# jacarvalho/mpd-public

Measured on AMD Instinct MI355X. Metric: denoising-steps/s, higher is better.
Workload: dtype f32; 1 GPU; cfg2: EnvDense2D-RobotPointMass shape, 100 trajectories (1 context(s)) x H=64 x D=4, T=100 (+5) reverse steps, unguided, U-Net dim_mults (1, 2, 4, 8), one plan = one bench step; parallelism=single, denoising_steps_per_plan=105

## Files before the change

include/mpdx.h:

```cpp
#ifndef MPDX_H
#define MPDX_H

#include <stddef.h>
#include <stdint.h>

#ifdef __cplusplus
extern "C" {
#endif

#define MPDX_E_INVALID   (-1)
#define MPDX_E_NOTFOUND  (-2)
#define MPDX_E_STATE     (-3)
#define MPDX_E_DEVICE    (-4)

#define MPDX_MAX_LEVELS 8

typedef struct mpdx_unet mpdx_unet;

typedef struct mpdx_unet_cfg {
    int32_t state_dim;
    int32_t n_support_points;
    int32_t unet_input_dim;
    int32_t n_levels;
    int32_t dim_mults[MPDX_MAX_LEVELS];
    int32_t time_emb_dim;
    int32_t self_attention;
} mpdx_unet_cfg;

const char* mpdx_last_error(void);
int mpdx_version(void);

int    mpdx_unet_create(const mpdx_unet_cfg* cfg, mpdx_unet** out);
void   mpdx_unet_destroy(mpdx_unet* u);
int    mpdx_unet_set_plan_join(mpdx_unet* u, int on);
int    mpdx_unet_plan_joined(const mpdx_unet* u);
int    mpdx_unet_set_inner_run(mpdx_unet* u, int on);
int    mpdx_unet_set_inner_run_parts(mpdx_unet* u, int parts);
int    mpdx_unet_set_inner_run_width(mpdx_unet* u, int width);
int    mpdx_inner_run_block(int B, int width, int cus, int block, int32_t* cluster, int32_t* tile, int32_t* counter_lines);
int    mpdx_unet_inner_runs(const mpdx_unet* u);
int    mpdx_unet_inner_run_layers(const mpdx_unet* u);
int    mpdx_unet_status(const mpdx_unet* u);
int    mpdx_unet_set_status(mpdx_unet* u, unsigned word);
int    mpdx_unet_num_params(const mpdx_unet* u);
int    mpdx_unet_param_info(const mpdx_unet* u, int idx, const char** name, int32_t shape[3], int32_t* ndim);
size_t mpdx_unet_packed_floats(const mpdx_unet* u);
size_t mpdx_unet_timetab_floats(const mpdx_unet* u, int T);
size_t mpdx_unet_workspace_floats(const mpdx_unet* u, int B);
int    mpdx_unet_pack_param(mpdx_unet* u, const char* name, const float* src_dev, size_t n_floats,
                            float* packed_dev, void* stream);
int    mpdx_unet_build_timetab(mpdx_unet* u, const float* packed_dev, const float* freqs16_dev, int T,
                               float* timetab_dev, void* stream);

int mpdx_unet_forward(mpdx_unet* u, const float* packed_dev, const float* timetab_dev, int T,
                      const float* x, int t, float* eps, int B, float* ws, void* stream);

typedef struct mpdx_step_coefs {
    float sqrt_recip_alphas_cumprod;
    float sqrt_recipm1_alphas_cumprod;
    float posterior_mean_coef1;
    float posterior_mean_coef2;
    float noise_scale;
    float noise_std_extra;
    int32_t predict_epsilon;
    int32_t clip_denoised;
    float ddim_k1;
    float ddim_k2;
    float guide_scale;
} mpdx_step_coefs;

int mpdx_ddpm_step(mpdx_unet* u, const float* packed_dev, const float* timetab_dev, int T,
                   float* x_io, const float* noise, const float* hard_start, const float* hard_goal,
                   const mpdx_step_coefs* coefs, int t, int mean_only, float* chain_out,
                   uint32_t* absmax_out, int n_per_ctx, int B, float* ws, void* stream);

int mpdx_add_noise(float* x_io, const float* noise, const float* hard_start, const float* hard_goal,
                   float noise_scale, float noise_std_extra, float* chain_out, int B, int H, int D, void* stream);

int mpdx_hard_conds(float* x_io, float* chain_out, int n, const int32_t* horizon_idx, const float* const* values, int B, int H, int D, void* stream);

int mpdx_q_sample(const float* x_start, const float* noise, const long long* t_dev, const float* sqrt_alphas_cumprod_dev,
                  const float* sqrt_one_minus_alphas_cumprod_dev, const float* hard_start, const float* hard_goal, float* out, int B, int H,
                  int D, int T, void* stream);
int mpdx_weighted_loss(const float* pred, const float* targ, const float* weights_hd, const float* hard_start, const float* hard_goal,
                       int l1, float* out1, int B, int H, int D, void* stream);

size_t mpdx_train_flat_floats(mpdx_unet* u);
size_t mpdx_train_dgrad_pack_floats(mpdx_unet* u);
size_t mpdx_train_workspace_floats(mpdx_unet* u, int B);
int    mpdx_train_param_offset(mpdx_unet* u, int idx, size_t* off, size_t* n);
int    mpdx_train_pack(mpdx_unet* u, const float* flat, float* packed, float* packedT, void* stream);
int    mpdx_train_loss_backward(mpdx_unet* u, const float* flat, const float* packed, const float* packedT, float* grads_flat,
                                const float* x_start, const float* noise, const long long* t_dev, const float* sqrt_alphas_cumprod_dev,
                                const float* sqrt_one_minus_alphas_cumprod_dev, const float* freqs16, const float* hard_start,
                                const float* hard_goal, const float* weights_hd, int T, int B, int predict_epsilon, int l1, float loss_scale,
                                float* loss_out, float* ws, void* stream);
int    mpdx_adam_step(float* params, const float* grads, float* exp_avg, float* exp_avg_sq, size_t n, float lr, float beta1, float beta2,
                      float eps, int step, float max_norm, float* scratch, void* stream);
int    mpdx_train_draw(mpdx_unet* u, unsigned long long seed, const int* step_counter_dev);
int    mpdx_ema_update(float* ema, const float* params, size_t n, float beta, void* stream);

int mpdx_randn(float* out, size_t n, uint64_t seed, uint64_t offset, void* stream);

#define MPDX_MAX_FIELDS 4
#define MPDX_FIELD_OBJECTS   0
#define MPDX_FIELD_WORKSPACE 1
#define MPDX_FIELD_SELF      2
#define MPDX_FIELD_GRID      3
#define MPDX_ROBOT_POINTMASS 0
#define MPDX_ROBOT_PANDA     1
#define MPDX_ROBOT_CHAIN     2

typedef struct mpdx_field {
    int32_t kind;
    float   weight;
    int32_t sphere_off, n_spheres;
    int32_t box_off, n_boxes;
    float   ws_min[3], ws_max[3];
    int32_t grid_sdf_off;
    int32_t grid_grad_off;
    int32_t n[3];
    float   origin[3];
    float   cell;
    int32_t mode;
} mpdx_field;
#define MPDX_GRID_LINEAR  0
#define MPDX_GRID_NEAREST 1

typedef struct mpdx_guide_params {
    int32_t robot;
    int32_t q_dim;
    int32_t ws_dim;
    int32_t interpolate;
    int32_t n_interp;
    int32_t clip_grad;
    float   max_grad_norm;
    float   mins[16], maxs[16];
    float   cutoff_margin;
    float   link_margin;
    int32_t n_fields;
    mpdx_field fields[MPDX_MAX_FIELDS];
    int32_t use_gp;
    float   gp_weight;
    float   dt;
    float   sigma_gp;
    const float* prims;
    int32_t n_prim_floats;
    int32_t clip_rule;
    float   max_grad_value;
    int32_t gp_half_factor;
    int32_t identity_normalizer;
    const float* grids;
    int32_t n_grid_floats;
    int32_t n_scenes;
    int32_t scene_stride;
    const int32_t* scene_of_ctx;
    int32_t scene_n_per_ctx;
    const float* chain;
    int32_t n_chain_floats;
    int32_t tool_frame;
    float   tool_axis[3];
    float   tool_world[3];
    float   tool_cos_min;
    float   tool_weight;
} mpdx_guide_params;
#define MPDX_ROBOT_CHAIN_MAX_JOINTS    8
#define MPDX_ROBOT_CHAIN_MAX_SPHERES   16
#define MPDX_ROBOT_CHAIN_MAX_PAIRS     24
#define MPDX_ROBOT_CHAIN_HEADER_FLOATS 4
#define MPDX_ROBOT_CHAIN_JOINT_FLOATS  16
#define MPDX_ROBOT_CHAIN_SPHERE_FLOATS 8
#define MPDX_ROBOT_CHAIN_REVOLUTE      0
#define MPDX_ROBOT_CHAIN_PRISMATIC     1
#define MPDX_SCENE_HEADER_WORDS 8
#define MPDX_SCENE_MAX_STAGED_FLOATS 12288

int mpdx_guide_step(const mpdx_guide_params* gp, float* x, float* grad_out, const float* hard_start, const float* hard_goal,
                    const uint32_t* absmax_in, uint32_t* absmax_out, int n_per_ctx, int B, int H, int D, void* stream);
int mpdx_guide_step_scaled(const mpdx_guide_params* gp, float* x, float* grad_out, const float* hard_start, const float* hard_goal,
                           const uint32_t* absmax_in, uint32_t* absmax_out, int n_per_ctx, int B, int H, int D, float guide_scale,
                           void* stream);
int mpdx_guide_time(const mpdx_guide_params* gp, float* x, float* grad_out, const uint32_t* absmax_in, int n_per_ctx, int B, int H, int D,
                    int reps, void* stream, float* ms_avg);
int mpdx_guide_trace(const mpdx_guide_params* gp, float* x, const uint32_t* absmax_in, int B, int H, int D, void* stream,
                     long long* stamps128);
int mpdx_guide_variant(const mpdx_guide_params* gp, int B, int H, int D);
int mpdx_absmax(const float* x, uint32_t* absmax_out, int n_per_ctx, int B, int H, int D, void* stream);

int mpdx_traj_metrics(const mpdx_guide_params* gp, const float* x_unnormalised, float* out4, int n_check, int B, int H, int D,
                      void* stream);
int mpdx_traj_metrics_mask(const mpdx_guide_params* gp, const float* x_unnormalised, float* out4, uint8_t* mask, int n_check, int B,
                           int H, int D, void* stream);

int mpdx_traj_tool_metrics(const mpdx_guide_params* gp, const float* x_unnormalised, float* out2, uint8_t* mask, int n_check, int B, int H, int D,
                           void* stream);

int mpdx_sdf_grid_bake(const mpdx_guide_params* gp, int field, float* sdf_out, float* grad_out, const int n[3], const float origin[3], float cell,
                       void* stream);

size_t mpdx_sdf_grid_edt_ws_bytes(const int n[3]);
int mpdx_sdf_grid_from_occupancy(const uint8_t* occ, float* sdf_out, float* grad_out, int32_t* d2_out, const int n[3], float cell, float inflate, void* ws,
                                 size_t ws_bytes, void* stream);
int mpdx_occupancy_from_points(const float* points, int n_points, uint8_t* occ, const int n[3], const float origin[3], float cell, void* stream);

#define MPDX_MESH_SIGN_WINDING 0
#define MPDX_MESH_SIGN_NONE    1
int mpdx_sdf_grid_from_mesh(const float* vertices, int n_vertices, const int32_t* faces, int n_faces, float* sdf_out, float* grad_out ,
                            float* wind_out , const int n[3], const float origin[3], float cell, float inflate,
                            int sign_mode, void* stream);

typedef struct mpdx_gpmp_opts {
    float   sigma_obs;
    float   lambda_up, lambda_down, lambda_min, lambda_max;
    float   step;
    int32_t adaptive;
} mpdx_gpmp_opts;
int mpdx_gpmp_step(const mpdx_guide_params* gp, const mpdx_gpmp_opts* opts, float* x, float* delta, float* state, int B, int H, int D,
                   int solve, void* stream);

typedef struct mpdx_rrt_opts {
    float    q_lo[8], q_hi[8];
    float    step;
    int32_t  max_nodes, max_iters, max_connect_steps, n_edge_checks;
    uint64_t seed;
} mpdx_rrt_opts;
int mpdx_rrt_connect(const mpdx_guide_params* gp, const mpdx_rrt_opts* opts, const float* start, const float* goal, float* nodes,
                     int32_t* parent, int32_t* count, int32_t* link, int32_t* iters, int n, void* stream);

int mpdx_rrt_paths(const mpdx_guide_params* gp, const float* start, const float* goal, const float* nodes, const int32_t* parent, const int32_t* link,
                   float* trajs_out, int32_t* path_len, int n, int max_nodes, int H, float dt, int n_edge_checks, int rounds, void* stream);

typedef struct mpdx_ik_opts {
    int32_t  frame;
    float    offset[3];
    float    q_lo[8], q_hi[8];
    float    rot_weight;
    float    pos_tol, rot_tol;
    float    lambda_init, lambda_up, lambda_down, lambda_min, lambda_max;
    int32_t  adaptive;
    int32_t  max_iters;
    uint64_t seed;
} mpdx_ik_opts;
int mpdx_ik_solve(const mpdx_guide_params* gp, const mpdx_ik_opts* opts, const float* target, const float* q_init, float* q_out, float* err_out,
                  int32_t* status, int n, int restarts, void* stream);

int mpdx_plan(mpdx_unet* u, const float* packed_dev, const float* timetab_dev, int T, const mpdx_step_coefs* coefs,
              int n_without_noise, float* x, const float* noise, const float* hard_start, const float* hard_goal,
              float* chain, int B, float* ws, const mpdx_guide_params* guide, int n_guide_steps, int t_start_guide,
              uint32_t* guide_flags, int n_per_ctx, uint64_t rng_seed, uint64_t rng_offset, void* stream);

int mpdx_unet_profile(mpdx_unet* u, const float* packed_dev, const float* timetab_dev, int T, const float* x, int t,
                      int B, float* ws, void* stream, int cap, float* ms_out, double* flops_out,
                      const char** names_out, int* n_out);
int mpdx_layer_trace(mpdx_unet* u, const float* packed_dev, const float* timetab_dev, const float* x, int layer, int B, float* ws,
                     void* stream, long long* stamps32);
int mpdx_fused_trace(mpdx_unet* u, const float* packed_dev, const float* timetab_dev, const float* x, int seg, int B,
                     float* ws, void* stream, long long* stamps_out, int cap, int* n_out, int* nops_out);
int mpdx_unet_time_units(mpdx_unet* u, const float* packed_dev, const float* timetab_dev, int T, const float* x, int t, int B,
                         float* ws, void* stream, int unit_first, int unit_last, int reps, float* ms_avg);
int mpdx_unet_time_without(mpdx_unet* u, const float* packed_dev, const float* timetab_dev, int T, const float* x, int t, int B,
                           float* ws, void* stream, unsigned long long skip_mask, int reps, float* ms_avg);
int mpdx_unet_unit_layer(const mpdx_unet* u, int B, int i);
int mpdx_unet_fused_program(const mpdx_unet* u, int seg);
double mpdx_unet_unit_bytes(const mpdx_unet* u, int B, int i);
int mpdx_unet_unit_is_pair(const mpdx_unet* u, int B, int i);
int mpdx_bench_layer(mpdx_unet* u, const float* packed_dev, const float* timetab_dev, const float* x, int layer, int B,
                     float* ws, void* stream, int reps, int dbg, float* ms_per_launch);
int mpdx_unet_layer_tile(const mpdx_unet* u, int i, int B, char* buf, size_t buflen);
int mpdx_attention_block(float* x, const float* to_qkv_w, const float* to_out_w, const float* to_out_b, const float* norm_g, const float* norm_b,
                         int B, int L, int Lv, int C, void* stream);

#ifdef __cplusplus
}
#endif
#endif
```

mpd_public_amd/_lib.py:

```python
from __future__ import annotations

import ctypes as C
from pathlib import Path

import os as _os

_LIB_PATH = Path(_os.environ["MPDX_LIB"]) if _os.environ.get("MPDX_LIB") else Path(__file__).resolve().parent / "libmpdx.so"
_lib = None

MAX_LEVELS = 8


class UnetCfg(C.Structure):
    _fields_ = [("state_dim", C.c_int32), ("n_support_points", C.c_int32), ("unet_input_dim", C.c_int32),
                ("n_levels", C.c_int32), ("dim_mults", C.c_int32 * MAX_LEVELS), ("time_emb_dim", C.c_int32),
                ("self_attention", C.c_int32)]


class StepCoefs(C.Structure):
    _fields_ = [("sqrt_recip_alphas_cumprod", C.c_float), ("sqrt_recipm1_alphas_cumprod", C.c_float),
                ("posterior_mean_coef1", C.c_float), ("posterior_mean_coef2", C.c_float),
                ("noise_scale", C.c_float), ("noise_std_extra", C.c_float),
                ("predict_epsilon", C.c_int32), ("clip_denoised", C.c_int32), ("ddim_k1", C.c_float), ("ddim_k2", C.c_float),
                ("guide_scale", C.c_float)]


MAX_FIELDS = 4
SCENE_HEADER_WORDS = 2 * MAX_FIELDS
SCENE_MAX_STAGED_FLOATS = 12 * 1024
FIELD_OBJECTS, FIELD_WORKSPACE, FIELD_SELF, FIELD_GRID = 0, 1, 2, 3
GRID_LINEAR, GRID_NEAREST = 0, 1
MESH_SIGN_WINDING, MESH_SIGN_NONE = 0, 1
ROBOT_POINTMASS, ROBOT_PANDA, ROBOT_CHAIN = 0, 1, 2
ROBOT_CHAIN_MAX_JOINTS, ROBOT_CHAIN_MAX_SPHERES, ROBOT_CHAIN_MAX_PAIRS = 8, 16, 24
ROBOT_CHAIN_HEADER_FLOATS, ROBOT_CHAIN_JOINT_FLOATS, ROBOT_CHAIN_SPHERE_FLOATS = 4, 16, 8
ROBOT_CHAIN_REVOLUTE, ROBOT_CHAIN_PRISMATIC = 0, 1


class Field(C.Structure):
    _fields_ = [("kind", C.c_int32), ("weight", C.c_float), ("sphere_off", C.c_int32), ("n_spheres", C.c_int32),
                ("box_off", C.c_int32), ("n_boxes", C.c_int32), ("ws_min", C.c_float * 3), ("ws_max", C.c_float * 3),
                ("grid_sdf_off", C.c_int32), ("grid_grad_off", C.c_int32), ("n", C.c_int32 * 3), ("origin", C.c_float * 3),
                ("cell", C.c_float), ("mode", C.c_int32)]


class GuideParams(C.Structure):
    _fields_ = [("robot", C.c_int32), ("q_dim", C.c_int32), ("ws_dim", C.c_int32), ("interpolate", C.c_int32),
                ("n_interp", C.c_int32), ("clip_grad", C.c_int32), ("max_grad_norm", C.c_float),
                ("mins", C.c_float * 16), ("maxs", C.c_float * 16), ("cutoff_margin", C.c_float), ("link_margin", C.c_float),
                ("n_fields", C.c_int32), ("fields", Field * MAX_FIELDS), ("use_gp", C.c_int32), ("gp_weight", C.c_float),
                ("dt", C.c_float), ("sigma_gp", C.c_float), ("prims", C.c_void_p), ("n_prim_floats", C.c_int32),
                ("clip_rule", C.c_int32), ("max_grad_value", C.c_float), ("gp_half_factor", C.c_int32),
                ("identity_normalizer", C.c_int32), ("grids", C.c_void_p), ("n_grid_floats", C.c_int32),
                ("n_scenes", C.c_int32), ("scene_stride", C.c_int32), ("scene_of_ctx", C.c_void_p), ("scene_n_per_ctx", C.c_int32),
                ("chain", C.c_void_p), ("n_chain_floats", C.c_int32),
                ("tool_frame", C.c_int32), ("tool_axis", C.c_float * 3), ("tool_world", C.c_float * 3), ("tool_cos_min", C.c_float),
                ("tool_weight", C.c_float)]


class GpmpOpts(C.Structure):
    _fields_ = [("sigma_obs", C.c_float), ("lambda_up", C.c_float), ("lambda_down", C.c_float), ("lambda_min", C.c_float),
                ("lambda_max", C.c_float), ("step", C.c_float), ("adaptive", C.c_int32)]


class RrtOpts(C.Structure):
    _fields_ = [("q_lo", C.c_float * 8), ("q_hi", C.c_float * 8), ("step", C.c_float), ("max_nodes", C.c_int32), ("max_iters", C.c_int32),
                ("max_connect_steps", C.c_int32), ("n_edge_checks", C.c_int32), ("seed", C.c_uint64)]


class IkOpts(C.Structure):
    _fields_ = [("frame", C.c_int32), ("offset", C.c_float * 3), ("q_lo", C.c_float * 8), ("q_hi", C.c_float * 8), ("rot_weight", C.c_float),
                ("pos_tol", C.c_float), ("rot_tol", C.c_float), ("lambda_init", C.c_float), ("lambda_up", C.c_float), ("lambda_down", C.c_float),
                ("lambda_min", C.c_float), ("lambda_max", C.c_float), ("adaptive", C.c_int32), ("max_iters", C.c_int32), ("seed", C.c_uint64)]


_vp, _sz, _i, _f = C.c_void_p, C.c_size_t, C.c_int, C.c_float
SIGNATURES = {
    "mpdx_last_error": (C.c_char_p, []),
    "mpdx_version": (_i, []),
    "mpdx_unet_create": (_i, [C.POINTER(UnetCfg), C.POINTER(_vp)]),
    "mpdx_unet_destroy": (None, [_vp]),
    "mpdx_unet_set_plan_join": (_i, [_vp, _i]),
    "mpdx_unet_plan_joined": (_i, [_vp]),
    "mpdx_unet_set_inner_run": (_i, [_vp, _i]),
    "mpdx_unet_set_inner_run_parts": (_i, [_vp, _i]),
    "mpdx_unet_set_inner_run_width": (_i, [_vp, _i]),
    "mpdx_inner_run_block": (_i, [_i, _i, _i, _i, _vp, _vp, _vp]),
    "mpdx_unet_inner_runs": (_i, [_vp]),
    "mpdx_unet_inner_run_layers": (_i, [_vp]),
    "mpdx_unet_status": (_i, [_vp]),
    "mpdx_unet_set_status": (_i, [_vp, C.c_uint]),
    "mpdx_unet_num_params": (_i, [_vp]),
    "mpdx_unet_param_info": (_i, [_vp, _i, C.POINTER(C.c_char_p), C.POINTER(C.c_int32 * 3), C.POINTER(C.c_int32)]),
    "mpdx_unet_packed_floats": (_sz, [_vp]),
    "mpdx_unet_timetab_floats": (_sz, [_vp, _i]),
    "mpdx_unet_workspace_floats": (_sz, [_vp, _i]),
    "mpdx_unet_pack_param": (_i, [_vp, C.c_char_p, _vp, _sz, _vp, _vp]),
    "mpdx_unet_build_timetab": (_i, [_vp, _vp, _vp, _i, _vp, _vp]),
    "mpdx_unet_forward": (_i, [_vp, _vp, _vp, _i, _vp, _i, _vp, _i, _vp, _vp]),
    "mpdx_ddpm_step": (_i, [_vp, _vp, _vp, _i, _vp, _vp, _vp, _vp, C.POINTER(StepCoefs), _i, _i, _vp, _vp, _i, _i, _vp, _vp]),
    "mpdx_add_noise": (_i, [_vp, _vp, _vp, _vp, _f, _f, _vp, _i, _i, _i, _vp]),
    "mpdx_hard_conds": (_i, [_vp, _vp, _i, C.POINTER(C.c_int32), C.POINTER(_vp), _i, _i, _i, _vp]),
    "mpdx_q_sample": (_i, [_vp, _vp, _vp, _vp, _vp, _vp, _vp, _vp, _i, _i, _i, _i, _vp]),
    "mpdx_weighted_loss": (_i, [_vp, _vp, _vp, _vp, _vp, _i, _vp, _i, _i, _i, _vp]),
    "mpdx_plan": (_i, [_vp, _vp, _vp, _i, C.POINTER(StepCoefs), _i, _vp, _vp, _vp, _vp, _vp, _i, _vp,
                        C.POINTER(GuideParams), _i, _i, _vp, _i, C.c_uint64, C.c_uint64, _vp]),
    "mpdx_guide_step": (_i, [C.POINTER(GuideParams), _vp, _vp, _vp, _vp, _vp, _vp, _i, _i, _i, _i, _vp]),
    "mpdx_guide_step_scaled": (_i, [C.POINTER(GuideParams), _vp, _vp, _vp, _vp, _vp, _vp, _i, _i, _i, _i, _f, _vp]),
    "mpdx_guide_time": (_i, [C.POINTER(GuideParams), _vp, _vp, _vp, _i, _i, _i, _i, _i, _vp, C.POINTER(C.c_float)]),
    "mpdx_traj_metrics": (_i, [C.POINTER(GuideParams), _vp, _vp, _i, _i, _i, _i, _vp]),
    "mpdx_traj_metrics_mask": (_i, [C.POINTER(GuideParams), _vp, _vp, _vp, _i, _i, _i, _i, _vp]),
    "mpdx_traj_tool_metrics": (_i, [C.POINTER(GuideParams), _vp, _vp, _vp, _i, _i, _i, _i, _vp]),
    "mpdx_guide_trace": (_i, [C.POINTER(GuideParams), _vp, _vp, _i, _i, _i, _vp, C.POINTER(C.c_longlong)]),
    "mpdx_guide_variant": (_i, [C.POINTER(GuideParams), _i, _i, _i]),
    "mpdx_absmax": (_i, [_vp, _vp, _i, _i, _i, _i, _vp]),
    "mpdx_sdf_grid_bake": (_i, [C.POINTER(GuideParams), _i, _vp, _vp, C.POINTER(C.c_int * 3), C.POINTER(C.c_float * 3), _f, _vp]),
    "mpdx_sdf_grid_edt_ws_bytes": (_sz, [C.POINTER(C.c_int * 3)]),
    "mpdx_sdf_grid_from_occupancy": (_i, [_vp, _vp, _vp, _vp, C.POINTER(C.c_int * 3), _f, _f, _vp, _sz, _vp]),
    "mpdx_occupancy_from_points": (_i, [_vp, _i, _vp, C.POINTER(C.c_int * 3), C.POINTER(C.c_float * 3), _f, _vp]),
    "mpdx_sdf_grid_from_mesh": (_i, [_vp, _i, _vp, _i, _vp, _vp, _vp, C.POINTER(C.c_int * 3), C.POINTER(C.c_float * 3), _f, _f, _i, _vp]),
    "mpdx_unet_profile": (_i, [_vp, _vp, _vp, _i, _vp, _i, _i, _vp, _vp, _i, C.POINTER(C.c_float), C.POINTER(C.c_double),
                                C.POINTER(C.c_char_p), C.POINTER(C.c_int)]),
    "mpdx_layer_trace": (_i, [_vp, _vp, _vp, _vp, _i, _i, _vp, _vp, C.POINTER(C.c_longlong)]),
    "mpdx_fused_trace": (_i, [_vp, _vp, _vp, _vp, _i, _i, _vp, _vp, C.POINTER(C.c_longlong), _i, C.POINTER(C.c_int), C.POINTER(C.c_int)]),
    "mpdx_unet_time_units": (_i, [_vp, _vp, _vp, _i, _vp, _i, _i, _vp, _vp, _i, _i, _i, C.POINTER(C.c_float)]),
    "mpdx_unet_time_without": (_i, [_vp, _vp, _vp, _i, _vp, _i, _i, _vp, _vp, C.c_uint64, _i, C.POINTER(C.c_float)]),
    "mpdx_unet_unit_layer": (_i, [_vp, _i, _i]),
    "mpdx_unet_unit_is_pair": (_i, [_vp, _i, _i]),
    "mpdx_unet_unit_bytes": (C.c_double, [_vp, _i, _i]),
    "mpdx_unet_fused_program": (_i, [_vp, _i]),
    "mpdx_bench_layer": (_i, [_vp, _vp, _vp, _vp, _i, _i, _vp, _vp, _i, _i, C.POINTER(C.c_float)]),
    "mpdx_unet_layer_tile": (_i, [_vp, _i, _i, C.c_char_p, _sz]),
    "mpdx_attention_block": (_i, [_vp, _vp, _vp, _vp, _vp, _vp, _i, _i, _i, _i, _vp]),
    "mpdx_randn": (_i, [_vp, _sz, C.c_uint64, C.c_uint64, _vp]),
    "mpdx_train_flat_floats": (_sz, [_vp]),
    "mpdx_train_dgrad_pack_floats": (_sz, [_vp]),
    "mpdx_train_workspace_floats": (_sz, [_vp, _i]),
    "mpdx_train_param_offset": (_i, [_vp, _i, C.POINTER(_sz), C.POINTER(_sz)]),
    "mpdx_train_pack": (_i, [_vp, _vp, _vp, _vp, _vp]),
    "mpdx_train_loss_backward": (_i, [_vp, _vp, _vp, _vp, _vp, _vp, _vp, _vp, _vp, _vp, _vp, _vp, _vp, _vp, _i, _i, _i, _i, _f, _vp, _vp, _vp]),
    "mpdx_adam_step": (_i, [_vp, _vp, _vp, _vp, _sz, _f, _f, _f, _f, _i, _f, _vp, _vp]),
    "mpdx_train_draw": (_i, [_vp, C.c_uint64, _vp]),
    "mpdx_ema_update": (_i, [_vp, _vp, _sz, _f, _vp]),
    "mpdx_gpmp_step": (_i, [C.POINTER(GuideParams), C.POINTER(GpmpOpts), _vp, _vp, _vp, _i, _i, _i, _i, _vp]),
    "mpdx_rrt_paths": (_i, [C.POINTER(GuideParams), _vp, _vp, _vp, _vp, _vp, _vp, _vp, _i, _i, _i, _f, _i, _i, _vp]),
    "mpdx_rrt_connect": (_i, [C.POINTER(GuideParams), C.POINTER(RrtOpts), _vp, _vp, _vp, _vp, _vp, _vp, _vp, _i, _vp]),
    "mpdx_ik_solve": (_i, [C.POINTER(GuideParams), C.POINTER(IkOpts), _vp, _vp, _vp, _vp, _vp, _i, _i, _vp]),
}


def lib_path() -> Path:
    return _LIB_PATH


class LibraryUnavailable(RuntimeError):
    """libmpdx.so is missing or cannot be loaded on this host (every compute entry point raises it; nothing falls back)"""


def load():
    global _lib
    if _lib is not None:
        return _lib
    if not _LIB_PATH.exists():
        raise LibraryUnavailable(f"{_LIB_PATH} is missing - build it with `python -m mpd_public_amd.build` (hipcc, gfx950). "
                           "mpd_public_amd has no CPU fallback.")
    try:
        lib = C.CDLL(str(_LIB_PATH))
    except OSError as e:
        raise LibraryUnavailable(f"cannot load {_LIB_PATH}: {e}") from e
    for name, (res, args) in SIGNATURES.items():
        try:
            fn = getattr(lib, name)
        except AttributeError as e:
            raise LibraryUnavailable(f"{_LIB_PATH} does not export {name}; rebuild it") from e
        fn.restype, fn.argtypes = res, args
    _lib = lib
    return lib


def check(rc: int, what: str = "") -> None:
    if rc != 0:
        msg = load().mpdx_last_error()
        raise RuntimeError(f"libmpdx {what} failed (code {rc}): {msg.decode() if msg else '?'}")


def ptr(t) -> int:
    if t is None:
        return None
    return t.data_ptr()


def current_stream() -> int:
    import torch
    return torch.cuda.current_stream().cuda_stream
```

mpd_public_amd/csrc/fused_level.hpp:

```cpp
#pragma once
#include "conv_block.hpp"
#include "fused_geom.hpp"

namespace mpdx {

#define MPDX_FUSED_SHAPES(X)                                                                                   \
    X(0, CONV_S1, 5, 1, 0, 32, 64, 1) X(1, CONV_S1, 5, 2, 1, 32, 64, 1) X(2, CONV_S1, 5, 2, 0, 32, 64, 1) X(3, CONV_DOWN, 3, 2, 0, 32, 32, 0)     \
    X(4, CONV_S1, 5, 2, 0, 64, 32, 1) X(5, CONV_S1, 5, 4, 2, 64, 32, 1) X(6, CONV_S1, 5, 4, 0, 64, 32, 1) X(7, CONV_DOWN, 3, 4, 0, 64, 16, 0)     \
    X(8, CONV_S1, 5, 16, 0, 64, 16, 1) X(9, CONV_S1, 5, 4, 16, 64, 16, 1) X(10, CONV_S1, 5, 4, 0, 64, 16, 1) X(11, CONV_UPT, 4, 4, 0, 64, 32, 0)  \
    X(12, CONV_S1, 5, 8, 0, 32, 32, 1) X(13, CONV_S1, 5, 2, 8, 32, 32, 1) X(14, CONV_S1, 5, 2, 0, 32, 32, 1) X(15, CONV_UPT, 4, 2, 0, 32, 64, 0) \
    X(16, CONV_S1, 5, 4, 0, 128, 16, 1) X(17, CONV_S1, 5, 8, 4, 128, 16, 1) X(18, CONV_S1, 5, 8, 0, 128, 16, 1) X(19, CONV_DOWN, 3, 8, 0, 128, 8, 0)
constexpr int kFusedShapeFinal = 63;

inline int fused_shape_id(int mode, int ks, int nc16, int rnc16, int cout, int L_out, int gn) {
#define X(id, M, K, N, R, CO, LO, G) if (mode == M && ks == K && nc16 == N && rnc16 == R && cout == CO && L_out == LO && gn == G) return id;
    MPDX_FUSED_SHAPES(X)
#undef X
    return -1;
}

constexpr int kFusedWaves = 4;
constexpr int kFusedThreads = 64 * kFusedWaves;

template <int MODE_, int KS_, int NC16_, int NCR_, int COUT_, int LOUT_, int GN_>
struct FusedShape {
    static constexpr int MODE = MODE_, KS = KS_, NC16 = NC16_, NCR = NCR_, COUT = COUT_, LOUT = LOUT_, GN = GN_;
    static constexpr int NTAP = (MODE == CONV_UPT) ? 2 : KS;
    static constexpr int NBLK = NC16 * NTAP;
    static constexpr int TOT = NBLK + NCR;
    static constexpr int MSn = COUT / 16;
    static constexpr int MSW = MSn < kFusedWaves ? MSn : kFusedWaves;
    static constexpr int MP = MSn / MSW;
    static constexpr int NSn = LOUT >= 16 ? LOUT / 16 : 1;
    static constexpr int T = MSn * NSn;
    static constexpr int NTW = T / kFusedWaves;
    static constexpr int NSEQ = (MODE == CONV_UPT) ? NTW : MP;
    static constexpr int NJ = (MODE == CONV_UPT) ? 1 : NTW / MP;
    static constexpr int SLEN = NSEQ * TOT;
    static constexpr int GS = COUT / 8;
    static constexpr int RB = GS / 4;
    static constexpr int NPARTS = NSn * RB;
    static_assert(T == 4 || T == 8, "4 or 8 tiles");
    static_assert(MSn == 2 || MSn == 4 || MSn == 8, "2, 4 or 8 tile rows");
    static_assert(MP == 1 || (MODE != CONV_UPT && NSn == 1), "M-passes: one position tile");
    static_assert(MODE != CONV_UPT || NTW == 2, "ConvTranspose: a wave owns both parities of its tile");
    static_assert(MODE != CONV_UPT || NCR == 0, "no folded residual on resampling ops");
    static_assert(!GN || NPARTS == 2 || NPARTS == 4, "GroupNorm region of 128 or 256 elements");
    static_assert(LOUT >= 16 || !GN, "half-used tiles: resampling ops only");
};

struct FusedOp {
    int shape;
    int src_off4, src_rs4;
    int rsrc_off4, rsrc_rs4;
    int res_off4, res_rs4;
    int dst_off4, dst_rs4;
    int gdst;
    int sbase;
    int p_off;
    int tb_off;
    int save_out, save_pre;
};

constexpr int kMaxFusedOps = 16;
#ifndef MPDX_FUSED_RING
#define MPDX_FUSED_RING 16
#endif
#ifndef MPDX_FUSED_DB
#define MPDX_FUSED_DB 2
#endif
constexpr int kFusedRing = MPDX_FUSED_RING;

struct FusedArgs {
    const float* packed;
    const float* tt_row;
    const float* gsrc1;
    const float* gsrc2;
    float* gout[3];
    int gc1, gc2, L0;
    int in_off4, in_rs4, in_rows, in_clear;
    const float* gsrc3;
    float* save;
    int tt_stride;
    int fpar_off;
    int c3, L3, s3_off4, s3_rs4, s3_col4;
    int B, nops;
    int stat_off;
    int par_off;
    int gpar_off, par_floats;
    int tt_off;
    int tt_lo, tt_n;
    int lg_c4n;
    FusedOp ops[kMaxFusedOps];
    int msmask[kMaxFusedOps];
    int slen[kMaxFusedOps];
    const float* x_in; const float* noise; const float* hs; const float* hg;
    float* out; float* chain; uint32_t* absmax;
    int D, Cf, fmode, n_per_ctx, fw_off, fb_off, H;
    mpdx_step_coefs k;
    NoiseRng rng;
    long long* trace;
};

struct FusedJoinDown {
    const float* packed;
    const float* tt_row;
    float* gout[3];
    int gpar_off, tt_lo;
    int sbase[kMaxFusedOps];
};
struct FusedJoinArgs { FusedArgs up; FusedJoinDown dn; };
__device__ __forceinline__ FusedOp fused_runtime_desc(const FusedJoinDown& a, int i) {
    FusedOp op = {};
    op.sbase = a.sbase[i]; op.save_out = op.save_pre = -1;
    return op;
}

struct FusedLay {
    int in_off4, in_rs4, in_rows, L0, gc1, gc2, c3, L3, s3_off4, s3_rs4, s3_col4, stat_off, par_off, par_floats, tt_off, tt_n, fpar_off, H, Cf, lg_c4n;
};
template <class GEOM>
__device__ __forceinline__ FusedLay fused_lay(const FusedArgs& a) {
    if constexpr (GEOM::has) {
        constexpr FusedGeom g = GEOM::g;
        constexpr int c4n = (g.gc1 + g.gc2 + 3) >> 2;
        constexpr int lg = g.gc1 < 0 ? -2 : (c4n == 1 ? 0 : c4n == 2 ? 1 : c4n == 4 ? 2 : c4n == 8 ? 3 : c4n == 16 ? 4 : c4n == 32 ? 5 : c4n == 64 ? 6 : -1);
        return FusedLay{g.in_off4, g.in_rs4, g.in_rows, g.L0, g.gc1 < 0 ? a.gc1 : g.gc1, g.gc1 < 0 ? a.gc2 : g.gc2, g.c3, g.L3, g.s3_off4, g.s3_rs4, g.s3_col4,
                        g.stat_off, g.par_off, g.par_floats < 0 ? a.par_floats : g.par_floats, g.tt_off, g.tt_n, g.fpar_off, g.H, g.Cf,
                        lg == -2 ? a.lg_c4n : lg};
    } else {
        return FusedLay{a.in_off4, a.in_rs4, a.in_rows, a.L0, a.gc1, a.gc2, a.c3, a.L3, a.s3_off4, a.s3_rs4, a.s3_col4, a.stat_off, a.par_off, a.par_floats,
                        a.tt_off, a.tt_n, a.fpar_off, a.H, a.Cf, a.lg_c4n};
    }
}

inline bool fused_geom_matches(const FusedArgs& a, const FusedGeom& g, int state_dim) {
    if (a.nops != g.nops || a.in_off4 != g.in_off4 || a.in_rs4 != g.in_rs4 || a.in_rows != g.in_rows || a.L0 != g.L0) return false;
    if (g.gc1 < 0) { if (a.gc1 != state_dim || a.gc2 != 0 || state_dim > 16) return false; }
    else if (a.gc1 != g.gc1 || a.gc2 != g.gc2) return false;
    if (a.c3 != g.c3 || (g.c3 && (a.L3 != g.L3 || a.s3_off4 != g.s3_off4 || a.s3_rs4 != g.s3_rs4 || a.s3_col4 != g.s3_col4))) return false;
    if (a.stat_off != g.stat_off || a.par_off != g.par_off || a.tt_off != g.tt_off || a.tt_n != g.tt_n) return false;
    if (g.par_floats >= 0 && a.par_floats != g.par_floats) return false;
    if (g.H && (a.H != g.H || a.Cf != g.Cf || a.fpar_off != g.fpar_off || state_dim > 16)) return false;
    for (int k = 0; k < g.nops; ++k) {
        const FusedOp& o = a.ops[k];
        const FusedGeomOp& t = g.ops[k];
        if (o.shape != t.shape || o.src_off4 != t.src_off4 || o.src_rs4 != t.src_rs4) return false;
        if (o.shape == kFusedShapeFinal) continue;
        if (o.rsrc_off4 != t.rsrc_off4 || o.rsrc_rs4 != t.rsrc_rs4 || o.res_off4 != t.res_off4 || o.res_rs4 != t.res_rs4 || o.dst_off4 != t.dst_off4 ||
            o.dst_rs4 != t.dst_rs4 || o.gdst != t.gdst || o.p_off != t.p_off || o.tb_off != t.tb_off)
            return false;
    }
    return true;
}

__device__ __forceinline__ void lds_barrier() { asm volatile("s_waitcnt lgkmcnt(0)\n\ts_barrier" ::: "memory"); }

typedef int i32x4_t __attribute__((ext_vector_type(4)));
__device__ __forceinline__ __amdgpu_buffer_rsrc_t fused_weights_rsrc(const float* packed) {
    return __builtin_amdgcn_make_buffer_rsrc((void*)packed, 0, 0x7fffffff, 0x00020000);
}
__device__ __forceinline__ f32x4 fused_ld_block(__amdgpu_buffer_rsrc_t rs, int stream_bytes, int blk, unsigned lane_bytes) {
    return __builtin_bit_cast(f32x4, __builtin_amdgcn_raw_buffer_load_b128(rs, (int)lane_bytes, stream_bytes + blk * 1024, 0));
}

__device__ __forceinline__ void fused_ring_request(f32x4 (&ring)[kFusedRing], __amdgpu_buffer_rsrc_t rs, int wbase, int slen, unsigned lane_bytes) {
#pragma unroll
    for (int p = 0; p < kFusedRing; ++p)
        if (p < slen) ring[p] = fused_ld_block(rs, wbase, p, lane_bytes);
    __builtin_amdgcn_sched_barrier(0);
}


__device__ __forceinline__ float row_sum16(float v) {
    v += __builtin_bit_cast(float, __builtin_amdgcn_update_dpp(0, __builtin_bit_cast(int, v), 0xB1, 0xF, 0xF, true));
    v += __builtin_bit_cast(float, __builtin_amdgcn_update_dpp(0, __builtin_bit_cast(int, v), 0x4E, 0xF, 0xF, true));
    v += __builtin_bit_cast(float, __builtin_amdgcn_update_dpp(0, __builtin_bit_cast(int, v), 0x141, 0xF, 0xF, true));
    v += __builtin_bit_cast(float, __builtin_amdgcn_update_dpp(0, __builtin_bit_cast(int, v), 0x140, 0xF, 0xF, true));
    return v;
}

template <class S, bool SAVE = false, class A = FusedArgs>
__device__ __forceinline__ void fused_conv_op(const A& a, const FusedLay& lay, const FusedOp& op, f32x4 (&ring)[kFusedRing], float* smem, int wave, int lane, int b,
                                              int nbase, int nmax, long long* tr_base, int& tr) {
    constexpr int P = kFusedRing, DB = MPDX_FUSED_DB, NTW = S::NTW, NJ = S::NJ;
    f32x4* const sm4 = (f32x4*)smem;
    const int j = lane & 15, q = lane >> 4;
    const int ms = wave & (S::MSW - 1);
    const int nsg = wave / S::MSW;
#define FOP_STAMP() do { if (tr_base) tr_base[tr] = (long long)__builtin_readcyclecounter(); ++tr; } while (0)
    int ns[NTW], npos[NTW];
#pragma unroll
    for (int t = 0; t < NTW; ++t) {
        ns[t] = (S::MP > 1) ? 0 : nsg * NTW + t;
        npos[t] = (S::MODE == CONV_UPT) ? 2 * (nsg * 16 + j) + t : ns[t] * 16 + j;
    }
    const bool col_ok = S::LOUT >= 16 || j < S::LOUT;
    const f32x4* brow[NJ];
    const f32x4* rrow[NJ];
#pragma unroll
    for (int t = 0; t < NJ; ++t) {
        int boff;
        if (S::MODE == CONV_UPT) boff = op.src_off4 + (nsg * 16 + j + 2) * op.src_rs4 + q;
        else {
            constexpr int pad = (S::MODE == CONV_S1) ? S::KS / 2 : 1;
            int l = ns[t] * 16 + j;
            if (S::LOUT < 16) l = l < S::LOUT ? l : S::LOUT - 1;
            boff = op.src_off4 + ((S::MODE == CONV_DOWN ? 2 * l : l) + 2 - pad) * op.src_rs4 + q;
        }
        brow[t] = sm4 + boff;
        rrow[t] = sm4 + (S::NCR > 0 ? op.rsrc_off4 + (ns[t] * 16 + j + 2) * op.rsrc_rs4 + q : 0);
    }
    const int rs4 = op.src_rs4;
    const __amdgpu_buffer_rsrc_t wrs = fused_weights_rsrc(a.packed);
    const int sbase = (op.sbase + ms * (S::SLEN * 256)) * 4;
    const unsigned lane_bytes = (unsigned)lane * 16u;
    auto read_b = [&](int r, int t) -> f32x4 {
        const int rr = r % S::TOT, par = r / S::TOT;
        if (rr < S::NBLK) {
            const int c16 = rr / S::NTAP, ts = rr % S::NTAP;
            const int roff = (S::MODE == CONV_UPT) ? ((ts == 0) ? 0 : (par == 0 ? -1 : 1)) : ts;
            return brow[t][roff * rs4 + c16 * 4];
        }
        return rrow[t][(rr - S::NBLK) * 4];
    };
    f32x4 acc[NTW][2], racc[NTW][2];
#pragma unroll
    for (int t = 0; t < NTW; ++t) acc[t][0] = acc[t][1] = racc[t][0] = racc[t][1] = (f32x4){0.f, 0.f, 0.f, 0.f};
    FOP_STAMP();
    f32x4 bq[DB + 1][NJ];
#pragma unroll
    for (int r = 0; r < DB && r < S::SLEN; ++r)
#pragma unroll
        for (int t = 0; t < NJ; ++t) bq[r][t] = read_b(r, t);
    __builtin_amdgcn_sched_barrier(0);
#pragma unroll
    for (int r = 0; r < S::SLEN; ++r) {
        if (r + DB < S::SLEN) {
#pragma unroll
            for (int t = 0; t < NJ; ++t) bq[(r + DB) % (DB + 1)][t] = read_b(r + DB, t);
        }
        const f32x4 af = ring[r % P];
        const bool is_res = (r % S::TOT) >= S::NBLK;
#pragma unroll
        for (int e = 0; e < 4; ++e)
#pragma unroll
            for (int t = 0; t < NJ; ++t) {
                const int tt = (S::NSEQ > 1) ? r / S::TOT : t;
                f32x4& d = is_res ? racc[tt][e & 1] : acc[tt][e & 1];
                d = __builtin_amdgcn_mfma_f32_16x16x4f32(af[e], bq[r % (DB + 1)][t][e], d, 0, 0, 0);
            }
        if (r + P < S::SLEN) ring[r % P] = fused_ld_block(wrs, sbase, r + P, lane_bytes);
        else { const int k = r % P; ring[k] = fused_ld_block(wrs, nbase, k < nmax ? k : nmax, lane_bytes); }
        if (S::SLEN < P) {
#pragma unroll
            for (int k = S::SLEN; k < P; ++k)
                if ((k - S::SLEN) % S::SLEN == r) ring[k] = fused_ld_block(wrs, nbase, k < nmax ? k : nmax, lane_bytes);
        }
        __builtin_amdgcn_sched_barrier(0);
    }
    FOP_STAMP();

    __builtin_amdgcn_s_setprio(2);
    const float* par_op = smem + lay.par_off + op.p_off;
    int c0t[NTW], mst[NTW];
#pragma unroll
    for (int t = 0; t < NTW; ++t) { mst[t] = (S::MP > 1) ? ms + t * S::MSW : ms; c0t[t] = mst[t] * 16 + q * 4; }
    f32x4 y[NTW];
    if (S::GN) {
        constexpr bool LOCAL = (S::MSW == kFusedWaves);
        constexpr int NG = (S::MP > 1) ? NTW : 1;
        constexpr int TPG = NTW / NG;
        f32x4 v[NTW], addv[NTW], gat[NTW], bet[NTW];
        bool have_add = false;
#pragma unroll
        for (int t = 0; t < NTW; ++t) {
            const int c0 = c0t[t];
            const f32x4 bi = *(const f32x4*)(par_op + c0);
            if (S::MP > 1 || t == 0) { gat[t] = *(const f32x4*)(par_op + S::COUT + c0); bet[t] = *(const f32x4*)(par_op + 2 * S::COUT + c0); }
            else { gat[t] = gat[0]; bet[t] = bet[0]; }
            if (op.tb_off >= 0) { addv[t] = *(const f32x4*)(smem + lay.tt_off + op.tb_off + c0); have_add = true; }
            if (S::NCR > 0) {
                const f32x4 r = (racc[t][0] + racc[t][1]) + *(const f32x4*)(par_op + 3 * S::COUT + c0);
                addv[t] = (op.tb_off >= 0) ? addv[t] + r : r;
                have_add = true;
            } else if (op.res_off4 >= 0) {
                const f32x4 r = sm4[op.res_off4 + (npos[t] + 2) * op.res_rs4 + (c0 >> 2)];
                addv[t] = (op.tb_off >= 0) ? addv[t] + r : r;
                have_add = true;
            }
            v[t] = (acc[t][0] + acc[t][1]) + bi;
            if constexpr (SAVE) if (op.save_pre >= 0) *(f32x4*)(a.save + op.save_pre + ((size_t)b * S::LOUT + npos[t]) * S::COUT + c0) = v[t];
        }
        auto rows_sum = [&](float x) -> float {
            if constexpr (LOCAL && S::RB >= 2)
                x += __builtin_bit_cast(float, __builtin_amdgcn_ds_swizzle(__builtin_bit_cast(int, x), 0x401F));
            if constexpr (LOCAL && S::RB == 4)
                x += __builtin_bit_cast(float, __builtin_amdgcn_ds_bpermute((lane ^ 32) << 2, __builtin_bit_cast(int, x)));
            return x;
        };
        constexpr int NLOC = 64 * TPG * (LOCAL ? S::RB : 1);
        float mean_g[NG], rstd_g[NG];
        f32x4 d[NTW];
        float m2_g[NG];
#pragma unroll
        for (int g = 0; g < NG; ++g) {
            float sl = 0.f;
#pragma unroll
            for (int k = 0; k < TPG; ++k) {
                const f32x4& x = v[g * TPG + k];
                const float p = (x[0] + x[1]) + (x[2] + x[3]);
                sl = (k == 0) ? p : sl + p;
            }
            mean_g[g] = rows_sum(row_sum16(sl)) * (1.0f / (float)NLOC);
            float ql = 0.f;
#pragma unroll
            for (int k = 0; k < TPG; ++k) {
                const int t = g * TPG + k;
                d[t] = v[t] - mean_g[g];
                const float p = (d[t][0] * d[t][0] + d[t][1] * d[t][1]) + (d[t][2] * d[t][2] + d[t][3] * d[t][3]);
                ql = (k == 0) ? p : ql + p;
            }
            m2_g[g] = rows_sum(row_sum16(ql));
        }
        if constexpr (LOCAL) {
            FOP_STAMP();
#pragma unroll
            for (int g = 0; g < NG; ++g) rstd_g[g] = gn_rstd(m2_g[g] * (1.0f / (float)NLOC));
        } else {
            float* stat = smem + lay.stat_off;
            if (j == 0) *(f32x2*)(stat + ((nsg * S::MSW + ms) * 4 + q) * 2) = (f32x2){mean_g[0], m2_g[0]};
            lds_barrier();
            FOP_STAMP();
            const f32x2 o = *(const f32x2*)(stat + (((nsg ^ 1) * S::MSW + ms) * 4 + q) * 2);
            const float dm = o[0] - mean_g[0];
            const float mean = 0.5f * (mean_g[0] + o[0]);
            const float M2 = (m2_g[0] + o[1]) + (0.5f * (float)NLOC) * (dm * dm);
            rstd_g[0] = gn_rstd(M2 * (1.0f / (float)(2 * NLOC)));
            const float shift = mean_g[0] - mean;
#pragma unroll
            for (int t = 0; t < NTW; ++t) d[t] = d[t] + shift;
        }
#pragma unroll
        for (int t = 0; t < NTW; ++t) {
            const int g = (S::MP > 1) ? t : 0;
            const f32x4 sc = gat[t] * rstd_g[g];
#pragma unroll
            for (int e = 0; e < 4; ++e) y[t][e] = mish_nosel(d[t][e] * sc[e] + bet[t][e]);
            if (have_add) y[t] += addv[t];
        }
    } else {
#pragma unroll
        for (int t = 0; t < NTW; ++t) y[t] = (acc[t][0] + acc[t][1]) + *(const f32x4*)(par_op + c0t[t]);
        FOP_STAMP();
    }
#pragma unroll
    for (int t = 0; t < NTW; ++t) {
        if (!col_ok) continue;
        if (op.dst_off4 >= 0) sm4[op.dst_off4 + (npos[t] + 2) * op.dst_rs4 + (c0t[t] >> 2)] = y[t];
        if (op.gdst >= 0) *(f32x4*)(a.gout[op.gdst] + ((size_t)b * S::LOUT + npos[t]) * S::COUT + c0t[t]) = y[t];
        if constexpr (SAVE) if (op.save_out >= 0) *(f32x4*)(a.save + op.save_out + ((size_t)b * S::LOUT + npos[t]) * S::COUT + c0t[t]) = y[t];
    }
    if (op.dst_off4 >= 0) {
        const f32x4 z = {0.f, 0.f, 0.f, 0.f};
        const int tid = wave * 64 + lane;
        if (tid < 2 * op.dst_rs4) {
            sm4[op.dst_off4 + tid] = z;
            sm4[op.dst_off4 + (S::LOUT + 2) * op.dst_rs4 + tid] = z;
        }
    }
    FOP_STAMP();
    __builtin_amdgcn_s_setprio(0);
    lds_barrier();
    FOP_STAMP();
#undef FOP_STAMP
}

template <class GEOM>
__device__ __forceinline__ void fused_prologue(const FusedArgs& a, const FusedLay& lay, float* smem, f32x4 (&ring)[kFusedRing], int tid, int lane, int wave, int b,
                                               long long* tr_base, int& tr) {
    f32x4* const sm4 = (f32x4*)smem;
#define FUSED_STAMP() do { if (tr_base) tr_base[tr] = (long long)__builtin_readcyclecounter(); ++tr; } while (0)
    fused_ring_request(ring, fused_weights_rsrc(a.packed), (a.ops[0].sbase + (wave & a.msmask[0]) * a.slen[0] * 256) * 4, a.slen[0], (unsigned)lane * 16u);

    constexpr int NT_ = kFusedThreads;
    constexpr int kIn4 = !GEOM::has ? 2048 : (GEOM::g.gc1 < 0 ? GEOM::g.L0 * 4 : GEOM::g.L0 * ((GEOM::g.gc1 + GEOM::g.gc2 + 3) / 4));
    constexpr int kS34 = !GEOM::has ? 1024 : GEOM::g.L3 * (GEOM::g.c3 / 4);
    constexpr int kPar4 = !GEOM::has ? 2048
                                     : ((GEOM::g.par_floats >= 0 ? GEOM::g.par_floats : GEOM::g.fpar_off + (16 * (GEOM::g.Cf + 4) + 16 + 3) / 4 * 4) + GEOM::g.tt_n) / 4;
    const int cin = lay.gc1 + lay.gc2;
    const int c4n = (cin + 3) >> 2;
    const int n_in = lay.L0 * c4n;
    constexpr int IK = (kIn4 + NT_ - 1) / NT_;
    f32x4 iv[IK];
    int idst[IK], ck[IK];
    const bool vec_ok = ((lay.gc1 & 3) == 0) && ((lay.gc2 & 3) == 0);
    {
        int lk[IK];
        bool vk[IK];
#pragma unroll
        for (int k = 0; k < IK; ++k) {
            const int idx = tid + k * NT_;
            vk[k] = idx < n_in;
            const int idc = vk[k] ? idx : 0;
            lk[k] = lay.lg_c4n >= 0 ? (idc >> lay.lg_c4n) : (idc / c4n);
            ck[k] = (idc - lk[k] * c4n) << 2;
            idst[k] = vk[k] ? lay.in_off4 + (lk[k] + 2) * lay.in_rs4 + (ck[k] >> 2) : -1;
        }
        if (vec_ok) {
#pragma unroll
            for (int k = 0; k < IK; ++k) {
                if (k * NT_ >= n_in) continue;
                const size_t pos = (size_t)b * lay.L0 + lk[k];
                const float* src = (ck[k] < lay.gc1) ? a.gsrc1 + pos * lay.gc1 + ck[k] : a.gsrc2 + pos * lay.gc2 + (ck[k] - lay.gc1);
                iv[k] = *(const f32x4*)src;
            }
        } else {
#pragma unroll
            for (int k = 0; k < IK; ++k) {
                if (k * NT_ >= n_in) continue;
                const size_t pos = (size_t)b * lay.L0 + lk[k];
#pragma unroll
                for (int e = 0; e < 4; ++e) {
                    const int ce = ck[k] + e;
                    const float* src = (ce < lay.gc1) ? a.gsrc1 + pos * lay.gc1 + ce : (ce < cin) ? a.gsrc2 + pos * lay.gc2 + (ce - lay.gc1) : a.gsrc1 + pos * lay.gc1;
                    iv[k][e] = *src;
                }
            }
        }
    }
    constexpr int SK = (kS34 + NT_ - 1) / NT_;
    f32x4 sv[SK > 0 ? SK : 1];
    const int s3c4 = lay.c3 >> 2, n_s3 = lay.L3 * s3c4;
#pragma unroll
    for (int k = 0; k < SK; ++k) {
        const int idx = tid + k * NT_;
        if (k * NT_ >= n_s3) continue;
        sv[k] = *(const f32x4*)(a.gsrc3 + ((size_t)b * n_s3 + (idx < n_s3 ? idx : 0)) * 4);
    }
    constexpr int PK = (kPar4 + NT_ - 1) / NT_;
    f32x4 pv[PK];
    const int npar4 = lay.par_floats >> 2, ntt4 = lay.tt_n >> 2;
#pragma unroll
    for (int k = 0; k < PK; ++k) {
        const int idx = tid + k * NT_;
        if (k * NT_ >= npar4 + ntt4) continue;
        const float* src = idx < npar4 ? a.packed + a.gpar_off + (size_t)idx * 4 : a.tt_row + (size_t)b * a.tt_stride + a.tt_lo + (size_t)(idx - npar4 < ntt4 ? idx - npar4 : 0) * 4;
        pv[k] = *(const f32x4*)src;
    }
    FUSED_STAMP();
    {
        const f32x4 z = {0.f, 0.f, 0.f, 0.f};
        for (int i = tid; i < 2 * lay.in_rs4; i += NT_) {
            sm4[lay.in_off4 + i] = z;
            sm4[lay.in_off4 + (lay.in_rows - 2) * lay.in_rs4 + i] = z;
        }
        if (a.in_clear) {
            const int padw = lay.in_rs4 - c4n;
            for (int i = tid; i < lay.L0 * padw; i += NT_) {
                const int l = i / padw, cc = i - l * padw;
                sm4[lay.in_off4 + (l + 2) * lay.in_rs4 + c4n + cc] = z;
            }
        }
    }
    FUSED_STAMP();
#pragma unroll
    for (int k = 0; k < IK; ++k) {
        if (!vec_ok) {
#pragma unroll
            for (int e = 0; e < 4; ++e) iv[k][e] = (ck[k] + e < cin) ? iv[k][e] : 0.f;
        }
        if (idst[k] >= 0) sm4[idst[k]] = iv[k];
    }
#pragma unroll
    for (int k = 0; k < SK; ++k) {
        const int idx = tid + k * NT_;
        if (idx < n_s3) {
            const int l = idx / s3c4, c = idx - l * s3c4;
            sm4[lay.s3_off4 + (l + 2) * lay.s3_rs4 + lay.s3_col4 + c] = sv[k];
        }
    }
#pragma unroll
    for (int k = 0; k < PK; ++k) {
        const int idx = tid + k * NT_;
        if (idx < npar4) sm4[(lay.par_off >> 2) + idx] = pv[k];
        else if (idx - npar4 < ntt4) sm4[(lay.tt_off >> 2) + idx - npar4] = pv[k];
    }
    lds_barrier();
    FUSED_STAMP();

#undef FUSED_STAMP
}

constexpr int kFinalPre = 4;
struct FinalPre { float xv[kFinalPre], nz[kFinalPre], hc[kFinalPre]; };

__device__ __forceinline__ void fused_final_prefetch(const FusedArgs& a, const FusedLay& lay, FinalPre& fp, int tid, int b) {
    if (a.fmode == 0) return;
    const int H = lay.H, n = H * a.D;
#pragma unroll
    for (int k = 0; k < kFinalPre; ++k) {
        const int idx = tid + k * kFusedThreads;
        if (k * kFusedThreads >= n) continue;
        const int ic = idx < n ? idx : 0;
        const int p = ic / a.D, d = ic - p * a.D;
        const size_t o = (size_t)b * n + ic;
        fp.xv[k] = a.x_in[o];
        if (a.fmode == 1 && !a.rng.on && a.noise) fp.nz[k] = a.noise[o];
        if (a.hs && p == 0) fp.hc[k] = a.hs[(size_t)b * a.D + d];
        if (a.hg && p == H - 1) fp.hc[k] = a.hg[(size_t)b * a.D + d];
    }
}

template <int CF = 0, int JOIN_OFF4 = -1, int JOIN_RS4 = 0>
__device__ __forceinline__ void fused_final_op(const FusedArgs& a, const FusedLay& lay, const FusedOp& op, const FinalPre& fp, float* smem, int tid, int lane, int b) {
    f32x4* const sm4 = (f32x4*)smem;
    constexpr int NT_ = kFusedThreads;
    float vmax = 0.f;
    const int H = lay.H, n = H * a.D;
    const int Cf = CF ? CF : lay.Cf;
    const int wrs = Cf + 4;
    const float* const fw = smem + lay.par_off + lay.fpar_off;
    float nzr[kFinalPre];
    const bool coop = a.fmode == 1 && a.rng.on && (((a.rng.elem0 + (unsigned long long)b * (unsigned)n) & 3ull) == 0ull) && (n & 3) == 0;
    if (coop) {
        const int qidx = (tid & ~63) + (lane >> 4) * NT_ + (lane & 15) * 4;
        float z[4] = {0.f, 0.f, 0.f, 0.f};
        if (qidx < n) philox_normal4(a.rng.seed, a.rng.offset + ((a.rng.elem0 + (unsigned long long)b * (unsigned)n + (unsigned)qidx) >> 2), z);
#pragma unroll
        for (int k = 0; k < kFinalPre; ++k) {
            const int src = k * 16 + (lane >> 2);
            const float v0 = __shfl(z[0], src, 64), v1 = __shfl(z[1], src, 64), v2 = __shfl(z[2], src, 64), v3 = __shfl(z[3], src, 64);
            const int c = lane & 3;
            nzr[k] = c == 0 ? v0 : c == 1 ? v1 : c == 2 ? v2 : v3;
        }
    }
#pragma unroll
    for (int k = 0; k < kFinalPre; ++k) {
        const int idx = tid + k * NT_;
        if (idx >= n) continue;
        const int p = idx / a.D, d = idx - p * a.D;
        float s = fw[a.D * wrs + d];
        const float* wrow = fw + d * wrs;
#pragma unroll
        for (int c = 0; c < Cf; c += 4) {
            const f32x4 hv = sm4[op.src_off4 + (p + 2) * op.src_rs4 + (c >> 2)];
            const f32x4 wv = *(const f32x4*)(wrow + c);
            s = fmaf(hv[0], wv[0], s); s = fmaf(hv[1], wv[1], s);
            s = fmaf(hv[2], wv[2], s); s = fmaf(hv[3], wv[3], s);
        }
        const size_t o = (size_t)b * n + idx;
        float r;
        if (a.fmode == 0) {
            r = s;
        } else {
            const float xv = fp.xv[k];
            float x0 = a.k.predict_epsilon
                           ? __fsub_rn(__fmul_rn(a.k.sqrt_recip_alphas_cumprod, xv), __fmul_rn(a.k.sqrt_recipm1_alphas_cumprod, s))
                           : s;
            if (a.fmode == 3) {
                const float pn = a.k.predict_epsilon
                                     ? s
                                     : __fdiv_rn(__fsub_rn(__fmul_rn(a.k.sqrt_recip_alphas_cumprod, xv), s), a.k.sqrt_recipm1_alphas_cumprod);
                r = __fadd_rn(__fmul_rn(x0, a.k.ddim_k1), __fmul_rn(a.k.ddim_k2, pn));
                if (a.hs && p == 0) r = fp.hc[k];
                if (a.hg && p == H - 1) r = fp.hc[k];
            } else {
                if (a.k.clip_denoised) x0 = fminf(fmaxf(x0, -1.0f), 1.0f);
                r = __fadd_rn(__fmul_rn(a.k.posterior_mean_coef1, x0), __fmul_rn(a.k.posterior_mean_coef2, xv));
                if (a.fmode == 1) {
                    if (a.rng.on) r = __fadd_rn(r, __fmul_rn(__fmul_rn(a.k.noise_scale, coop ? nzr[k] : philox_normal_at(a.rng.seed, a.rng.offset, a.rng.elem0 + o)), a.k.noise_std_extra));
                    else if (a.noise) r = __fadd_rn(r, __fmul_rn(__fmul_rn(a.k.noise_scale, fp.nz[k]), a.k.noise_std_extra));
                    if (a.hs && p == 0) r = fp.hc[k];
                    if (a.hg && p == H - 1) r = fp.hc[k];
                }
            }
        }
        a.out[o] = r;
        if (a.chain) a.chain[o] = r;
        if constexpr (JOIN_OFF4 >= 0) smem[(JOIN_OFF4 + (p + 2) * JOIN_RS4) * 4 + d] = r;
        vmax = fmaxf(vmax, fabsf(r));
    }
    if (a.absmax) {
#pragma unroll
        for (int s = 32; s >= 1; s >>= 1) vmax = fmaxf(vmax, __shfl_xor(vmax, s, 64));
        if (lane == 0) atomicMax(a.absmax + b / a.n_per_ctx, __float_as_uint(vmax));
    }
}

template <bool SAVE>
__global__ __launch_bounds__(kFusedThreads) void fused_level_kernel(const FusedArgs a) {
#ifndef MPDX_NO_WARM_KERNARG
    warm_kernarg<(int)sizeof(FusedArgs)>();
#endif
    extern __shared__ __attribute__((aligned(16))) float smem[];
    const int tid = threadIdx.x, lane = tid & 63;
    const int wave = __builtin_amdgcn_readfirstlane(tid >> 6);
    const int b = blockIdx.x;
    int tr = 0;
    long long* const tr_base = (MPDX_TRACE_PTR(a.trace) && b == 0 && lane == 0) ? a.trace + wave * 128 : nullptr;
    if (tr_base) tr_base[tr] = (long long)__builtin_readcyclecounter();
    ++tr;
    f32x4 ring[kFusedRing];
    FinalPre fp;
    const FusedLay lay = fused_lay<GeomNone>(a);
    fused_prologue<GeomNone>(a, lay, smem, ring, tid, lane, wave, b, tr_base, tr);
    for (int oi = 0; oi < a.nops; ++oi) {
        const FusedOp op = a.ops[oi];
        if (oi + 1 < a.nops && a.ops[oi + 1].shape == kFusedShapeFinal) fused_final_prefetch(a, lay, fp, tid, b);
        if (op.shape == kFusedShapeFinal) {
            fused_final_op(a, lay, op, fp, smem, tid, lane, b);
            if (tr_base) tr_base[tr] = (long long)__builtin_readcyclecounter();
            ++tr;
            continue;
        }
        int nbase = op.sbase * 4;
        int nmax = 0;
        if (oi + 1 < a.nops && a.ops[oi + 1].shape != kFusedShapeFinal) {
            nbase = (a.ops[oi + 1].sbase + (wave & a.msmask[oi + 1]) * a.slen[oi + 1] * 256) * 4;
            nmax = a.slen[oi + 1] - 1;
        }
        switch (op.shape) {
#define X(id, M, K, N, R, CO, LO, G) \
    case id: fused_conv_op<FusedShape<M, K, N, R, CO, LO, G>, SAVE>(a, lay, op, ring, smem, wave, lane, b, nbase, nmax, tr_base, tr); break;
            MPDX_FUSED_SHAPES(X)
#undef X
            default: break;
        }
    }
}

template <int ID> struct FusedShapeOf;
#define X(id, M, K, N, R, CO, LO, G) template <> struct FusedShapeOf<id> { using type = FusedShape<M, K, N, R, CO, LO, G>; };
MPDX_FUSED_SHAPES(X)
#undef X

__device__ __forceinline__ FusedOp fused_runtime_desc(const FusedArgs& a, int i) { return a.ops[i]; }
template <class GEOM, int I, bool SAVE, class A = FusedArgs>
__device__ __forceinline__ FusedOp fused_static_desc(const A& a) {
    FusedOp op = fused_runtime_desc(a, I);
    if constexpr (GEOM::has) {
        constexpr FusedGeomOp g = GEOM::g.ops[I];
        op.shape = g.shape;
        op.src_off4 = g.src_off4; op.src_rs4 = g.src_rs4; op.rsrc_off4 = g.rsrc_off4; op.rsrc_rs4 = g.rsrc_rs4;
        op.res_off4 = g.res_off4; op.res_rs4 = g.res_rs4; op.dst_off4 = g.dst_off4; op.dst_rs4 = g.dst_rs4;
        op.p_off = g.p_off; op.tb_off = g.tb_off;
        if constexpr (!SAVE) op.gdst = g.gdst;
    }
    return op;
}

template <class GEOM, int SH, int I, int NEXT_SH, int PREV_COUT, bool SAVE>
__device__ __forceinline__ void fused_static_op(const FusedArgs& a, const FusedLay& lay, f32x4 (&ring)[kFusedRing], FinalPre& fp, float* smem, int tid, int wave,
                                                int lane, int b, long long* tr_base, int& tr) {
    if constexpr (NEXT_SH == kFusedShapeFinal) fused_final_prefetch(a, lay, fp, tid, b);
    const FusedOp op = fused_static_desc<GEOM, I, SAVE>(a);
    if constexpr (SH == kFusedShapeFinal) {
        fused_final_op<PREV_COUT>(a, lay, op, fp, smem, tid, lane, b);
        if (tr_base) tr_base[tr] = (long long)__builtin_readcyclecounter();
        ++tr;
    } else {
        int nbase = a.ops[I].sbase * 4;
        int nmax = 0;
        if constexpr (NEXT_SH >= 0 && NEXT_SH != kFusedShapeFinal) {
            using N = typename FusedShapeOf<NEXT_SH>::type;
            nbase = (a.ops[I + 1].sbase + (wave & (N::MSn < kFusedWaves ? N::MSn - 1 : kFusedWaves - 1)) * (N::SLEN * 256)) * 4;
            nmax = N::SLEN - 1;
        }
        fused_conv_op<typename FusedShapeOf<SH>::type, SAVE>(a, lay, op, ring, smem, wave, lane, b, nbase, nmax, tr_base, tr);
    }
}

template <class GEOM_, int... SH>
struct FusedSeq {
    using GEOM = GEOM_;
    static constexpr int N = sizeof...(SH);
    static constexpr int ids[sizeof...(SH)] = {SH...};
    template <int I>
    static constexpr int prev_cout() {
        if constexpr (I > 0 && ids[I > 0 ? I - 1 : 0] != kFusedShapeFinal) return FusedShapeOf<ids[I > 0 ? I - 1 : 0]>::type::COUT;
        else return 0;
    }
    template <int I, bool SAVE>
    __device__ static __forceinline__ void run_from(const FusedArgs& a, const FusedLay& lay, f32x4 (&ring)[kFusedRing], FinalPre& fp, float* smem, int tid, int wave,
                                                    int lane, int b, long long* tr_base, int& tr) {
        if constexpr (I < N) {
            fused_static_op<GEOM, ids[I], I, (I + 1 < N ? ids[I + 1 < N ? I + 1 : I] : -1), prev_cout<I>(), SAVE>(a, lay, ring, fp, smem, tid, wave, lane, b, tr_base, tr);
            run_from<I + 1, SAVE>(a, lay, ring, fp, smem, tid, wave, lane, b, tr_base, tr);
        }
    }
};

template <class SEQ, bool SAVE = false>
__global__ __launch_bounds__(kFusedThreads) void fused_program_kernel(const FusedArgs a) {
#ifndef MPDX_NO_WARM_KERNARG
    warm_kernarg<(int)sizeof(FusedArgs)>();
#endif
    extern __shared__ __attribute__((aligned(16))) float smem[];
    const int tid = threadIdx.x, lane = tid & 63;
    const int wave = __builtin_amdgcn_readfirstlane(tid >> 6);
    const int b = blockIdx.x;
    int tr = 0;
    long long* const tr_base = (MPDX_TRACE_PTR(a.trace) && b == 0 && lane == 0) ? a.trace + wave * 128 : nullptr;
    if (tr_base) tr_base[tr] = (long long)__builtin_readcyclecounter();
    ++tr;
    f32x4 ring[kFusedRing];
    FinalPre fp;
    const FusedLay lay = fused_lay<typename SEQ::GEOM>(a);
    fused_prologue<typename SEQ::GEOM>(a, lay, smem, ring, tid, lane, wave, b, tr_base, tr);
    SEQ::template run_from<0, SAVE>(a, lay, ring, fp, smem, tid, wave, lane, b, tr_base, tr);
}

using FusedSeqDown = FusedSeq<GeomDown, 0, 1, 2, 2, 3, 4, 5, 6, 6, 7>;
using FusedSeqUpA = FusedSeq<GeomNone, 8, 9, 10, 10, 11>;
using FusedSeqUpB = FusedSeq<GeomNone, 12, 13, 14, 14, 15, 2, kFusedShapeFinal>;
using FusedSeqUpAB = FusedSeq<GeomUpAB, 8, 9, 10, 10, 11, 12, 13, 14, 14, 15, 2, kFusedShapeFinal>;
using FusedSeqDown3 = FusedSeq<GeomDown3, 0, 1, 2, 2, 3, 4, 5, 6, 6, 7, 16, 17, 18, 18, 19>;
using FusedSeqMid2 = FusedSeq<GeomNone, 16, 17, 18, 18, 19>;
using FusedSeqMid3 = FusedSeq<GeomMid3, 16, 17, 18, 18, 18, 18, 18, 18>;


constexpr int kJoinTail = 16512;

template <class SU, class SD>
struct FusedJoinLay {
    static constexpr FusedGeom gu = SU::GEOM::g, gd = SD::GEOM::g;
    static constexpr int shift = kJoinTail - gd.stat_off;
    static constexpr int stat_off = gd.stat_off + shift, tt_off = gd.tt_off + shift, par_off = gd.par_off + shift;
    static constexpr int lds_floats = par_off + gd.par_floats;
    static constexpr int npar4 = gd.par_floats / 4, ntt4 = gd.tt_n / 4;
    static constexpr int JK = (npar4 + ntt4 + kFusedThreads - 1) / kFusedThreads;
    static constexpr int fsrc_off4 = gu.ops[SU::N - 1].src_off4, fsrc_rs4 = gu.ops[SU::N - 1].src_rs4;
    static_assert(SU::GEOM::has && SD::GEOM::has, "joined programs need geometry tables");
    static_assert(SU::ids[SU::N - 1] == kFusedShapeFinal && SU::ids[SU::N - 2] != kFusedShapeFinal, "the up program ends in conv op + final op");
    static_assert(gd.gc1 < 0 && gd.c3 == 0 && gd.L0 == gu.H, "the down program starts from the network input");
    static_assert(gd.par_floats >= 0 && gd.par_floats % 4 == 0 && gd.tt_n % 4 == 0, "down parameters: whole float4");
    static_assert(gu.par_off + gu.fpar_off + 16 * (gu.Cf + 4) + 16 <= kJoinTail && gd.stat_off <= kJoinTail, "down tail behind both programs' other areas");
    static_assert(gd.in_off4 + gd.in_rows * gd.in_rs4 <= fsrc_off4 || fsrc_off4 + (gu.H + 4) * fsrc_rs4 <= gd.in_off4, "staged input overlaps the final op's source");
    static_assert((gd.in_off4 + gd.in_rows * gd.in_rs4) * 4 <= gu.stat_off, "staged input overlaps the up program's tail");
    static_assert(2 * gd.in_rs4 <= kFusedThreads, "the junction zeroes the halo rows in one pass of the workgroup");
};

template <class SU, class SD, int I>
__device__ __forceinline__ void fused_join_up_from(const FusedArgs& a, const FusedJoinDown& dn, const FusedLay& lay, f32x4 (&ring)[kFusedRing], FinalPre& fp, float* smem,
                                                   int tid, int wave, int lane, int b, long long* tr_base, int& tr) {
    using GU = typename SU::GEOM;
    if constexpr (I < SU::N) {
        constexpr int SH = SU::ids[I], NEXT = I + 1 < SU::N ? SU::ids[I + 1 < SU::N ? I + 1 : I] : -1;
        if constexpr (SH == kFusedShapeFinal) {
            const FusedOp op = fused_static_desc<GU, I, false>(a);
            fused_final_op<SU::template prev_cout<I>(), SD::GEOM::g.in_off4, SD::GEOM::g.in_rs4>(a, lay, op, fp, smem, tid, lane, b);
            if (tr_base) tr_base[tr] = (long long)__builtin_readcyclecounter();
            ++tr;
        } else if constexpr (NEXT == kFusedShapeFinal) {
            fused_final_prefetch(a, lay, fp, tid, b);
            const FusedOp op = fused_static_desc<GU, I, false>(a);
            using N0 = typename FusedShapeOf<SD::ids[0]>::type;
            const int nbase = (dn.sbase[0] + (wave & (N0::MSn < kFusedWaves ? N0::MSn - 1 : kFusedWaves - 1)) * (N0::SLEN * 256)) * 4;
            fused_conv_op<typename FusedShapeOf<SH>::type, false>(a, lay, op, ring, smem, wave, lane, b, nbase, N0::SLEN - 1, tr_base, tr);
        } else {
            fused_static_op<GU, SH, I, NEXT, SU::template prev_cout<I>(), false>(a, lay, ring, fp, smem, tid, wave, lane, b, tr_base, tr);
        }
        fused_join_up_from<SU, SD, I + 1>(a, dn, lay, ring, fp, smem, tid, wave, lane, b, tr_base, tr);
    }
}

template <class SD, int I>
__device__ __forceinline__ void fused_join_down_from(const FusedJoinDown& dn, const FusedLay& lay, f32x4 (&ring)[kFusedRing], float* smem, int wave, int lane, int b,
                                                     long long* tr_base, int& tr) {
    if constexpr (I < SD::N) {
        const FusedOp op = fused_static_desc<typename SD::GEOM, I, false>(dn);
        int nbase = dn.sbase[I] * 4;
        int nmax = 0;
        if constexpr (I + 1 < SD::N) {
            using N = typename FusedShapeOf<SD::ids[I + 1 < SD::N ? I + 1 : I]>::type;
            nbase = (dn.sbase[I + 1] + (wave & (N::MSn < kFusedWaves ? N::MSn - 1 : kFusedWaves - 1)) * (N::SLEN * 256)) * 4;
            nmax = N::SLEN - 1;
        }
        fused_conv_op<typename FusedShapeOf<SD::ids[I]>::type, false>(dn, lay, op, ring, smem, wave, lane, b, nbase, nmax, tr + 5 <= 128 ? tr_base : nullptr, tr);
        fused_join_down_from<SD, I + 1>(dn, lay, ring, smem, wave, lane, b, tr_base, tr);
    }
}

template <class SU, class SD>
__global__ __launch_bounds__(kFusedThreads) void fused_join_kernel(const FusedJoinArgs ja) {
#ifndef MPDX_NO_WARM_KERNARG
    warm_kernarg<(int)sizeof(FusedJoinArgs)>();
#endif
    using JL = FusedJoinLay<SU, SD>;
    extern __shared__ __attribute__((aligned(16))) float smem[];
    f32x4* const sm4 = (f32x4*)smem;
    const FusedArgs& a = ja.up;
    const FusedJoinDown& dn = ja.dn;
    const int tid = threadIdx.x, lane = tid & 63;
    const int wave = __builtin_amdgcn_readfirstlane(tid >> 6);
    const int b = blockIdx.x;
    int tr = 0;
    long long* const tr_base = (MPDX_TRACE_PTR(a.trace) && b == 0 && lane == 0) ? a.trace + wave * 128 : nullptr;
    if (tr_base) tr_base[tr] = (long long)__builtin_readcyclecounter();
    ++tr;
    f32x4 jv[JL::JK];
#pragma unroll
    for (int k = 0; k < JL::JK; ++k) {
        const int idx = tid + k * kFusedThreads;
        const int it = idx - JL::npar4 < JL::ntt4 ? idx - JL::npar4 : 0;
        const float* src = idx < JL::npar4 ? dn.packed + dn.gpar_off + (size_t)idx * 4 : dn.tt_row + dn.tt_lo + (size_t)it * 4;
        jv[k] = *(const f32x4*)src;
    }
    __builtin_amdgcn_sched_barrier(0);
    f32x4 ring[kFusedRing];
    FinalPre fp;
    const FusedLay lay = fused_lay<typename SU::GEOM>(a);
    fused_prologue<typename SU::GEOM>(a, lay, smem, ring, tid, lane, wave, b, tr_base, tr);
#pragma unroll
    for (int k = 0; k < JL::JK; ++k) {
        const int idx = tid + k * kFusedThreads;
        if (idx < JL::npar4) sm4[(JL::par_off >> 2) + idx] = jv[k];
        else if (idx - JL::npar4 < JL::ntt4) sm4[(JL::tt_off >> 2) + idx - JL::npar4] = jv[k];
    }
    fused_join_up_from<SU, SD, 0>(a, dn, lay, ring, fp, smem, tid, wave, lane, b, tr_base, tr);

    {
        constexpr FusedGeom gd = SD::GEOM::g;
        const f32x4 z = {0.f, 0.f, 0.f, 0.f};
        if (tid < 2 * gd.in_rs4) {
            sm4[gd.in_off4 + tid] = z;
            sm4[gd.in_off4 + (gd.in_rows - 2) * gd.in_rs4 + tid] = z;
        }
        const int D = a.D;
#pragma unroll
        for (int k = 0; k < (gd.L0 * gd.in_rs4 + kFusedThreads - 1) / kFusedThreads; ++k) {
            const int i = tid + k * kFusedThreads;
            if (i >= gd.L0 * gd.in_rs4) continue;
            const int l = i / gd.in_rs4, c = (i - l * gd.in_rs4) * 4;
            const int at = gd.in_off4 + (l + 2) * gd.in_rs4 + (c >> 2);
            if (c >= D) sm4[at] = z;
            else if (c + 4 > D) {
#pragma unroll
                for (int e = 1; e < 4; ++e)
                    if (c + e >= D) smem[at * 4 + e] = 0.f;
            }
        }
    }
    lds_barrier();
    if (tr_base) tr_base[tr] = (long long)__builtin_readcyclecounter();
    ++tr;
    FusedLay dlay = {};
    dlay.stat_off = JL::stat_off; dlay.par_off = JL::par_off; dlay.tt_off = JL::tt_off;
    fused_join_down_from<SD, 0>(dn, dlay, ring, smem, wave, lane, b, tr_base, tr);
}

}
```

mpd_public_amd/csrc/host.hpp:

```cpp
#pragma once
#include <hip/hip_runtime.h>

#include <algorithm>
#include <cmath>
#include <cstdarg>
#include <cstdio>
#include <cstdlib>
#include <cstring>
#include <mutex>
#include <set>
#include <string>
#include <unordered_map>
#include <vector>

#include "../../include/mpdx.h"
#include "conv_block.hpp"
#include "conv_ws.hpp"
#include "fused_level.hpp"
#include "switches.hpp"
#include "train_types.hpp"

namespace mpdx {

int fail(int code, const char* fmt, ...);
#define HIP_TRY(expr)                                                                                 \
    do {                                                                                              \
        hipError_t e_ = (expr);                                                                       \
        if (e_ != hipSuccess) return ::mpdx::fail((int)e_, "%s: %s (%s:%d)", #expr, hipGetErrorString(e_), __FILE__, __LINE__); \
    } while (0)
int raise_lds_limit(const void* kern);
int dev_hooks_missing(const char* fn);
inline bool finite_f(float v) { return fabsf(v) < 3.0e38f; }

struct FinalArgs {
    const float* h;
    const float* w;
    const float* bias;
    const float* x_in;
    const float* noise;
    const float* hs;
    const float* hg;
    float* out;
    float* chain;
    uint32_t* absmax;
    int B, H, D, C;
    int Hc;
    int mode;
    int n_per_ctx;
    mpdx_step_coefs k;
    NoiseRng rng;
};

enum ParamKind { PK_VEC = 0, PK_CONV = 1, PK_CONVT = 2 };

struct Param {
    std::string name;
    int32_t shape[3] = {0, 0, 0};
    int32_t ndim = 0;
    size_t n = 0;
    size_t off = 0;
    size_t foff = 0;
    size_t pn = 0;
    int kind = PK_VEC;
    int cout = 0, cin = 0, ksz = 0, cin_pad = 0, nslot = 0;
    bool done = false;
};

enum { SRC_X = -1, SRC_NONE = -2 };

struct Layer {
    int mode = CONV_S1, ks = 5, epi = EPI_GN_MISH;
    int c1 = 0, c2 = 0, cout = 0, L_in = 0, L_out = 0, gs = 0;
    int Lv_out = 0;
    int src1 = SRC_NONE, src2 = SRC_NONE, dst = 0, res = SRC_NONE;
    int w = -1, b = -1, gamma = -1, beta = -1;
    int tb_off = -1;
    int cin_pad = 0, rs = 0;
    bool attn = false;
    int w2 = -1, b2 = -1;
    bool pin_nt = false;
    std::string name;
};

}

struct mpdx_unet {
    mpdx_unet_cfg cfg;
    std::vector<mpdx::Param> params;
    std::unordered_map<std::string, int> pidx;
    std::vector<mpdx::Layer> layers;
    size_t packed_floats = 0;
    size_t slot_floats = 0;
    int n_slots = 0;
    int tt_row = 0;
    std::vector<int> tt_w, tt_b, tt_cout, tt_off;
    int final_slot = 0;
    int n_done = 0;
    int Hc = 0, xpad_slot = -1;
    bool masked() const { return Hc != cfg.n_support_points; }
    int plan_join = 1;
    enum RunPart { kRunSeven = 1, kRunTail = 2 };
    int inner_run = kRunSeven | kRunTail;
    int inner_run_width = 0;
    int plan_joined = 0, inner_runs = 0;
    int inner_run_layers = 0;
    struct InnerRunState {
        int capacity = -1;
        int seven_wgs[2] = {0, 0}, tail_wgs[2] = {0, 0};
        long long budget = 0;
        unsigned* counters = nullptr;
        struct Counters {
            unsigned* p = nullptr;
            unsigned base = 0;
            int live = 1 << 30;
            bool rezero = false;
        } ctr[2];
        unsigned *status = nullptr, *status_dev = nullptr;
        unsigned status_host = 0;
        unsigned status_word() const { return status ? __atomic_load_n(status, __ATOMIC_RELAXED) : status_host; }
    } run;
    struct CopyJob { size_t src, dst; int n0, ss0, ds0, n1, ss1, ds1, n_inner; };
    struct Fused {
        int first = 0, count = 0;
        bool has_final = false;
        int in1 = 0, in2 = 0;
        int in3 = mpdx::SRC_NONE;
        int gout_slot[3] = {-1, -1, -1};
        size_t lds_bytes = 0;
        mpdx::FusedArgs tmpl;
        int program = -1;
        std::vector<CopyJob> jobs;
        std::vector<int> op_layer;
        int in3_consumer = -1;
    };
    std::vector<Fused> fused;
    void* jobs_dev = nullptr;
    int n_jobs = 0;
    const float* streams_for = nullptr;
    int pack_version = 0, streams_version = -1;
    enum UnitKind { kProgram, kLayer, kPair, kInnerRun, kTailRun };
    struct Unit { UnitKind kind; int fused; int layer; int count; int width = 0; };
    std::vector<int> owner;
    struct TrainLayer {
        int src1_l = -2, src2_l = -2, res_l = -2;
        bool need_dgrad = false;
        size_t dgrad_woff = 0;
        mpdx::Layer dg;
    };
    bool train_ready = false;
    size_t flat_floats = 0, packedT_floats = 0;
    std::vector<TrainLayer> tl;
    std::vector<mpdx::PackDesc> pack_descs_host;
    void* pack_descs_dev = nullptr;
    void* pack_chunks_dev = nullptr;
    size_t n_pack_chunks = 0;
};

namespace mpdx {

int pick_row_stride(int cin_pad, int mode, int L_in, int L_out, int LP);
void choose_tile(const Layer& l, int B, int& MT, int& NT);
bool layer_ksplit(const Layer& l);
int check_ready(const mpdx_unet* u);
unsigned fused_mask(int B);
bool fused_save_variant(const mpdx_unet::Fused& f);
int ensure_fused_streams(mpdx_unet* u, const float* packed, hipStream_t st);
int claim_fused_stream_jobs(mpdx_unet* u, const float* packed, const void** jobs, int* n);
int launch_final_step(const FinalArgs& fa, hipStream_t st);
int launch_conv_layer(const Layer& l, ConvArgs& a, int B, hipStream_t st);
bool pair_tile(const Layer& l1, const Layer& l2, int B, int& MT, int& NT);
int launch_conv_pair(int MT, int NT, const ConvArgs& a1, const ConvArgs& a2, const Layer& l1, const Layer& l2, hipStream_t st);
template <int N> struct RunArgs;
bool inner_run_width_ok(int width);
int inner_run_clusters(int B, int width);
int inner_run_grid(int B, int width);
void inner_run_slot(int block, int* cluster, int* tile);
int inner_run_workgroups_per_cu(int width);
int tail_run_workgroups_per_cu(int width);
int launch_inner_run(const RunArgs<7>& ra, int B, int width, hipStream_t st);
int launch_tail_run(const RunArgs<4>& ra, int B, int width, hipStream_t st);
struct AttnArgs;
const char* attn_unsupported(int C, int L);
int launch_attention(const Layer& l, AttnArgs& a, int B, hipStream_t st);
int launch_weight_stationary(int variant, const Layer& l, ConvArgs& a, const ConvArgs& a2, int B, hipStream_t st);
int launch_fused_args(const mpdx_unet::Fused& f, const FusedArgs& a, int B, hipStream_t st, bool save = false);
int launch_fused_train(const mpdx_unet::Fused& f, const FusedArgs& a, int B, hipStream_t st);
int launch_fused_join(const FusedJoinArgs& ja, int B, hipStream_t st);
size_t fused_join_lds_bytes();
struct NoiseRng;
int launch_guide(const mpdx_guide_params* gp, float* x, float* grad_out, const float* hs, const float* hg, const uint32_t* amax_in,
                 uint32_t* amax_out, int n_per_ctx, int B, int H, int D, hipStream_t st, const float* noise = nullptr, float noise_scale = 0.f,
                 float noise_extra = 0.f, float* chain = nullptr, float guide_scale = 1.0f, const NoiseRng* rng = nullptr);
const char* chain_params_problem(const mpdx_guide_params& gp);
const char* tool_params_problem(const mpdx_guide_params& gp);
struct ChainInfo;
int guide_block_problem(const mpdx_guide_params* gp, int D, ChainInfo* chain_info);

}
```

mpd_public_amd/csrc/k_fused.hip:

```cpp
#include "host.hpp"

namespace mpdx {

int launch_fused_args(const mpdx_unet::Fused& f, const FusedArgs& a, int B, hipStream_t st, bool save) {
    if (save) return launch_fused_train(f, a, B, st);
    switch (f.program) {
        case 0:
            if (int rc = raise_lds_limit((const void*)fused_program_kernel<FusedSeqDown>)) return rc;
            hipLaunchKernelGGL(fused_program_kernel<FusedSeqDown>, dim3(B), dim3(kFusedThreads), f.lds_bytes, st, a);
            break;
        case 1:
            if (int rc = raise_lds_limit((const void*)fused_program_kernel<FusedSeqUpA>)) return rc;
            hipLaunchKernelGGL(fused_program_kernel<FusedSeqUpA>, dim3(B), dim3(kFusedThreads), f.lds_bytes, st, a);
            break;
        case 2:
            if (int rc = raise_lds_limit((const void*)fused_program_kernel<FusedSeqUpB>)) return rc;
            hipLaunchKernelGGL(fused_program_kernel<FusedSeqUpB>, dim3(B), dim3(kFusedThreads), f.lds_bytes, st, a);
            break;
        case 3:
            if (int rc = raise_lds_limit((const void*)fused_program_kernel<FusedSeqUpAB>)) return rc;
            hipLaunchKernelGGL(fused_program_kernel<FusedSeqUpAB>, dim3(B), dim3(kFusedThreads), f.lds_bytes, st, a);
            break;
        case 4:
            if (int rc = raise_lds_limit((const void*)fused_program_kernel<FusedSeqMid2>)) return rc;
            hipLaunchKernelGGL(fused_program_kernel<FusedSeqMid2>, dim3(B), dim3(kFusedThreads), f.lds_bytes, st, a);
            break;
        case 5:
            if (int rc = raise_lds_limit((const void*)fused_program_kernel<FusedSeqDown3>)) return rc;
            hipLaunchKernelGGL(fused_program_kernel<FusedSeqDown3>, dim3(B), dim3(kFusedThreads), f.lds_bytes, st, a);
            break;
        case 6:
            if (int rc = raise_lds_limit((const void*)fused_program_kernel<FusedSeqMid3>)) return rc;
            hipLaunchKernelGGL(fused_program_kernel<FusedSeqMid3>, dim3(B), dim3(kFusedThreads), f.lds_bytes, st, a);
            break;
        default:
            if (int rc = raise_lds_limit((const void*)fused_level_kernel<false>)) return rc;
            hipLaunchKernelGGL(fused_level_kernel<false>, dim3(B), dim3(kFusedThreads), f.lds_bytes, st, a);
    }
    return 0;
}

size_t fused_join_lds_bytes() { return (size_t)FusedJoinLay<FusedSeqUpAB, FusedSeqDown3>::lds_floats * sizeof(float); }
int launch_fused_join(const FusedJoinArgs& ja, int B, hipStream_t st) {
    if (int rc = raise_lds_limit((const void*)fused_join_kernel<FusedSeqUpAB, FusedSeqDown3>)) return rc;
    hipLaunchKernelGGL((fused_join_kernel<FusedSeqUpAB, FusedSeqDown3>), dim3(B), dim3(kFusedThreads), fused_join_lds_bytes(), st, ja);
    return 0;
}

}
```

mpd_public_amd/csrc/mpdx.hip:

```cpp
#include "host.hpp"
#include "attn.hpp"
#include "inner_run.hpp"
#include "loss.hpp"
#include "scene_table.hpp"

namespace mpdx {

static thread_local char g_err[512] = "";
int fail(int code, const char* fmt, ...) {
    va_list ap;
    va_start(ap, fmt);
    vsnprintf(g_err, sizeof(g_err), fmt, ap);
    va_end(ap);
    return code;
}

int raise_lds_limit(const void* kern) {
    static std::mutex mu;
    static std::set<std::pair<int, const void*>> done;
    int dev = 0;
    HIP_TRY(hipGetDevice(&dev));
    std::lock_guard<std::mutex> lock(mu);
    if (done.count({dev, kern})) return 0;
    HIP_TRY(hipFuncSetAttribute(kern, hipFuncAttributeMaxDynamicSharedMemorySize, 160 * 1024));
// ... 381 lines not shown
    int L = H, cur = SRC_X, curC = D;
    for (int i = 0; i < nl; ++i) {
        const int co = dims[i + 1];
        const std::string p = "downs." + std::to_string(i);
        const int a = other(cur);
        rtb(p + ".0", cur, curC, SRC_NONE, 0, co, L, a);
        rtb(p + ".1", a, co, SRC_NONE, 0, co, L, S0 + i);
        attention(p + ".2", S0 + i, co, L);
        cur = S0 + i; curC = co;
        if (i < nl - 1) {
            conv_layer(p + ".4.conv.weight", p + ".4.conv.bias", CONV_DOWN, 3, EPI_BIAS, cur, co, SRC_NONE, 0, co, L, L / 2, P0);
            cur = P0; L /= 2;
        }
    }
    rtb("mid_block1", cur, curC, SRC_NONE, 0, curC, L, P0);
    attention("mid_attn", P0, curC, L);
    rtb("mid_block2", P0, curC, SRC_NONE, 0, curC, L, P1);
    cur = P1;
    for (int j = 0; j < nl - 1; ++j) {
        const int lv = nl - 1 - j;
        const int dout = dims[lv + 1], din = dims[lv];
        const std::string p = "ups." + std::to_string(j);
        const int a = other(cur);
        rtb(p + ".0", cur, dout, S0 + lv, dout, din, L, a);
        const int b = other(a);
        rtb(p + ".1", a, din, SRC_NONE, 0, din, L, b);
        attention(p + ".2", b, din, L);
        const int d = other(b);
        conv_layer(p + ".4.conv.weight", p + ".4.conv.bias", CONV_UPT, 4, EPI_BIAS, b, din, SRC_NONE, 0, din, L, 2 * L, d);
        cur = d; L *= 2; curC = din;
    }
    cblock("final_conv.0", cur, curC, SRC_NONE, 0, c.unet_input_dim, L, HB);
    u->final_slot = HB;
    add_param(u, "final_conv.1.weight", {D, c.unet_input_dim, 1});
    add_param(u, "final_conv.1.bias", {D});
    u->slot_floats = std::max(slot, (size_t)c.unet_input_dim * H);
    if (H != Hv) u->xpad_slot = u->n_slots++;
}

}

#include "fused_build.hpp"

namespace mpdx {

void choose_tile(const Layer& l, int B, int& MT, int& NT) {
    const int min_mt = (l.epi == EPI_GN_MISH && l.gs > 16) ? 32 : 16;
    const int min_nt = std::max(l.mode == CONV_UPT ? 32 : 16, l.L_out);
    const long npos = (long)B * l.L_out;
    if (const char* ov = sw::tile()) {
        int mt = 0, nt = 0;
        if (sscanf(ov, "%dx%d", &mt, &nt) == 2 && mt >= min_mt && nt >= min_nt && l.cout % mt == 0 && nt % l.L_out == 0) { MT = mt; NT = nt; return; }
    }
    if (min_nt > 64) {
        NT = min_nt;
        MT = (min_mt <= 16 && l.cout % 16 == 0) ? 16 : 32;
        return;
    }
    const int target = std::max(1, sw::target_wgs());
    auto wgs = [&](int mt, int nt) { return (long)(l.cout / mt) * ((npos + nt - 1) / nt); };
    const int pad = (l.mode == CONV_S1) ? l.ks / 2 : 1;
    auto lds = [&](int mt, int nt) {
        const size_t stage = (size_t)(nt / l.L_out) * (l.L_in + 2 * pad) * l.rs * sizeof(float);
        const size_t red = (size_t)8 * nt * (mt + 4) * sizeof(float);
        return std::max(stage, red);
    };
    const int mts[2] = {32, 16}, nts[3] = {64, 32, 16};
    if (l.pin_nt && !layer_ksplit(l)) {
        NT = min_nt;
        for (int mt : mts)
            if (mt >= min_mt && l.cout % mt == 0 && lds(mt, NT) <= (size_t)sw::lds_cap_kb() * 1024 && wgs(mt, NT) >= target) { MT = mt; return; }
        MT = (min_mt <= 16 && l.cout % 16 == 0) ? 16 : 32;
        return;
    }
    const size_t cap = (size_t)sw::lds_cap_kb() * 1024;
    for (int nt : nts)
        for (int mt : mts) {
            if (mt < min_mt || nt < min_nt || l.cout % mt || lds(mt, nt) > cap) continue;
            if (wgs(mt, nt) >= target) { MT = mt; NT = nt; return; }
        }
    MT = (min_mt <= 16 && l.cout % 16 == 0) ? 16 : 32;
    NT = min_nt;
}

static int layer_ntap(const Layer& l) { return l.mode == CONV_UPT ? 2 : l.ks; }
bool layer_ksplit(const Layer& l) {
    if (!(l.mode == CONV_S1 && l.ks == 5 && l.epi == EPI_GN_MISH)) return true;
    if (const int forced = sw::ksplit(); forced >= 0) return forced != 0;
    return (l.cin_pad / 16) * layer_ntap(l) >= 16;
}
static double layer_flops(const Layer& l, int B) {
    if (l.attn) return (double)B * l.L_out * (1024.0 * l.cout + 16384.0);
    return 2.0 * l.cout * (double)B * l.L_out * (l.c1 + l.c2) * layer_ntap(l);
}


static int make_conv_args(const mpdx_unet* u, const Layer& l, const float* packed, const float* tt_row, const float* x, float* ws, int B,
                          int dbg, ConvArgs& a) {
    const size_t slot = u->slot_floats * (size_t)B;
    auto src = [&](int s) -> const float* { return s == SRC_X ? x : (s == SRC_NONE ? nullptr : ws + slot * s); };
    memset(&a, 0, sizeof(a));
    a.src1 = src(l.src1); a.src2 = src(l.src2);
    a.c1 = l.c1; a.c2 = l.c2;
    a.wp = packed + u->params[l.w].off;
    a.bias = packed + u->params[l.b].off;
    a.gamma = l.gamma >= 0 ? packed + u->params[l.gamma].off : nullptr;
    a.beta = l.beta >= 0 ? packed + u->params[l.beta].off : nullptr;
    a.tbias = (l.tb_off >= 0 && tt_row) ? tt_row + l.tb_off : nullptr;
    a.res = src(l.res);
    a.dst = ws + slot * l.dst;
    a.B = B; a.L_in = l.L_in; a.L_out = l.L_out; a.C_out = l.cout;
    a.cin_pad = l.cin_pad; a.rs = l.rs; a.gs = l.gs; a.dbg = dbg;
    a.Lv_out = l.Lv_out;
    a.trace = g_conv_trace;
    auto lg2 = [](int v) { int k = 0; while ((1 << k) < v) ++k; return k; };
    a.lg_c4n = lg2(l.cin_pad / 4); a.lg_Lin = lg2(l.L_in); a.lg_Lout = lg2(l.L_out); a.lg_gs = l.gs > 0 ? lg2(l.gs) : 0;
    if ((1 << a.lg_c4n) != l.cin_pad / 4 || (1 << a.lg_Lin) != l.L_in || (1 << a.lg_Lout) != l.L_out || (l.gs > 0 && (1 << a.lg_gs) != l.gs))
        return fail(MPDX_E_INVALID, "layer %s: channel/length/group sizes must be powers of two", l.name.c_str());
    return 0;
}

static int weight_stationary_variant(const Layer& l, const Layer* l2, const ConvArgs& a, int B, int dbg) {
    const int ws_env = sw::ws();
    const int wsn_min_b = sw::wsn_min_b(), wsp_min_b = sw::wsp_min_b();
    const bool wsn_on = sw::wsn() && ws_env != 0 && B >= wsn_min_b;
    const bool wsp_on = ws_env != 0 && B >= wsp_min_b && sw::wsp();
    if (l.mode == CONV_UPT && l.ks == 4 && l.epi == EPI_BIAS && !l2 && l.L_in == 8 && l.L_out == 16 && !l.Lv_out && l.c1 == 128 && l.c2 == 0 &&
        l.cin_pad == 128 && l.cout == 128 && !dbg && !a.pre && !a.accum && !a.dst2 && wsn_on && (long)B * 8 >= 16L * kWsGroups * 8)
        return 5;
    if (!(l.mode == CONV_S1 && l.ks == 5 && l.epi == EPI_GN_MISH && l.L_out == 8 && l.L_in == 8) || l.Lv_out) return 0;
    if (dbg || a.pre || (l.c1 & 3) || (l.c2 & 3) || l.cin_pad != l.c1 + l.c2) return 0;
    if ((long)B * l.L_out < 16L * kWsGroups * 8) return 0;
    if (ws_env == 0 || (l2 && ws_env == 2)) return 0;
    if (l2) {
        if (!(l2->mode == CONV_S1 && l2->ks == 1 && l2->epi == EPI_BIAS && l2->cout == l.cout && l2->L_out == 8 && l2->c1 == l.c1 && l2->c2 == l.c2)) return 0;
        if (l.cout == 128 && l.gs == 16 && l.cin_pad == 512) return 3;
        if (l.cout == 256 && l.gs == 32 && l.cin_pad == 128 && l.c2 == 0 && wsp_on && !a.res)
            return 6;
        return 0;
    }
    if (l.cout == 256 && l.gs == 32 && l.cin_pad == 256) return 1;
    if (l.cout == 128 && l.gs == 16 && l.cin_pad == 128 && l.c2 == 0 && wsn_on) return 4;
    return 0;
}


static int run_layer(const mpdx_unet* u, const Layer& l, const float* packed, const float* tt_row, const float* x,
                     float* ws, int B, hipStream_t st, int dbg = 0) {
    if (l.attn) {
        AttnArgs aa;
        memset(&aa, 0, sizeof(aa));
        aa.x = ws + u->slot_floats * (size_t)B * l.dst;
        aa.wqkv = packed + u->params[l.w].off; aa.wout = packed + u->params[l.w2].off; aa.bout = packed + u->params[l.b2].off;
        aa.g = packed + u->params[l.gamma].off; aa.b = packed + u->params[l.beta].off;
        return launch_attention(l, aa, B, st);
    }
    ConvArgs a;
    if (int rc = make_conv_args(u, l, packed, tt_row, x, ws, B, dbg, a)) return rc;
    if (const int v = weight_stationary_variant(l, nullptr, a, B, dbg)) return launch_weight_stationary(v, l, a, a, B, st);
    return launch_conv_layer(l, a, B, st);
}

bool pair_tile(const Layer& l1, const Layer& l2, int B, int& MT, int& NT) {
    if (!sw::pair()) return false;
    if (!(l1.mode == CONV_S1 && l1.ks == 5 && l1.epi == EPI_GN_MISH && l2.mode == CONV_S1 && l2.ks == 1 && l2.epi == EPI_BIAS)) return false;
    if ((l1.gs * l1.L_out != 128 && l1.gs * l1.L_out != 256) || l1.Lv_out) return false;
    if (l1.src1 != l2.src1 || l1.src2 != l2.src2 || l1.cout != l2.cout || l1.L_out != l2.L_out || !layer_ksplit(l1)) return false;
    choose_tile(l1, B, MT, NT);
    if (l1.cout % MT) MT = 16;
    if (l1.cout % MT || NT % l1.L_out) return false;
    const size_t lds = std::max({(size_t)(NT / l1.L_out) * (l1.L_in + 4) * l1.rs * sizeof(float), (size_t)(NT / l2.L_out) * l2.L_in * l2.rs * sizeof(float),
                                 (size_t)8 * NT * (MT + 4) * sizeof(float)});
    return lds <= 160 * 1024;
}

static int run_pair(const mpdx_unet* u, const Layer& l1, const Layer& l2, const float* packed, const float* tt_row, const float* x, float* ws,
                    int B, hipStream_t st) {
    int MT, NT;
    if (!pair_tile(l1, l2, B, MT, NT)) return fail(MPDX_E_STATE, "layers %s / %s do not pair", l1.name.c_str(), l2.name.c_str());
    ConvArgs a1, a2;
    if (int rc = make_conv_args(u, l1, packed, tt_row, x, ws, B, 0, a1)) return rc;
    if (int rc = make_conv_args(u, l2, packed, tt_row, x, ws, B, 0, a2)) return rc;
    if (const int v = weight_stationary_variant(l1, &l2, a1, B, 0)) return launch_weight_stationary(v, l1, a1, a2, B, st);
    a1.n_tiles_n = a2.n_tiles_n = (int)(((long)B * l1.L_out + NT - 1) / NT);
    return launch_conv_pair(MT, NT, a1, a2, l1, l2, st) == 1 ? 0 : fail(MPDX_E_INVALID, "pair launch failed (tile %dx%d)", MT, NT);
}

int check_ready(const mpdx_unet* u) {
    if (u->n_done != (int)u->params.size())
        return fail(MPDX_E_STATE, "%d of %zu parameters packed; call mpdx_unet_pack_param for every state-dict tensor first",
                    u->n_done, u->params.size());
    return 0;
}

unsigned fused_mask(int B) {
    (void)B;
    return sw::fused() ? sw::fused_mask() : 0u;
}
static std::vector<mpdx_unet::Unit> current_units(const mpdx_unet* u, int B, bool* final_in_fused) {
    std::vector<mpdx_unet::Unit> out;
    const unsigned m = fused_mask(B);
    bool fin = false;
    const int nlay = (int)u->layers.size();
    auto fused_on = [&](int i) { const int o = u->owner[i]; return o >= 0 && ((m >> o) & 1u); };
    for (int i = 0; i < nlay; ++i) {
        const int o = u->owner[i];
        if (fused_on(i)) {
            if (i == u->fused[o].first) { out.push_back({mpdx_unet::kProgram, o, i, u->fused[o].count}); fin |= u->fused[o].has_final; }
            continue;
        }
        int MT, NT;
        if (i + 1 < nlay && !fused_on(i + 1) && pair_tile(u->layers[i], u->layers[i + 1], B, MT, NT)) {
            out.push_back({mpdx_unet::kPair, -1, i, 2});
            ++i;
            continue;
        }
        out.push_back({mpdx_unet::kLayer, -1, i, 1});
    }
    if (final_in_fused) *final_in_fused = fin;
    return out;
}

static int run_final(mpdx_unet* u, const float* packed, FinalArgs& fa, int B, float* ws, hipStream_t st) {
    const mpdx_unet_cfg& c = u->cfg;
    fa.h = ws + u->slot_floats * (size_t)B * u->final_slot;
    fa.w = packed + u->params[u->pidx.at("final_conv.1.weight")].off;
    fa.bias = packed + u->params[u->pidx.at("final_conv.1.bias")].off;
    fa.B = B; fa.H = c.n_support_points; fa.D = c.state_dim; fa.C = c.unet_input_dim;
    fa.Hc = u->Hc;
    return launch_final_step(fa, st);
}
int launch_final_step(const FinalArgs& fa, hipStream_t st) {
    const int n = fa.B * fa.H;
    const size_t lds = (size_t)(fa.D * fa.C + fa.D) * sizeof(float);
    hipLaunchKernelGGL(final_step_kernel, dim3((n + 255) / 256), dim3(256), lds, st, fa);
    return 0;
}

static long long* g_fused_trace = nullptr;
static int g_fused_trace_seg = -1;

__global__ __launch_bounds__(256) void restream_all_kernel(float* __restrict__ packed, const CopyJobDev* __restrict__ jobs) {
    restream_job(packed, jobs[blockIdx.y], blockIdx.x * 256u + threadIdx.x, gridDim.x * 256u);
}

static int ensure_stream_jobs(mpdx_unet* u) {
    if (!u->jobs_dev) {
        std::vector<CopyJobDev> all;
        for (const auto& f : u->fused)
            for (const auto& j : f.jobs) all.push_back({(unsigned long long)j.src, (unsigned long long)j.dst, j.n0, j.ss0, j.ds0, j.n1, j.ss1, j.ds1, j.n_inner});
        u->n_jobs = (int)all.size();
        if (u->n_jobs) {
            HIP_TRY(hipMalloc(&u->jobs_dev, all.size() * sizeof(CopyJobDev)));
            HIP_TRY(hipMemcpy(u->jobs_dev, all.data(), all.size() * sizeof(CopyJobDev), hipMemcpyHostToDevice));
        }
    }
    return 0;
}
int ensure_fused_streams(mpdx_unet* u, const float* packed, hipStream_t st) {
    if (u->streams_for == packed && u->streams_version == u->pack_version) return 0;
    if (int rc = ensure_stream_jobs(u)) return rc;
    if (u->n_jobs)
        hipLaunchKernelGGL(restream_all_kernel, dim3(64, (unsigned)u->n_jobs), dim3(256), 0, st, const_cast<float*>(packed), (const CopyJobDev*)u->jobs_dev);
    HIP_TRY(hipGetLastError());
    u->streams_for = packed; u->streams_version = u->pack_version;
    return 0;
}
int claim_fused_stream_jobs(mpdx_unet* u, const float* packed, const void** jobs, int* n) {
    *jobs = nullptr; *n = 0;
    if (u->streams_for == packed && u->streams_version == u->pack_version) return 0;
    if (int rc = ensure_stream_jobs(u)) return rc;
    *jobs = u->jobs_dev; *n = u->n_jobs;
    u->streams_for = packed; u->streams_version = u->pack_version;
    return 0;
}

bool fused_save_variant(const mpdx_unet::Fused& f) { return f.program == 0 || f.program == 3 || f.program == 5 || f.program == 6 || f.program < 0; }
static int fill_fused_args(mpdx_unet* u, const mpdx_unet::Fused& f, const float* packed, const float* tt_row, const float* x, float* ws,
                           int B, const FinalArgs* fa, FusedArgs& a) {
    const size_t slot = u->slot_floats * (size_t)B;
    auto src = [&](int s) -> const float* { return s == SRC_X ? x : (s == SRC_NONE ? nullptr : ws + slot * s); };
    a = f.tmpl;
    a.packed = packed; a.tt_row = tt_row;
    a.gsrc1 = src(f.in1); a.gsrc2 = src(f.in2);
    a.gsrc3 = f.in3 != SRC_NONE ? src(f.in3) : a.gsrc1;
    for (int k = 0; k < 3; ++k) a.gout[k] = f.gout_slot[k] >= 0 ? ws + slot * f.gout_slot[k] : nullptr;
    a.B = B;
    a.trace = (g_fused_trace && (g_fused_trace_seg < 0 || g_fused_trace_seg == (int)(&f - &u->fused[0]))) ? g_fused_trace : nullptr;
    if (f.has_final) {
        if (!fa) return fail(MPDX_E_STATE, "fused final segment needs the step arguments");
        a.x_in = fa->x_in; a.noise = fa->noise; a.hs = fa->hs; a.hg = fa->hg; a.out = fa->out; a.chain = fa->chain;
        a.absmax = fa->absmax; a.fmode = fa->mode; a.n_per_ctx = fa->n_per_ctx > 0 ? fa->n_per_ctx : B; a.k = fa->k;
        a.rng = fa->rng;
    }
    return 0;
}
static int run_fused(mpdx_unet* u, const mpdx_unet::Fused& f, const float* packed, const float* tt_row, const float* x, float* ws,
                     int B, const FinalArgs* fa, hipStream_t st) {
    if (int rc = ensure_fused_streams(u, packed, st)) return rc;
    FusedArgs a;
    if (int rc = fill_fused_args(u, f, packed, tt_row, x, ws, B, fa, a)) return rc;
    return launch_fused_args(f, a, B, st);
}
static int run_fused_join(mpdx_unet* u, const mpdx_unet::Fused& up, const mpdx_unet::Fused& dn, const float* packed, const float* tt_row, const float* tt_next,
                          const float* x, float* ws, int B, const FinalArgs* fa, hipStream_t st, long long* trace = nullptr) {
    if (int rc = ensure_fused_streams(u, packed, st)) return rc;
    FusedJoinArgs ja;
    FusedArgs d;
    if (int rc = fill_fused_args(u, up, packed, tt_row, x, ws, B, fa, ja.up)) return rc;
    if (int rc = fill_fused_args(u, dn, packed, tt_next, x, ws, B, nullptr, d)) return rc;
    ja.up.trace = trace;
    ja.dn.packed = d.packed; ja.dn.tt_row = d.tt_row;
    for (int k = 0; k < 3; ++k) ja.dn.gout[k] = d.gout[k];
    ja.dn.gpar_off = d.gpar_off; ja.dn.tt_lo = d.tt_lo;
    for (int k = 0; k < kMaxFusedOps; ++k) ja.dn.sbase[k] = k < d.nops ? d.ops[k].sbase : 0;
    return launch_fused_join(ja, B, st);
}

static int run_index(int width) { return width == kRunNarrow ? 1 : 0; }
static int inner_run_resident(int cus, int width, int wgs_per_cu) { return cus * std::min(width == kRunNarrow ? 2 : 1, wgs_per_cu); }
static int inner_run_counter_lines(int cus, int width) { return inner_run_resident(cus, width, 2) / 8 + 8; }
static size_t inner_run_counter_bytes(int cus, int width) { return (size_t)inner_run_counter_lines(cus, width) * kInnerRunCounterStride * sizeof(unsigned); }
static int inner_run_create(mpdx_unet::InnerRunState& r, int cus) {
    if (r.capacity >= 0) return 0;
    r.capacity = 0;
    int dev = 0, khz = 0;
    if (cus <= 0 || hipGetDevice(&dev) != hipSuccess || hipDeviceGetAttribute(&khz, hipDeviceAttributeClockRate, dev) != hipSuccess)
        return (void)hipGetLastError(), 0;
    bool any = false;
    for (int width : {kRunWide, kRunNarrow}) {
        r.seven_wgs[run_index(width)] = inner_run_workgroups_per_cu(width);
        r.tail_wgs[run_index(width)] = tail_run_workgroups_per_cu(width);
        any = any || r.seven_wgs[run_index(width)] > 0 || r.tail_wgs[run_index(width)] > 0;
    }
    if (!any) return 0;
    const size_t bytes = inner_run_counter_bytes(cus, kRunWide) + inner_run_counter_bytes(cus, kRunNarrow);
    HIP_TRY(hipMalloc((void**)&r.counters, bytes));
    HIP_TRY(hipMemset(r.counters, 0, bytes));
    r.ctr[0].p = r.counters;
    r.ctr[1].p = r.counters + inner_run_counter_lines(cus, kRunWide) * kInnerRunCounterStride;
    HIP_TRY(hipHostMalloc((void**)&r.status, 64, hipHostMallocMapped));
    *r.status = r.status_host;
    HIP_TRY(hipHostGetDevicePointer((void**)&r.status_dev, r.status, 0));
    r.budget = 4LL * (khz > 0 ? khz : 2400000);
    r.capacity = cus;
    return 0;
}
static int inner_run_begin(mpdx_unet::InnerRunState& r, int width, int nc, int n_layers, hipStream_t st, unsigned** counters_out, unsigned* base_out) {
    mpdx_unet::InnerRunState::Counters& k = r.ctr[run_index(width)];
    if (nc > inner_run_counter_lines(r.capacity, width)) return fail(MPDX_E_STATE, "run of width %d: %d clusters, %d counter lines", width, nc, inner_run_counter_lines(r.capacity, width));
    if (k.rezero || nc > k.live) {
        HIP_TRY(hipMemsetAsync(k.p, 0, inner_run_counter_bytes(r.capacity, width), st));
        k.base = 0; k.rezero = false;
    }
    k.live = nc;
    *counters_out = k.p;
    *base_out = k.base;
    k.base += 8u * (unsigned)n_layers;
    return 0;
}
static void inner_run_free(mpdx_unet::InnerRunState& r) {
    if (r.counters) (void)hipFree(r.counters);
    if (r.status) (void)hipHostFree(r.status);
}
static int handle_status_error(const mpdx_unet* u, const char* fn) {
    const unsigned w = u->run.status_word();
    if (!w) return 0;
    return fail(MPDX_E_DEVICE, "%s: a workgroup of the inner-level run gave up its wait (status 0x%x: layer %u of the run); the outputs of that plan hold NaN. "
                "mpdx_unet_set_status(u, 0) clears the word", fn, w, w >> 8);
}
static long long* g_run_trace = nullptr;
static int g_run_trace_kind = -1;
constexpr int kRunTraceSlots = 32;
template <int N>
static int fill_run_args(mpdx_unet* u, int kind, int first, int width, const float* packed, const float* row, const float* x, float* ws, int B, hipStream_t st, RunArgs<N>& ra) {
    memset(&ra, 0, sizeof(ra));
    if (!inner_run_width_ok(width)) return fail(MPDX_E_STATE, "run unit of width %d", width);
    const int nc = inner_run_clusters(B, width);
    for (int k = 0; k < N; ++k) {
        if (int rc = make_conv_args(u, u->layers[first + k], packed, row, x, ws, B, 0, ra.layer[k])) return rc;
        ra.layer[k].n_tiles_n = nc;
        ra.layer[k].trace = g_run_trace && g_run_trace_kind == kind ? g_run_trace + k * kRunTraceSlots : nullptr;
    }
    ra.n_layers = N; ra.nc = nc;
    if (int rc = inner_run_begin(u->run, width, nc, N, st, &ra.counters, &ra.base)) return rc;
    ra.status = u->run.status_dev; ra.budget = u->run.budget;
    u->inner_run_layers += N;
    return 0;
}
static int run_inner_run(mpdx_unet* u, int first, int width, const float* packed, const float* row, const float* x, float* ws, int B, hipStream_t st) {
    InnerRunArgs ra;
    if (int rc = fill_run_args(u, mpdx_unet::kInnerRun, first, width, packed, row, x, ws, B, st, ra)) return rc;
    u->inner_runs++;
    return launch_inner_run(ra, B, width, st);
}
static int run_tail_run(mpdx_unet* u, int first, int spare, int width, const float* packed, const float* row, const float* x, float* ws, int B, hipStream_t st) {
    TailRunArgs ra;
    if (spare < 0 || spare >= u->n_slots) return fail(MPDX_E_STATE, "tail run without a spare slot");
    if (int rc = fill_run_args(u, mpdx_unet::kTailRun, first, width, packed, row, x, ws, B, st, ra)) return rc;
    float* const sp = ws + u->slot_floats * (size_t)B * spare;
    ra.layer[0].dst = sp; ra.layer[1].src1 = sp; ra.layer[2].res = sp;
    return launch_tail_run(ra, B, width, st);
}

static int run_unit(mpdx_unet* u, const mpdx_unet::Unit& un, const float* packed, const float* row, const float* x, float* ws, int B,
                    const FinalArgs* fa, hipStream_t st) {
    if (un.kind == mpdx_unet::kProgram) return run_fused(u, u->fused[un.fused], packed, row, x, ws, B, fa, st);
    if (un.kind == mpdx_unet::kPair) return run_pair(u, u->layers[un.layer], u->layers[un.layer + 1], packed, row, x, ws, B, st);
    if (un.kind == mpdx_unet::kInnerRun) return run_inner_run(u, un.layer, un.width, packed, row, x, ws, B, st);
    if (un.kind == mpdx_unet::kTailRun) return run_tail_run(u, un.layer, un.fused, un.width, packed, row, x, ws, B, st);
    return run_layer(u, u->layers[un.layer], packed, row, x, ws, B, st);
}
static double unit_flops(const mpdx_unet* u, const mpdx_unet::Unit& un, int B) {
    double fl = 0.0;
    for (int k = un.layer; k < un.layer + un.count; ++k) fl += layer_flops(u->layers[k], B);
    return fl;
}

static double layer_param_bytes(const mpdx_unet* u, const Layer& l) {
    if (l.attn) return 4.0 * ((double)u->params[l.w].n + (double)u->params[l.w2].n + 3.0 * l.cout);
    double n = (double)u->params[l.w].n + l.cout;
    if (l.gamma >= 0) n += 2.0 * l.cout;
    if (l.tb_off >= 0) n += l.cout;
    return 4.0 * n;
}
static double unit_bytes(const mpdx_unet* u, const mpdx_unet::Unit& un, int B) {
    auto act = [&](int L, int C) { return 4.0 * B * (double)L * C; };
    if (un.kind == mpdx_unet::kProgram) {
        const auto& f = u->fused[un.fused];
        const Layer& l0 = u->layers[f.first];
        double b = act(l0.L_in, l0.c1 + l0.c2);
        if (f.in3_consumer >= 0) b += act(u->layers[f.in3_consumer].L_in, u->layers[f.in3_consumer].c2);
        for (int k = f.first; k < f.first + f.count; ++k) b += layer_param_bytes(u, u->layers[k]);
        for (int k = 0; k < f.tmpl.nops; ++k)
            if (f.tmpl.ops[k].shape != kFusedShapeFinal && f.tmpl.ops[k].gdst >= 0) {
                const Layer& l = u->layers[f.op_layer[k]];
                b += act(l.L_out, l.cout);
            }
        if (f.has_final) b += 3.0 * act(u->cfg.n_support_points, u->cfg.state_dim);
        return b;
    }
    double b = 0.0;
    for (int k = un.layer; k < un.layer + un.count; ++k) {
        const Layer& l = u->layers[k];
        b += layer_param_bytes(u, l) + act(l.L_out, l.cout) + (l.res != SRC_NONE ? act(l.L_out, l.cout) : 0.0);
        if (k == un.layer || un.kind != mpdx_unet::kPair) b += act(l.L_in, l.c1 + l.c2);
    }
    return b;
}

enum PassEvent { kSkipUnit, kBeforeLaunch, kAfterLaunch };
static int no_hook(PassEvent, int) { return 0; }
template <class Hook>
static int walk_pass(mpdx_unet* u, const std::vector<mpdx_unet::Unit>& units, const float* packed, const float* row, const float* x, float* ws,
                     int B, FinalArgs& fa, hipStream_t st, Hook&& hook, bool first_done = false, const float* next_row = nullptr,
                     long long* join_trace = nullptr) {
    const int n = (int)units.size();
    bool final_done = false;
    for (int i = first_done ? 1 : 0; i < n; ++i) {
        const mpdx_unet::Unit& un = units[i];
        if (un.kind == mpdx_unet::kProgram) final_done |= u->fused[un.fused].has_final;
        if (hook(kSkipUnit, i)) continue;
        if (int rc = hook(kBeforeLaunch, i)) return rc;
        const int rc = next_row && i == n - 1 ? run_fused_join(u, u->fused[un.fused], u->fused[units[0].fused], packed, row, next_row, x, ws, B, &fa, st, join_trace)
                                              : run_unit(u, un, packed, row, x, ws, B, &fa, st);
        if (rc) return rc;
        if (int rc = hook(kAfterLaunch, i)) return rc;
    }
    if (final_done) return 0;
    if (int rc = hook(kBeforeLaunch, n)) return rc;
    if (int rc = run_final(u, packed, fa, B, ws, st)) return rc;
    return hook(kAfterLaunch, n);
}

static const float* padded_input(const mpdx_unet* u, const float* x, float* ws, int B, hipStream_t st) {
    if (!u->masked()) return x;
    float* xc = ws + u->slot_floats * (size_t)B * u->xpad_slot;
    const size_t nx = (size_t)B * u->Hc * u->cfg.state_dim;
    hipLaunchKernelGGL(pad_input_kernel, dim3((unsigned)std::min<size_t>((nx + 255) / 256, 2048)), dim3(256), 0, st, x, xc, B, u->cfg.n_support_points, u->Hc,
                       u->cfg.state_dim);
    return xc;
}
static int run_unet_and_final(mpdx_unet* u, const float* packed, const float* timetab, int T, const float* x, int t, int B,
                              float* ws, FinalArgs& fa, hipStream_t st) {
    if (int rc = check_ready(u)) return rc;
    if (t < 0 || t >= T) return fail(MPDX_E_INVALID, "timestep %d outside [0,%d)", t, T);
    if (B <= 0) return fail(MPDX_E_INVALID, "B must be positive");
    return walk_pass(u, current_units(u, B, nullptr), packed, timetab + (size_t)t * u->tt_row, padded_input(u, x, ws, B, st), ws, B, fa, st, no_hook);
}

static int inner_run_first(const mpdx_unet* u, const std::vector<mpdx_unet::Unit>& units) {
    auto fits = [&](const mpdx_unet::Unit& un) {
        if (un.kind != mpdx_unet::kLayer) return false;
        const Layer& l = u->layers[un.layer];
        if (l.attn || !(l.mode == CONV_S1 && l.ks == 5 && l.epi == EPI_GN_MISH) || l.Lv_out) return false;
        if (!(l.c1 == 256 && l.c2 == 0 && l.src2 == SRC_NONE && l.cout == 256 && l.L_in == 8 && l.L_out == 8 && l.gs == 32 && l.cin_pad == 256 && l.rs == 264)) return false;
        if ((l.tb_off >= 0) == (l.res != SRC_NONE)) return false;
        return layer_ksplit(l);
    };
    const int n = (int)units.size();
    for (int i = 0; i + kInnerRunLayers <= n; ++i) {
        int k = 0;
        while (k < kInnerRunLayers && fits(units[i + k])) ++k;
        if (k == kInnerRunLayers) return i;
    }
    return -1;
}
static int tail_run_first(const mpdx_unet* u, const std::vector<mpdx_unet::Unit>& units, int* spare) {
    *spare = -1;
    auto layer_of = [&](const mpdx_unet::Unit& un) -> const Layer* {
        if (un.kind != mpdx_unet::kLayer) return nullptr;
        const Layer& l = u->layers[un.layer];
        if (l.attn || l.Lv_out || !(l.c1 == 128 && l.c2 == 0 && l.src2 == SRC_NONE && l.cout == 128 && l.L_in == 8 && l.cin_pad == 128)) return nullptr;
        return &l;
    };
    auto fits_gn = [&](const mpdx_unet::Unit& un) {
        const Layer* l = layer_of(un);
        if (!l || !(l->mode == CONV_S1 && l->ks == 5 && l->epi == EPI_GN_MISH && l->L_out == 8 && l->gs == 16 && l->rs == 136)) return false;
        if ((l->tb_off >= 0) == (l->res != SRC_NONE)) return false;
        return layer_ksplit(*l);
    };
    auto fits_up = [&](const mpdx_unet::Unit& un) {
        const Layer* l = layer_of(un);
        return l && l->mode == CONV_UPT && l->ks == 4 && l->epi == EPI_BIAS && l->L_out == 16 && l->rs == 132 && l->res == SRC_NONE && l->tb_off < 0;
    };
    const int n = (int)units.size();
    for (int i = 0; i + kTailRunLayers <= n; ++i) {
        int k = 0;
        while (k < kTailRunLayers - 1 && fits_gn(units[i + k])) ++k;
        if (!(k == kTailRunLayers - 1 && fits_up(units[i + k]))) continue;
        const int f = units[i].layer;
        const Layer &l0 = u->layers[f], &l1 = u->layers[f + 1], &l2 = u->layers[f + 2], &l3 = u->layers[f + 3];
        if (units[i + 1].layer != f + 1 || units[i + 2].layer != f + 2 || units[i + 3].layer != f + 3) continue;
        if (!(l1.src1 == l0.dst && l2.src1 == l1.dst && l2.res == l0.dst && l3.src1 == l2.dst && l0.res != SRC_NONE && l1.res == SRC_NONE)) continue;
        std::vector<int> kept = {l0.dst, l1.dst, l2.dst};
        auto drop = [&](int s) { kept.erase(std::remove(kept.begin(), kept.end(), s), kept.end()); };
        auto held = [&](int s) { return std::find(kept.begin(), kept.end(), s) != kept.end(); };
        if (l0.dst == l1.dst || l1.dst == l2.dst || l0.dst == l2.dst) continue;
        drop(l3.dst);
        bool read_later = false;
        for (int j = f + kTailRunLayers; j < (int)u->layers.size() && !read_later; ++j) {
            const Layer& l = u->layers[j];
            read_later = held(l.src1) || held(l.src2) || held(l.res);
            drop(l.dst);
        }
        if (read_later || held(u->final_slot)) continue;
        auto named = [&](const Layer& l, int s) { return l.src1 == s || l.src2 == s || l.res == s || l.dst == s; };
        for (int s = 0; s < u->n_slots && *spare < 0; ++s) {
            if (s == u->xpad_slot || named(l0, s) || named(l1, s) || named(l2, s) || named(l3, s)) continue;
            bool dead = s != u->final_slot;
            for (int j = f + kTailRunLayers; j < (int)u->layers.size() && dead; ++j) {
                const Layer& l = u->layers[j];
                if (l.src1 == s || l.src2 == s || l.res == s) dead = false;
                else if (l.dst == s) break;
            }
            if (dead) *spare = s;
        }
        if (*spare < 0 || l3.dst == l1.dst || l3.dst == l2.dst || l3.dst == l0.src1 || l3.dst == l0.res) { *spare = -1; continue; }
        return i;
    }
    return -1;
}
static int device_cus() {
    int dev = 0, cus = 0;
    if (hipGetDevice(&dev) != hipSuccess || hipDeviceGetAttribute(&cus, hipDeviceAttributeMultiprocessorCount, dev) != hipSuccess) (void)hipGetLastError();
    return cus;
}
static int inner_run_auto_width(int B) { return (void)B, kRunNarrow; }
static int tail_run_auto_width(int B) { return B <= 64 ? kRunNarrow : kRunWide; }
struct PlanSchedule {
    std::vector<mpdx_unet::Unit> units;
    bool run = false;
    bool join = false;
    int build(mpdx_unet* u, int B, bool with_run = true) {
        units = current_units(u, B, nullptr);
        const int cus = device_cus();
        if (with_run && u->inner_run && !u->masked() && !u->cfg.self_attention && u->cfg.n_levels == 4 && u->cfg.n_support_points == 64) {
            if (int rc = inner_run_create(u->run, cus)) return rc;
            const bool may = u->run.capacity > 0 && sw::geo() && !sw::debug();
            auto width_of = [&](const int (&wgs)[2], int automatic) {
                auto fits = [&](int w) { return may && inner_run_grid(B, w) <= inner_run_resident(u->run.capacity, w, wgs[run_index(w)]); };
                if (u->inner_run_width) return fits(u->inner_run_width) ? u->inner_run_width : 0;
                return fits(automatic) ? automatic : fits(kRunWide) ? kRunWide : 0;
            };
            const int sw7 = width_of(u->run.seven_wgs, inner_run_auto_width(B)), swt = width_of(u->run.tail_wgs, tail_run_auto_width(B));
            const int rf = sw7 && (u->inner_run & mpdx_unet::kRunSeven) ? inner_run_first(u, units) : -1;
            if (rf >= 0) {
                units[rf] = {mpdx_unet::kInnerRun, -1, units[rf].layer, kInnerRunLayers, sw7};
                units.erase(units.begin() + rf + 1, units.begin() + rf + kInnerRunLayers);
                run = true;
            }
            int spare = -1;
            const int tf = swt && (u->inner_run & mpdx_unet::kRunTail) ? tail_run_first(u, units, &spare) : -1;
            if (tf >= 0) {
                units[tf] = {mpdx_unet::kTailRun, spare, units[tf].layer, kTailRunLayers, swt};
                units.erase(units.begin() + tf + 1, units.begin() + tf + kTailRunLayers);
                run = true;
            }
        }
        if (!u->plan_join || u->masked() || units.size() < 2) return 0;
        const mpdx_unet::Unit &first = units.front(), &last = units.back();
        if (first.kind != mpdx_unet::kProgram || last.kind != mpdx_unet::kProgram || first.fused == last.fused) return 0;
        const mpdx_unet::Fused &dn = u->fused[first.fused], &up = u->fused[last.fused];
        join = dn.program == 5 && dn.in1 == SRC_X && dn.in2 == SRC_NONE && !dn.has_final && up.program == 3 && up.has_final && B <= cus;
        return 0;
    }
};

int dev_hooks_missing(const char* fn) {
#ifdef MPDX_DEV_HOOKS
    return (void)fn, 0;
#endif
    return fail(MPDX_E_STATE, "%s needs a development build of libmpdx.so (MPDX_BUILD_DEFS=-DMPDX_DEV_HOOKS MPDX_BUILD_OUT=build_ab/libmpdx_dev.so python -m mpd_public_amd.build, then MPDX_LIB=build_ab/libmpdx_dev.so): "
                "the production kernels carry no trace / ablation hooks", fn);
}

}

using namespace mpdx;

#include "unet_measure.hpp"

extern "C" {

const char* mpdx_last_error(void) { return g_err; }
int mpdx_version(void) { return 1; }

int mpdx_unet_create(const mpdx_unet_cfg* cfg, mpdx_unet** out) {
    if (!cfg || !out) return fail(MPDX_E_INVALID, "null argument");
    if (cfg->n_levels < 2 || cfg->n_levels > MPDX_MAX_LEVELS) return fail(MPDX_E_INVALID, "n_levels %d unsupported", cfg->n_levels);
    if (cfg->state_dim < 1 || cfg->state_dim > 64) return fail(MPDX_E_INVALID, "state_dim %d unsupported", cfg->state_dim);
    if (cfg->time_emb_dim != 32) return fail(MPDX_E_INVALID, "time_emb_dim must be 32 (TimeEncoder(32, .), temporal_unet.py:66)");
    if (cfg->unet_input_dim % 16) return fail(MPDX_E_INVALID, "unet_input_dim must be a multiple of 16");
    if (cfg->self_attention != 0 && cfg->self_attention != 1) return fail(MPDX_E_INVALID, "self_attention must be 0 or 1");
    if (cfg->dim_mults[0] != 1) return fail(MPDX_E_INVALID, "dim_mults[0] must be 1: final_conv takes unet_input_dim channels (temporal_unet.py:113-116)");
    for (int i = 0; i < cfg->n_levels; ++i)
        if (cfg->dim_mults[i] < 1) return fail(MPDX_E_INVALID, "dim_mults[%d] = %d", i, cfg->dim_mults[i]);
    const int H = cfg->n_support_points;
    if (H < 16 || H > 128 || (H % (1 << (cfg->n_levels - 1))) || (H >> (cfg->n_levels - 1)) < 2)
        return fail(MPDX_E_INVALID, "n_support_points %d must be a multiple of 2^(levels-1) = %d in [16, 128] with >= 2 points at the coarsest level", H,
                    1 << (cfg->n_levels - 1));
    mpdx_unet* u = new mpdx_unet();
    u->cfg = *cfg;
    build_model(u);
    for (const Layer& l : u->layers)
        if (l.epi == EPI_GN_MISH) {
            const int re = l.gs * l.L_out;
            if (re < 64 || re > 2048 || (re & (re - 1)) || l.gs < 4 || 32 % l.gs) {
                std::string nm = l.name;
                delete u;
                return fail(MPDX_E_INVALID, "layer %s: GroupNorm region of %d elements (group of %d) unsupported", nm.c_str(), re, l.gs);
            }
        }
    for (const Layer& l : u->layers)
        if (l.attn)
            if (const char* why = attn_unsupported(l.cout, l.L_out)) {
                const std::string nm = l.name;
                const int ch = l.cout, np = l.L_out;
                delete u;
                return fail(MPDX_E_INVALID, "self-attention block %s (%d channels on %d positions): %s", nm.c_str(), ch, np, why);
            }
    if ((int)u->tt_w.size() > 40) { delete u; return fail(MPDX_E_INVALID, "too many residual blocks"); }
    build_units(u);
    u->packed_floats += 64;
    *out = u;
    return 0;
}

int mpdx_unet_set_plan_join(mpdx_unet* u, int on) {
    if (!u) return fail(MPDX_E_INVALID, "null argument");
    u->plan_join = on ? 1 : 0;
    return 0;
}
int mpdx_unet_plan_joined(const mpdx_unet* u) { return u ? u->plan_joined : 0; }

int mpdx_unet_set_inner_run(mpdx_unet* u, int on) {
    if (!u) return fail(MPDX_E_INVALID, "null argument");
    u->inner_run = on ? (mpdx_unet::kRunSeven | mpdx_unet::kRunTail) : 0;
    return 0;
}
int mpdx_unet_set_inner_run_parts(mpdx_unet* u, int parts) {
    if (!u) return fail(MPDX_E_INVALID, "null argument");
    if (parts & ~(mpdx_unet::kRunSeven | mpdx_unet::kRunTail)) return fail(MPDX_E_INVALID, "inner-run parts 0x%x: bit 0 the seven 256 -> 256 layers, bit 1 the tail of up level 0", parts);
    u->inner_run = parts;
    return 0;
}
int mpdx_unet_set_inner_run_width(mpdx_unet* u, int width) {
    if (!u) return fail(MPDX_E_INVALID, "null argument");
    if (width != 0 && !inner_run_width_ok(width)) return fail(MPDX_E_INVALID, "inner-run width %d: 0 (automatic), 16 or 32 positions per cluster", width);
    u->inner_run_width = width;
    return 0;
}
int mpdx_inner_run_block(int B, int width, int cus, int block, int32_t* cluster, int32_t* tile, int32_t* counter_lines) {
    if (B <= 0 || cus <= 0 || !inner_run_width_ok(width)) return fail(MPDX_E_INVALID, "mpdx_inner_run_block: B=%d width=%d cus=%d", B, width, cus);
    const int grid = inner_run_grid(B, width);
    if (block < 0 || block >= grid) return fail(MPDX_E_INVALID, "mpdx_inner_run_block: block %d of %d", block, grid);
    int c = 0, m = 0;
    inner_run_slot(block, &c, &m);
    if (cluster) *cluster = c < inner_run_clusters(B, width) ? c : -1;
    if (tile) *tile = m;
    if (counter_lines) *counter_lines = inner_run_counter_lines(cus, width);
    return grid;
}
int mpdx_unet_inner_runs(const mpdx_unet* u) { return u ? u->inner_runs : 0; }
int mpdx_unet_inner_run_layers(const mpdx_unet* u) { return u ? u->inner_run_layers : 0; }
int mpdx_unet_status(const mpdx_unet* u) {
    if (!u) return fail(MPDX_E_INVALID, "null argument");
    return handle_status_error(u, "mpdx_unet_status");
}
int mpdx_unet_set_status(mpdx_unet* u, unsigned word) {
    if (!u) return fail(MPDX_E_INVALID, "null argument");
    if (u->run.status) __atomic_store_n(u->run.status, word, __ATOMIC_RELAXED);
    u->run.status_host = word;
    if (!word && u->run.counters) u->run.ctr[0].rezero = u->run.ctr[1].rezero = true;
    return 0;
}

void mpdx_unet_destroy(mpdx_unet* u) {
    if (u && u->pack_descs_dev) (void)hipFree(u->pack_descs_dev);
    if (u && u->pack_chunks_dev) (void)hipFree(u->pack_chunks_dev);
    if (u && u->jobs_dev) (void)hipFree(u->jobs_dev);
    if (u) inner_run_free(u->run);
    delete u;
}

int mpdx_unet_num_params(const mpdx_unet* u) { return u ? (int)u->params.size() : 0; }

int mpdx_unet_param_info(const mpdx_unet* u, int idx, const char** name, int32_t shape[3], int32_t* ndim) {
    if (!u || idx < 0 || idx >= (int)u->params.size()) return fail(MPDX_E_INVALID, "bad parameter index %d", idx);
    const Param& p = u->params[idx];
    if (name) *name = p.name.c_str();
    if (shape) { shape[0] = p.shape[0]; shape[1] = p.shape[1]; shape[2] = p.shape[2]; }
    if (ndim) *ndim = p.ndim;
    return 0;
}

size_t mpdx_unet_packed_floats(const mpdx_unet* u) { return u ? u->packed_floats : 0; }
size_t mpdx_unet_timetab_floats(const mpdx_unet* u, int T) { return u ? (size_t)T * u->tt_row : 0; }
size_t mpdx_unet_workspace_floats(const mpdx_unet* u, int B) { return u ? u->slot_floats * (size_t)B * u->n_slots : 0; }

int mpdx_unet_pack_param(mpdx_unet* u, const char* name, const float* src, size_t n, float* packed, void* stream) {
    if (!u || !name || !src || !packed) return fail(MPDX_E_INVALID, "null argument");
    auto it = u->pidx.find(name);
    if (it == u->pidx.end()) return fail(MPDX_E_NOTFOUND, "unexpected state-dict key '%s'", name);
    Param& p = u->params[it->second];
    if (n != p.n) return fail(MPDX_E_INVALID, "'%s': got %zu floats, expected %zu", name, n, p.n);
    hipStream_t st = (hipStream_t)stream;
    if (p.kind == PK_VEC) {
        hipLaunchKernelGGL(copy_kernel, dim3((unsigned)std::min<size_t>((p.n + 255) / 256, 1024)), dim3(256), 0, st, src, packed + p.off, p.n);
    } else {
        hipLaunchKernelGGL(pack_conv_weights_kernel, dim3((unsigned)std::min<size_t>((p.pn + 255) / 256, 2048)), dim3(256), 0, st, src,
                           packed + p.off, p.cout, p.cin, p.ksz, p.cin_pad, p.nslot, p.kind == PK_CONVT ? 1 : 0);
    }
    HIP_TRY(hipGetLastError());
    if (!p.done) { p.done = true; u->n_done++; }
    u->pack_version++;
    return 0;
}

int mpdx_unet_build_timetab(mpdx_unet* u, const float* packed, const float* freqs16, int T, float* timetab, void* stream) {
    if (!u || !packed || !freqs16 || !timetab || T <= 0) return fail(MPDX_E_INVALID, "bad argument");
    if (int rc = check_ready(u)) return rc;
    TimeTabArgs a;
    memset(&a, 0, sizeof(a));
    a.packed = packed; a.freqs = freqs16; a.tab = timetab;
    a.w1 = (int)u->params[u->pidx.at("time_mlp.encoder.1.weight")].off;
    a.b1 = (int)u->params[u->pidx.at("time_mlp.encoder.1.bias")].off;
    a.w2 = (int)u->params[u->pidx.at("time_mlp.encoder.3.weight")].off;
    a.b2 = (int)u->params[u->pidx.at("time_mlp.encoder.3.bias")].off;
    a.row = u->tt_row;
    a.nblk = (int)u->tt_w.size();
    for (int i = 0; i < a.nblk; ++i) {
        a.woff[i] = (int)u->params[u->tt_w[i]].off;
        a.boff[i] = (int)u->params[u->tt_b[i]].off;
        a.cout[i] = u->tt_cout[i];
        a.toff[i] = u->tt_off[i];
    }
    hipLaunchKernelGGL(timetab_kernel, dim3(T), dim3(128), 0, (hipStream_t)stream, a);
    HIP_TRY(hipGetLastError());
    return 0;
}

int mpdx_unet_forward(mpdx_unet* u, const float* packed, const float* timetab, int T, const float* x, int t, float* eps,
                      int B, float* ws, void* stream) {
    if (!u || !packed || !timetab || !x || !eps || !ws) return fail(MPDX_E_INVALID, "null argument");
    hipStream_t st = (hipStream_t)stream;
    FinalArgs fa;
    memset(&fa, 0, sizeof(fa));
    fa.out = eps; fa.mode = 0; fa.n_per_ctx = 1;
    if (int rc = run_unet_and_final(u, packed, timetab, T, x, t, B, ws, fa, st)) return rc;
    HIP_TRY(hipGetLastError());
    return 0;
}

int mpdx_ddpm_step(mpdx_unet* u, const float* packed, const float* timetab, int T, float* x_io, const float* noise,
                   const float* hard_start, const float* hard_goal, const mpdx_step_coefs* coefs, int t, int mean_only,
                   float* chain_out, uint32_t* absmax_out, int n_per_ctx, int B, float* ws, void* stream) {
    if (!u || !packed || !timetab || !x_io || !coefs || !ws) return fail(MPDX_E_INVALID, "null argument");
    hipStream_t st = (hipStream_t)stream;
    FinalArgs fa;
    memset(&fa, 0, sizeof(fa));
    fa.x_in = x_io; fa.out = x_io; fa.noise = noise; fa.hs = hard_start; fa.hg = hard_goal;
    fa.chain = chain_out; fa.absmax = absmax_out; fa.n_per_ctx = n_per_ctx > 0 ? n_per_ctx : B;
    fa.mode = mean_only == 2 ? 3 : (mean_only ? 2 : 1);
    fa.k = *coefs;
    if (int rc = run_unet_and_final(u, packed, timetab, T, x_io, t, B, ws, fa, st)) return rc;
    HIP_TRY(hipGetLastError());
    return 0;
}

int mpdx_add_noise(float* x_io, const float* noise, const float* hard_start, const float* hard_goal, float noise_scale,
                   float noise_std_extra, float* chain_out, int B, int H, int D, void* stream) {
    if (!x_io || B <= 0) return fail(MPDX_E_INVALID, "bad argument");
    const size_t n = (size_t)B * H * D;
    hipLaunchKernelGGL(add_noise_kernel, dim3((unsigned)std::min<size_t>((n + 255) / 256, 2048)), dim3(256), 0, (hipStream_t)stream,
                       x_io, noise, hard_start, hard_goal, noise_scale, noise_std_extra, chain_out, B, H, D);
    HIP_TRY(hipGetLastError());
    return 0;
}

int mpdx_hard_conds(float* x_io, float* chain_out, int n, const int32_t* horizon_idx, const float* const* values, int B, int H, int D, void* stream) {
    if (!x_io || B <= 0 || H <= 0 || D <= 0 || n < 0 || (n && (!horizon_idx || !values))) return fail(MPDX_E_INVALID, "bad argument");
    if (n > kMaxHardConds) return fail(MPDX_E_INVALID, "at most 16 hard conditions per call");
    if (n == 0) return 0;
    HardCondArgs a;
    memset(&a, 0, sizeof(a));
    a.n = n;
    for (int k = 0; k < n; ++k) {
        int t = horizon_idx[k];
        if (t < 0) t += H;
        if (t < 0 || t >= H) return fail(MPDX_E_INVALID, "hard condition index out of range for this horizon");
        if (!values[k]) return fail(MPDX_E_INVALID, "null hard condition table");
        a.idx[k] = t; a.vals[k] = values[k];
    }
    const size_t per = (size_t)B * D;
    hipLaunchKernelGGL(hard_conds_kernel, dim3((unsigned)std::min<size_t>((per + 255) / 256, 1024)), dim3(256), 0, (hipStream_t)stream, x_io, chain_out, a, B, H, D);
    HIP_TRY(hipGetLastError());
    return 0;
}

int mpdx_q_sample(const float* x_start, const float* noise, const long long* t_dev, const float* sqrt_alphas_cumprod_dev,
                  const float* sqrt_one_minus_alphas_cumprod_dev, const float* hard_start, const float* hard_goal, float* out, int B, int H,
                  int D, int T, void* stream) {
    if (!x_start || !noise || !t_dev || !sqrt_alphas_cumprod_dev || !sqrt_one_minus_alphas_cumprod_dev || !out || B <= 0 || T <= 0)
        return fail(MPDX_E_INVALID, "bad argument");
    const size_t n = (size_t)B * H * D;
    hipLaunchKernelGGL(q_sample_kernel, dim3((unsigned)std::min<size_t>((n + 255) / 256, 2048)), dim3(256), 0, (hipStream_t)stream, x_start, noise,
                       t_dev, sqrt_alphas_cumprod_dev, sqrt_one_minus_alphas_cumprod_dev, hard_start, hard_goal, out, B, H, D, T);
    HIP_TRY(hipGetLastError());
    return 0;
}

int mpdx_weighted_loss(const float* pred, const float* targ, const float* weights_hd, const float* hard_start, const float* hard_goal,
                       int l1, float* out1, int B, int H, int D, void* stream) {
    if (!pred || !targ || !out1 || B <= 0) return fail(MPDX_E_INVALID, "bad argument");
    hipLaunchKernelGGL(weighted_loss_kernel, dim3(1), dim3(1024), 0, (hipStream_t)stream, pred, targ, weights_hd, hard_start, hard_goal, l1, out1,
                       B, H, D);
    HIP_TRY(hipGetLastError());
    return 0;
}

int mpdx_plan(mpdx_unet* u, const float* packed, const float* timetab, int T, const mpdx_step_coefs* coefs, int n_without_noise,
              float* x, const float* noise, const float* hard_start, const float* hard_goal, float* chain, int B, float* ws,
              const mpdx_guide_params* guide, int n_guide_steps, int t_start_guide, uint32_t* guide_flags, int n_per_ctx,
              uint64_t rng_seed, uint64_t rng_offset, void* stream) {
    if (!u || !packed || !timetab || !coefs || !x || !ws || T <= 0 || n_without_noise < 0 || B <= 0)
        return fail(MPDX_E_INVALID, "bad argument");
    if (int rc = handle_status_error(u, "mpdx_plan")) return rc;
    if (guide)
        if (const char* why = scene_params_problem(*guide)) return fail(MPDX_E_INVALID, "%s", why);
    if (guide)
        if (const char* why = chain_params_problem(*guide)) return fail(MPDX_E_INVALID, "%s", why);
    if (guide)
        if (const char* why = tool_params_problem(*guide)) return fail(MPDX_E_INVALID, "%s", why);
    if (int rc = check_ready(u)) return rc;
    PlanSchedule ps;
    if (int rc = ps.build(u, B)) return rc;
    u->inner_runs = u->inner_run_layers = u->plan_joined = 0;
    hipStream_t st = (hipStream_t)stream;
    const int H = u->cfg.n_support_points, D = u->cfg.state_dim;
    const size_t n = (size_t)B * H * D;
    const int npc = n_per_ctx > 0 ? n_per_ctx : B;
    const int n_ctx = (B + npc - 1) / npc;
    const int steps = T + n_without_noise;
    if (n_guide_steps < 0) return fail(MPDX_E_INVALID, "n_guide_steps %d", n_guide_steps);
    if (n_guide_steps == 0) guide = nullptr;
    const int dbg = sw::debug();
    if (guide) {
        if (!guide_flags) return fail(MPDX_E_INVALID, "guide needs guide_flags");
        if (B % npc) return fail(MPDX_E_INVALID, "B=%d is not a multiple of n_per_ctx=%d", B, npc);
        HIP_TRY(hipMemsetAsync(guide_flags, 0, (size_t)steps * (n_guide_steps + 1) * n_ctx * sizeof(uint32_t), st));
    }
    hipLaunchKernelGGL(add_noise_kernel, dim3((unsigned)std::min<size_t>((n + 255) / 256, 2048)), dim3(256), 0, st, x, (const float*)nullptr,
                       hard_start, hard_goal, 0.f, 0.f, chain, B, H, D);
    bool down_done = false;
    int k = 0;
    for (int i = T - 1; i >= -n_without_noise; --i, ++k) {
        const int t = i < 0 ? 0 : i;
        const bool guided = guide && i < t_start_guide;
        const bool join = ps.join && !guided && i > -n_without_noise;
        const float* tt_next = join ? timetab + (size_t)(i - 1 < 0 ? 0 : i - 1) * u->tt_row : nullptr;
        const float* nz = (t == 0 || !noise) ? nullptr : noise + (size_t)k * n;
        NoiseRng rng;
        memset(&rng, 0, sizeof(rng));
        if (!noise && t != 0) { rng.on = 1; rng.seed = rng_seed; rng.offset = rng_offset; rng.elem0 = (unsigned long long)(k + 1) * n; }
        float* ch = chain ? chain + (size_t)(k + 1) * n : nullptr;
        uint32_t* fl = guided ? guide_flags + (size_t)k * (n_guide_steps + 1) * n_ctx : nullptr;
        FinalArgs fa;
        memset(&fa, 0, sizeof(fa));
        fa.x_in = x; fa.out = x;
        fa.k = coefs[t];
        fa.n_per_ctx = npc;
        if (!guided) {
            fa.rng = rng; fa.noise = nz; fa.hs = hard_start; fa.hg = hard_goal;
            fa.chain = ch; fa.mode = 1;
        } else {
            fa.mode = 2; fa.absmax = fl;
        }
        if (int rc = walk_pass(u, ps.units, packed, timetab + (size_t)t * u->tt_row, padded_input(u, x, ws, B, st), ws, B, fa, st, no_hook, down_done, tt_next))
            return rc;
        down_done = join;
        u->plan_joined += join ? 1 : 0;
        if (guided) {
            for (int j = 0; j < n_guide_steps; ++j) {
                const bool last = j == n_guide_steps - 1;
                if (int rc = launch_guide(guide, x, nullptr, hard_start, hard_goal, fl + (size_t)j * n_ctx, fl + (size_t)(j + 1) * n_ctx, npc, B, H,
                                          D, st, last ? nz : nullptr, coefs[t].noise_scale, coefs[t].noise_std_extra, last ? ch : nullptr,
                                          coefs[t].guide_scale, last ? &rng : nullptr))
                    return rc;
            }
        }
        if (dbg) {
            if (dbg >= 2) {
                const hipError_t e = hipStreamSynchronize(st);
                if (e != hipSuccess) return fail((int)e, "mpdx_plan: loop iteration %d (t=%d%s) faulted: %s", k, t, guided ? ", guided" : "", hipGetErrorString(e));
            }
            hipError_t e = hipGetLastError();
            if (e != hipSuccess) return fail((int)e, "mpdx_plan: launch in loop iteration %d (t=%d%s) failed: %s", k, t, guided ? ", guided" : "", hipGetErrorString(e));
        }
    }
    HIP_TRY(hipGetLastError());
    return ps.run ? handle_status_error(u, "mpdx_plan") : 0;
}

int mpdx_randn(float* out, size_t n, uint64_t seed, uint64_t offset, void* stream) {
    if (!out) return fail(MPDX_E_INVALID, "null argument");
    if (n == 0) return 0;
    const size_t nquad = (n + 3) / 4;
    hipLaunchKernelGGL(randn_kernel, dim3((unsigned)std::min<size_t>((nquad + 255) / 256, 4096)), dim3(256), 0, (hipStream_t)stream, out, n,
                       seed, offset);
    HIP_TRY(hipGetLastError());
    return 0;
}

int mpdx_attention_block(float* x, const float* to_qkv_w, const float* to_out_w, const float* to_out_b, const float* norm_g, const float* norm_b,
                         int B, int L, int Lv, int C, void* stream) {
    if (!x || !to_qkv_w || !to_out_w || !to_out_b || !norm_g || !norm_b) return fail(MPDX_E_INVALID, "null argument");
    if (B <= 0) return fail(MPDX_E_INVALID, "batch must be positive");
    if (const char* why = attn_unsupported(C, L)) return fail(MPDX_E_INVALID, "self-attention block (%d channels on %d positions): %s", C, L, why);
    if (Lv < 1 || Lv > L) return fail(MPDX_E_INVALID, "valid positions must be in [1, %d]", L);
    hipStream_t st = (hipStream_t)stream;
    Layer l;
    l.name = "mpdx_attention_block"; l.attn = true; l.mode = CONV_S1; l.ks = 0; l.epi = EPI_BIAS;
    l.c1 = C; l.cout = C; l.L_in = L; l.L_out = L;
    l.Lv_out = Lv != L ? Lv : 0;
    l.cin_pad = pad_cin(C);
    l.rs = pick_row_stride(l.cin_pad, CONV_S1, L, L, L);
    const int hid_pad = pad_cin(kAttnHid);
    const size_t n_qkv = (size_t)(3 * kAttnHid / 16) * (l.cin_pad / 16) * 256, n_out = (size_t)(C / 16) * (hid_pad / 16) * 256;
    float* packed = nullptr;
    HIP_TRY(hipMalloc(&packed, (n_qkv + n_out) * sizeof(float)));
    hipLaunchKernelGGL(pack_conv_weights_kernel, dim3((unsigned)std::min<size_t>((n_qkv + 255) / 256, 2048)), dim3(256), 0, st, to_qkv_w, packed,
                       3 * kAttnHid, C, 1, l.cin_pad, 1, 0);
    hipLaunchKernelGGL(pack_conv_weights_kernel, dim3((unsigned)std::min<size_t>((n_out + 255) / 256, 2048)), dim3(256), 0, st, to_out_w, packed + n_qkv,
                       C, kAttnHid, 1, hid_pad, 1, 0);
    AttnArgs aa;
    memset(&aa, 0, sizeof(aa));
    aa.x = x; aa.wqkv = packed; aa.wout = packed + n_qkv; aa.bout = to_out_b; aa.g = norm_g; aa.b = norm_b;
    int rc = launch_attention(l, aa, B, st);
    hipError_t e = hipGetLastError();
    const hipError_t es = hipStreamSynchronize(st);
    if (e == hipSuccess) e = es;
    (void)hipFree(packed);
    if (rc) return rc;
    if (e != hipSuccess) return fail((int)e, "mpdx_attention_block: %s", hipGetErrorString(e));
    return 0;
}

}
```

mpd_public_amd/csrc/unet_measure.hpp:

```cpp
#pragma once
#include "host.hpp"

namespace mpdx {

struct __attribute__((visibility("hidden"))) Events {
    std::vector<hipEvent_t> ev;
    int create(int n) { ev.assign(n, nullptr); for (hipEvent_t& e : ev) HIP_TRY(hipEventCreate(&e)); return 0; }
    hipEvent_t operator[](int i) const { return ev[i]; }
    ~Events() { for (hipEvent_t e : ev) if (e) (void)hipEventDestroy(e); }
};
struct __attribute__((visibility("hidden"))) DevStamps {
    long long* p = nullptr;
    int alloc(size_t n, hipStream_t st) { HIP_TRY(hipMalloc(&p, n * sizeof(long long))); HIP_TRY(hipMemsetAsync(p, 0, n * sizeof(long long), st)); return 0; }
    ~DevStamps() { if (p) (void)hipFree(p); }
};
struct __attribute__((visibility("hidden"))) CapturedGraph {
    hipStream_t capturing = nullptr; hipGraph_t graph = nullptr; hipGraphExec_t exec = nullptr;
    ~CapturedGraph() {
        if (capturing) (void)hipStreamEndCapture(capturing, &graph);
        if (exec) (void)hipGraphExecDestroy(exec);
        if (graph) (void)hipGraphDestroy(graph);
    }
};
template <class T>
struct ResetOnExit { T& ref; T value; ~ResetOnExit() { ref = value; } };

static int eps_sink(const mpdx_unet* u, int B, FinalArgs& fa) {
    static float* scratch = nullptr;
    static size_t scratch_n = 0;
    const size_t need = (size_t)B * u->cfg.n_support_points * u->cfg.state_dim;
    if (scratch_n < need) {
        if (scratch) { (void)hipFree(scratch); scratch = nullptr; scratch_n = 0; }
        HIP_TRY(hipMalloc(&scratch, need * sizeof(float)));
        scratch_n = need;
    }
    memset(&fa, 0, sizeof(fa));
    fa.out = scratch; fa.mode = 0; fa.n_per_ctx = 1;
    return 0;
}

struct __attribute__((visibility("hidden"))) MeasuredPass {
    std::vector<mpdx_unet::Unit> units; bool final_in_fused = false;
    FinalArgs fa; const float* row = nullptr;
    int prepare(mpdx_unet* u, const float* timetab, int T, int t, int B) {
        if (int rc = check_ready(u)) return rc;
        if (t < 0 || t >= T) return fail(MPDX_E_INVALID, "timestep %d outside [0,%d)", t, T);
        units = current_units(u, B, &final_in_fused);
        row = timetab + (size_t)t * u->tt_row;
        return eps_sink(u, B, fa);
    }
};

static std::string fused_unit_name(const mpdx_unet* u, const mpdx_unet::Fused& f) {
    const std::string& first = u->layers[f.first].name;
    return "fused[" + first.substr(0, first.find(".blocks")) + "..+" + std::to_string(f.count) + (f.has_final ? " layers+final_conv.1+ddpm_step]" : " layers]");
}

static bool unit_at(const mpdx_unet* u, int B, int i, mpdx_unet::Unit& un) {
    if (!u) return false;
    const auto units = current_units(u, B, nullptr);
    if (i < 0 || i >= (int)units.size()) return false;
    un = units[i];
    return true;
}

}

extern "C" {

int mpdx_unet_profile(mpdx_unet* u, const float* packed, const float* timetab, int T, const float* x, int t, int B, float* ws,
                      void* stream, int cap, float* ms_out, double* flops_out, const char** names_out, int* n_out) {
    if (!u || !packed || !timetab || !x || !ws || !ms_out || !n_out) return fail(MPDX_E_INVALID, "null argument");
    hipStream_t st = (hipStream_t)stream;
    MeasuredPass p;
    if (int rc = p.prepare(u, timetab, T, t, B)) return rc;
    const int nu = (int)p.units.size(), nl = nu + (p.final_in_fused ? 0 : 1);
    if (cap < nl) return fail(MPDX_E_INVALID, "need room for %d launches", nl);
    static std::vector<std::string> fused_names;
    fused_names.resize(u->fused.size());
    for (int i = 0; i < nl; ++i) {
        const char* name = "final_conv.1+ddpm_step";
        if (i < nu && p.units[i].kind == mpdx_unet::kProgram) name = (fused_names[p.units[i].fused] = fused_unit_name(u, u->fused[p.units[i].fused])).c_str();
        else if (i < nu) name = u->layers[p.units[i].layer].name.c_str();
        if (names_out) names_out[i] = name;
        if (flops_out) flops_out[i] = i < nu ? unit_flops(u, p.units[i], B) : 0.0;
    }
    Events ev;
    if (int rc = ev.create(2 * nl)) return rc;
    auto bracket = [&](PassEvent e, int i) -> int {
        if (e != kSkipUnit) HIP_TRY(hipEventRecord(ev[2 * i + (e == kAfterLaunch ? 1 : 0)], st));
        return 0;
    };
    if (int rc = walk_pass(u, p.units, packed, p.row, x, ws, B, p.fa, st, bracket)) return rc;
    HIP_TRY(hipStreamSynchronize(st));
    for (int i = 0; i < nl; ++i) HIP_TRY(hipEventElapsedTime(&ms_out[i], ev[2 * i], ev[2 * i + 1]));
    *n_out = nl;
    return 0;
}

int mpdx_layer_trace(mpdx_unet* u, const float* packed, const float* timetab, const float* x, int layer, int B, float* ws, void* stream,
                     long long* stamps32) {
    if (int rc = dev_hooks_missing(__func__)) return rc;
    if (!u || layer < 0 || layer >= (int)u->layers.size() || !stamps32) return fail(MPDX_E_INVALID, "bad argument");
    if (int rc = check_ready(u)) return rc;
    hipStream_t st = (hipStream_t)stream;
    DevStamps dev;
    if (int rc = dev.alloc(32, st)) return rc;
    ResetOnExit<long long*> untrace{g_conv_trace, nullptr};
    g_conv_trace = dev.p;
    if (int rc = run_layer(u, u->layers[layer], packed, timetab, x, ws, B, st)) return rc;
    HIP_TRY(hipStreamSynchronize(st));
    HIP_TRY(hipMemcpy(stamps32, dev.p, 32 * sizeof(long long), hipMemcpyDeviceToHost));
    return 0;
}

int mpdx_fused_trace(mpdx_unet* u, const float* packed, const float* timetab, const float* x, int seg, int B, float* ws, void* stream,
                     long long* stamps_out, int cap, int* n_out, int* nops_out) {
    if (int rc = dev_hooks_missing(__func__)) return rc;
    if (!u || seg < 0 || seg > (int)u->fused.size() + 2) return fail(MPDX_E_INVALID, "bad segment");
    if (B <= 0) return fail(MPDX_E_INVALID, "B must be positive");
    const int nseg = (int)u->fused.size();
    const bool joined = seg == nseg;
    const int run_kind = seg == nseg + 1 ? (int)mpdx_unet::kInnerRun : seg == nseg + 2 ? (int)mpdx_unet::kTailRun : -1;
    PlanSchedule ps;
    if (int rc = ps.build(u, B, run_kind >= 0)) return rc;
    if (joined && !ps.join) return fail(MPDX_E_INVALID, "bad segment (this network / batch has no joined launch)");
    int run_layers = 0;
    for (const auto& un : ps.units)
        if ((int)un.kind == run_kind) run_layers = un.count;
    if (run_kind >= 0 && !run_layers) return fail(MPDX_E_INVALID, "bad segment (this network / batch / handle setting does not select that run)");
    if (int rc = check_ready(u)) return rc;
    hipStream_t st = (hipStream_t)stream;
    DevStamps dev;
    if (int rc = dev.alloc(1024, st)) return rc;
    FinalArgs fa;
    if (int rc = eps_sink(u, B, fa)) return rc;
    ResetOnExit<long long*> untrace{g_fused_trace, nullptr};
    ResetOnExit<int> unselect{g_fused_trace_seg, -1};
    ResetOnExit<long long*> untrace_run{g_run_trace, nullptr};
    ResetOnExit<int> unselect_run{g_run_trace_kind, -1};
    for (int pass = 0; pass < 3; ++pass) {
        if (pass == 2 && run_kind >= 0) { g_run_trace = dev.p; g_run_trace_kind = run_kind; }
        else if (pass == 2 && !joined) { g_fused_trace = dev.p; g_fused_trace_seg = seg; }
        const float* next_row = pass == 2 && joined ? timetab : nullptr;
        if (int rc = walk_pass(u, ps.units, packed, timetab, padded_input(u, x, ws, B, st), ws, B, fa, st, no_hook, false, next_row, dev.p)) return rc;
    }
    HIP_TRY(hipStreamSynchronize(st));
    const int n = std::min(cap, 1024);
    HIP_TRY(hipMemcpy(stamps_out, dev.p, n * sizeof(long long), hipMemcpyDeviceToHost));
    if (n_out) *n_out = n;
    if (nops_out) {
        if (run_kind >= 0) *nops_out = run_layers;
        else if (joined) *nops_out =u->fused[ps.units.back().fused].tmpl.nops + u->fused[ps.units.front().fused].tmpl.nops;
        else *nops_out = u->fused[seg].tmpl.nops;
    }
    return 0;
}

int mpdx_unet_time_units(mpdx_unet* u, const float* packed, const float* timetab, int T, const float* x, int t, int B, float* ws,
                         void* stream, int unit_first, int unit_last, int reps, float* ms_avg) {
    if (!u || !packed || !timetab || !x || !ws || !ms_avg || reps < 1) return fail(MPDX_E_INVALID, "bad argument");
    hipStream_t st = (hipStream_t)stream;
    MeasuredPass p;
    if (int rc = p.prepare(u, timetab, T, t, B)) return rc;
    if (unit_first < 0 || unit_last >= (int)p.units.size() || unit_first > unit_last) return fail(MPDX_E_INVALID, "bad unit range");
    Events ev;
    if (int rc = ev.create(2 * reps)) return rc;
    int r = 0;
    auto bracket = [&](PassEvent e, int i) -> int {
        if (e == kBeforeLaunch && i == unit_first) HIP_TRY(hipEventRecord(ev[2 * r], st));
        if (e == kAfterLaunch && i == unit_last) HIP_TRY(hipEventRecord(ev[2 * r + 1], st));
        return 0;
    };
    for (r = 0; r < reps; ++r)
        if (int rc = walk_pass(u, p.units, packed, p.row, x, ws, B, p.fa, st, bracket)) return rc;
    HIP_TRY(hipStreamSynchronize(st));
    double tot = 0.0;
    for (r = 0; r < reps; ++r) { float ms = 0.f; HIP_TRY(hipEventElapsedTime(&ms, ev[2 * r], ev[2 * r + 1])); tot += ms; }
    *ms_avg = (float)(tot / reps);
    return 0;
}

int mpdx_unet_time_without(mpdx_unet* u, const float* packed, const float* timetab, int T, const float* x, int t, int B, float* ws,
                           void* stream, unsigned long long skip_mask, int reps, float* ms_avg) {
    if (!u || !packed || !timetab || !x || !ws || !ms_avg || reps < 1) return fail(MPDX_E_INVALID, "bad argument");
    hipStream_t st = (hipStream_t)stream;
    MeasuredPass p;
    if (int rc = p.prepare(u, timetab, T, t, B)) return rc;
    if (p.units.size() > 64) return fail(MPDX_E_INVALID, "more than 64 launch units");
    Events ev;
    if (int rc = ev.create(2)) return rc;
    auto without = [&](PassEvent e, int i) -> int { return e == kSkipUnit && ((skip_mask >> i) & 1ull); };
    for (int r = 0; r < 3; ++r)
        if (int rc = walk_pass(u, p.units, packed, p.row, x, ws, B, p.fa, st, without)) return rc;
    HIP_TRY(hipEventRecord(ev[0], st));
    for (int r = 0; r < reps; ++r)
        if (int rc = walk_pass(u, p.units, packed, p.row, x, ws, B, p.fa, st, without)) return rc;
    HIP_TRY(hipEventRecord(ev[1], st));
    HIP_TRY(hipStreamSynchronize(st));
    float ms = 0.f;
    HIP_TRY(hipEventElapsedTime(&ms, ev[0], ev[1]));
    *ms_avg = ms / (float)reps;
    return 0;
}

int mpdx_unet_unit_layer(const mpdx_unet* u, int B, int i) {
    mpdx_unet::Unit un;
    return (unit_at(u, B, i, un) && un.kind != mpdx_unet::kProgram) ? un.layer : -1;
}

int mpdx_unet_fused_program(const mpdx_unet* u, int seg) {
    if (!u || seg < 0 || seg >= (int)u->fused.size()) return -2;
    return u->fused[seg].program;
}

double mpdx_unet_unit_bytes(const mpdx_unet* u, int B, int i) {
    mpdx_unet::Unit un;
    return unit_at(u, B, i, un) ? unit_bytes(u, un, B) : 0.0;
}

int mpdx_unet_unit_is_pair(const mpdx_unet* u, int B, int i) {
    mpdx_unet::Unit un;
    return (unit_at(u, B, i, un) && un.kind == mpdx_unet::kPair) ? 1 : 0;
}

int mpdx_bench_layer(mpdx_unet* u, const float* packed, const float* timetab, const float* x, int layer, int B, float* ws,
                     void* stream, int reps, int dbg, float* ms_per_launch) {
    if (!u || !packed || !timetab || !x || !ws || !ms_per_launch) return fail(MPDX_E_INVALID, "null argument");
    if (int rc = check_ready(u)) return rc;
    if (layer < 0 || layer >= (int)u->layers.size()) return fail(MPDX_E_INVALID, "bad layer index");
#ifndef MPDX_DEV_HOOKS
    if (dbg & 15) return fail(MPDX_E_STATE, "phase-ablation masks need a development build of libmpdx.so (MPDX_BUILD_DEFS=-DMPDX_DEV_HOOKS)");
#endif
    hipStream_t st = (hipStream_t)stream;
    const Layer& l = u->layers[layer];
    Events ev;
    if (int rc = ev.create(2)) return rc;
    for (int i = 0; i < 5; ++i)
        if (int rc = run_layer(u, l, packed, timetab, x, ws, B, st, dbg & 15)) return rc;
    CapturedGraph g;
    if (dbg & 16) {
        HIP_TRY(hipStreamBeginCapture(st, hipStreamCaptureModeThreadLocal));
        g.capturing = st;
        for (int i = 0; i < reps; ++i)
            if (int rc = run_layer(u, l, packed, timetab, x, ws, B, st, dbg & 15)) return rc;
        g.capturing = nullptr;
        HIP_TRY(hipStreamEndCapture(st, &g.graph));
        HIP_TRY(hipGraphInstantiate(&g.exec, g.graph, nullptr, nullptr, 0));
        HIP_TRY(hipGraphLaunch(g.exec, st));
        HIP_TRY(hipStreamSynchronize(st));
        HIP_TRY(hipEventRecord(ev[0], st));
        HIP_TRY(hipGraphLaunch(g.exec, st));
        HIP_TRY(hipEventRecord(ev[1], st));
    } else {
        HIP_TRY(hipEventRecord(ev[0], st));
        for (int i = 0; i < reps; ++i)
            if (int rc = run_layer(u, l, packed, timetab, x, ws, B, st, dbg)) return rc;
        HIP_TRY(hipEventRecord(ev[1], st));
    }
    HIP_TRY(hipStreamSynchronize(st));
    float ms = 0.f;
    HIP_TRY(hipEventElapsedTime(&ms, ev[0], ev[1]));
    *ms_per_launch = ms / reps;
    return 0;
}

int mpdx_unet_layer_tile(const mpdx_unet* u, int i, int B, char* buf, size_t buflen) {
    if (!u || !buf || i < 0 || i >= (int)u->layers.size()) return fail(MPDX_E_INVALID, "bad layer index");
    const Layer& l = u->layers[i];
    if (l.attn) { snprintf(buf, buflen, "attn %dx%d", attn_cols(l.cout, l.L_out) / l.L_out, l.L_out); return 0; }
    int MT, NT;
    ConvArgs dummy;
    memset(&dummy, 0, sizeof(dummy));
    const Layer* l2 = (i + 1 < (int)u->layers.size() && pair_tile(l, u->layers[i + 1], B, MT, NT)) ? &u->layers[i + 1] : nullptr;
    if (const int v = weight_stationary_variant(l, l2, dummy, B, 0)) {
        if (v == 6) snprintf(buf, buflen, "wsp 32x16/2x1+1x1");
        else if (v >= 4) snprintf(buf, buflen, "wsn 16x16/8x1");
        else snprintf(buf, buflen, "ws %dx16/1x8%s", v == 1 ? 32 : 16, v == 3 ? "+1x1" : "");
        return 0;
    }
    choose_tile(l, B, MT, NT);
    if (l.cout % MT) MT = 16;
    const bool ks = layer_ksplit(l);
    snprintf(buf, buflen, "%dx%d/%dx%d", MT, NT, ks ? 1 : NT / 16, ks ? 8 : 8 / (NT / 16));
    return 0;
}

}
```

mpd_public_amd/temporal_unet.py:

```python
from __future__ import annotations

import ctypes as C
import math

import torch
import torch.nn as nn

from . import _lib

UNET_DIM_MULTS = {0: (1, 2, 4), 1: (1, 2, 4, 8)}


def group_norm_n_groups(n_channels, target_n_groups=8):
    if n_channels < target_n_groups:
        return 1
    for n_groups in range(target_n_groups, target_n_groups + 10):
        if n_channels % n_groups == 0:
            return n_groups
    return 1


class _Holder(nn.Module):

    def forward(self, *a, **k):
        raise RuntimeError("parameter holder - TemporalUnet.forward runs libmpdx kernels, not torch modules")


def _seq_with(**at):
    n = max(int(k) for k in at) + 1
    return nn.Sequential(*[at.get(str(i), nn.Identity()) for i in range(n)])


def _conv_block(cin, cout, k=5):
    m = _Holder()
    m.block = _seq_with(**{"0": nn.Conv1d(cin, cout, k, padding=k // 2), "2": nn.GroupNorm(group_norm_n_groups(cout), cout), "4": nn.Identity()})
    return m


def _res_block(cin, cout, cond_dim):
    m = _Holder()
    m.blocks = nn.ModuleList([_conv_block(cin, cout), _conv_block(cout, cout)])
    m.cond_mlp = _seq_with(**{"1": nn.Linear(cond_dim, cout), "2": nn.Identity()})
    m.residual_conv = nn.Conv1d(cin, cout, 1) if cin != cout else nn.Identity()
    return m


SELF_ATTENTION_TRAINING_REFUSAL = ("self-attention network: the training pass has no backward for the self-attention blocks "
                                   "(self_attention=True runs inference and evaluation only)")


class _LayerNormHolder(_Holder):
    def __init__(self, dim):
        super().__init__()
        self.g = nn.Parameter(torch.ones(1, dim, 1))
        self.b = nn.Parameter(torch.zeros(1, dim, 1))


def _self_attention(dim, heads=4, dim_head=32):
    hidden = heads * dim_head
    res, pre, att = _Holder(), _Holder(), _Holder()
    att.to_qkv = nn.Conv1d(dim, hidden * 3, 1, bias=False)
    att.to_out = nn.Conv1d(hidden, dim, 1)
    pre.fn = att
    pre.norm = _LayerNormHolder(dim)
    res.fn = pre
    return res


def _resample(dim, up):
    m = _Holder()
    m.conv = nn.ConvTranspose1d(dim, dim, 4, 2, 1) if up else nn.Conv1d(dim, dim, 3, 2, 1)
    return m


class TemporalUnet(nn.Module):
    def __init__(self, n_support_points=None, state_dim=None, unet_input_dim=32, dim_mults=(1, 2, 4, 8), time_emb_dim=32,
                 self_attention=False, conditioning_embed_dim=4, conditioning_type=None, attention_num_heads=2,
                 attention_dim_head=32, **kwargs):
        super().__init__()
        if conditioning_type not in (None, "None"):
            raise NotImplementedError("mpd_public_amd.TemporalUnet: only conditioning_type=None is supported "
                                      "(the only configuration the reference scripts build)")
        self.self_attention = bool(self_attention)
        attn = (lambda dim: _self_attention(dim)) if self.self_attention else (lambda dim: nn.Identity())
        self.state_dim = state_dim
        self.conditioning_type = None
        self.n_support_points = n_support_points
        self.unet_input_dim = unet_input_dim
        self.dim_mults = tuple(int(m) for m in dim_mults)
        self.time_emb_dim = time_emb_dim

        dims = [state_dim] + [unet_input_dim * m for m in self.dim_mults]
        in_out = list(zip(dims[:-1], dims[1:]))
        n_res = len(in_out)

        self.time_mlp = _Holder()
        self.time_mlp.encoder = _seq_with(**{"1": nn.Linear(32, 32 * 4), "3": nn.Linear(32 * 4, time_emb_dim)})
        self.downs = nn.ModuleList()
        for i, (ci, co) in enumerate(in_out):
            last = i >= n_res - 1
            self.downs.append(nn.ModuleList([_res_block(ci, co, time_emb_dim), _res_block(co, co, time_emb_dim), attn(co),
                                             nn.Identity(), _resample(co, up=False) if not last else nn.Identity()]))
        self.ups = nn.ModuleList()
        for ci, co in reversed(in_out[1:]):
            self.ups.append(nn.ModuleList([_res_block(co * 2, ci, time_emb_dim), _res_block(ci, ci, time_emb_dim), attn(ci),
                                           nn.Identity(), _resample(ci, up=True)]))
        mid = dims[-1]
        self.mid_block1 = _res_block(mid, mid, time_emb_dim)
        self.mid_attn = attn(mid)
        self.mid_attention = nn.Identity()
        self.mid_block2 = _res_block(mid, mid, time_emb_dim)
        self.final_conv = nn.Sequential(_conv_block(unet_input_dim, unet_input_dim), nn.Conv1d(unet_input_dim, state_dim, 1))

        self._h = None
        self._packed = None
        self._timetab = None
        self._timetab_T = 0
        self._ws = None
        self._ws_B = 0
        self._stamp = None
        try:
            self._handle()
        except _lib.LibraryUnavailable:
            pass

    _DEVICE_STATE = {"_h": None, "_packed": None, "_timetab": None, "_timetab_T": 0, "_ws": None, "_ws_B": 0, "_stamp": None}

    def __getstate__(self):
        state = dict(self.__dict__)
        state.update(self._DEVICE_STATE)
        return state

    def __setstate__(self, state):
        self.__dict__.update(state)
        self.__dict__.update(self._DEVICE_STATE)

    def __del__(self):
        try:
            if getattr(self, "_h", None):
                _lib.load().mpdx_unet_destroy(self._h)
        except Exception:
            pass

    def _handle(self):
        if self._h is None:
            lib = _lib.load()
            mults = (C.c_int32 * _lib.MAX_LEVELS)(*self.dim_mults)
            cfg = _lib.UnetCfg(int(self.state_dim), int(self.n_support_points), int(self.unet_input_dim), len(self.dim_mults),
                               mults, int(self.time_emb_dim), int(self.self_attention))
            h = C.c_void_p()
            _lib.check(lib.mpdx_unet_create(C.byref(cfg), C.byref(h)), "mpdx_unet_create")
            self._h = h
        return self._h

    def set_plan_join(self, on: bool):
        _lib.check(_lib.load().mpdx_unet_set_plan_join(self._handle(), int(bool(on))), "mpdx_unet_set_plan_join")

    def plan_joined(self) -> int:
        return int(_lib.load().mpdx_unet_plan_joined(self._handle()))

    def set_inner_run(self, on: bool):
        _lib.check(_lib.load().mpdx_unet_set_inner_run(self._handle(), int(bool(on))), "mpdx_unet_set_inner_run")

    RUN_SEVEN, RUN_TAIL = 1, 2

    def set_inner_run_parts(self, parts: int):
        _lib.check(_lib.load().mpdx_unet_set_inner_run_parts(self._handle(), int(parts)), "mpdx_unet_set_inner_run_parts")

    def set_inner_run_width(self, width: int):
        _lib.check(_lib.load().mpdx_unet_set_inner_run_width(self._handle(), int(width)), "mpdx_unet_set_inner_run_width")

    def inner_runs(self) -> int:
        return int(_lib.load().mpdx_unet_inner_runs(self._handle()))

    def inner_run_layers(self) -> int:
        return int(_lib.load().mpdx_unet_inner_run_layers(self._handle()))

    def status(self) -> int:
        return int(_lib.load().mpdx_unet_status(self._handle()))

    def _param_stamp(self):
        d = self.__dict__
        n = d.get("_stamp_calls", 0) + 1
        d["_stamp_calls"] = n
        pl = d.get("_plist")
        if pl is None or n % 16 == 0:
            pl = d["_plist"] = list(self.parameters())
        return tuple((p.data_ptr(), p._version) for p in pl)

    def _apply(self, fn, *a, **k):
        self.__dict__["_plist"] = None
        return super()._apply(fn, *a, **k)

    def load_state_dict(self, *a, **k):
        r = super().load_state_dict(*a, **k)
        self.__dict__["_plist"] = None
        return r

    def engine(self, T: int, B: int):
        lib, h = _lib.load(), self._handle()
        dev = next(self.parameters()).device
        if dev.type != "cuda":
            raise RuntimeError("mpd_public_amd.TemporalUnet runs on an AMD GPU only (move the model to 'cuda'); there is no CPU fallback")
        st = _lib.current_stream()
        frozen = self.__dict__.get("_weights_frozen", False) and self._packed is not None and self._stamp is not None
        stamp = self._stamp if frozen else self._param_stamp()
        if self._packed is None or self._stamp != stamp or self._packed.device != dev:
            packed = torch.zeros(lib.mpdx_unet_packed_floats(h), dtype=torch.float32, device=dev)
            sd = self.state_dict()
            n = lib.mpdx_unet_num_params(h)
            if n != len(sd):
                raise RuntimeError(f"state dict has {len(sd)} tensors, libmpdx expects {n}")
            for name, t in sd.items():
                t = t.detach().to(device=dev, dtype=torch.float32).contiguous()
                _lib.check(lib.mpdx_unet_pack_param(h, name.encode(), t.data_ptr(), t.numel(), packed.data_ptr(), st), f"pack {name}")
            self._packed, self._stamp, self._timetab, self._timetab_T = packed, stamp, None, 0
        if self._timetab is None or self._timetab_T < T:
            T_tab = max(int(T), 128)
            tab = torch.empty(lib.mpdx_unet_timetab_floats(h, T_tab), dtype=torch.float32, device=dev)
            half = 16
            freqs = torch.exp(torch.arange(half) * -(math.log(10000) / (half - 1))).to(device=dev, dtype=torch.float32)
            _lib.check(lib.mpdx_unet_build_timetab(h, self._packed.data_ptr(), freqs.data_ptr(), T_tab, tab.data_ptr(), st), "timetab")
            torch.cuda.current_stream().synchronize()
            self._timetab, self._timetab_T = tab, T_tab
        if self._ws is None or self._ws_B < B or self._ws.device != dev:
            self._ws = torch.empty(lib.mpdx_unet_workspace_floats(h, B), dtype=torch.float32, device=dev)
            self._ws_B = B
        return h, self._packed, self._timetab, self._ws

    def forward(self, x, time, context=None):
        if context is not None:
            raise NotImplementedError("context conditioning is not supported (context is always None on this path, inference.py:182)")
        b, h, d = x.shape
        if h != self.n_support_points or d != self.state_dim:
            raise ValueError(f"expected [B,{self.n_support_points},{self.state_dim}], got {tuple(x.shape)}")
        x = x.to(torch.float32).contiguous()
        from .diffusion_model import timestep_hint
        hint = timestep_hint(time)
        tl = [hint] * int(time.numel()) if hint is not None and time.numel() in (1, b) else time.reshape(-1).tolist()
        if len(tl) not in (1, b):
            raise ValueError(f"time must have 1 or {b} entries, got {len(tl)}")
        out = torch.empty_like(x)
        lib = _lib.load()

        def run(xg, t0, og):
            hdl, packed, tab, ws = self.engine(t0 + 1, xg.shape[0])
            _lib.check(lib.mpdx_unet_forward(hdl, packed.data_ptr(), tab.data_ptr(), self._timetab_T, xg.data_ptr(), t0,
                                             og.data_ptr(), xg.shape[0], ws.data_ptr(), _lib.current_stream()), "mpdx_unet_forward")

        distinct = sorted(set(int(v) for v in tl))
        if len(distinct) == 1:
            run(x, distinct[0], out)
            return out
        self.engine(distinct[-1] + 1, b)
        tt = torch.as_tensor(tl, device=x.device)
        for t0 in distinct:
            idx = (tt == t0).nonzero(as_tuple=True)[0]
            xg = x.index_select(0, idx).contiguous()
            og = torch.empty_like(xg)
            run(xg, t0, og)
            out.index_copy_(0, idx, og)
        return out
```

Measured before the change: 6480 denoising-steps/s.

## Split the deepest fused U-Net level across two blocks per trajectory

Adds a level-split mode to the joined up/down fused kernel. From op 10 onward, each trajectory's 128-channel ops are computed by two workgroups, each producing half the output rows. The halves are swapped after every op through a global exchange buffer, guarded by per-trajectory atomic counters with a timed poll, and a poisoned fallback writes NaNs and sets a status word if the partner block never arrives. The aim is to cut the serial latency of the deep level by doubling the CUs per trajectory. In exchange it adds inter-block spin synchronisation, global round-trips for each exchange, and a dependency on both blocks of a pair being co-resident.

```diff
diff --git a/include/mpdx.h b/include/mpdx.h
--- a/include/mpdx.h
+++ b/include/mpdx.h
@@ -34,6 +34,9 @@
 void   mpdx_unet_destroy(mpdx_unet* u);
 int    mpdx_unet_set_plan_join(mpdx_unet* u, int on);
 int    mpdx_unet_plan_joined(const mpdx_unet* u);
+int    mpdx_unet_set_level_split(mpdx_unet* u, int on);
+int    mpdx_unet_plan_split(const mpdx_unet* u);
+int    mpdx_level_split_block(int B, int block, int32_t* trajectory, int32_t* role);
 int    mpdx_unet_set_inner_run(mpdx_unet* u, int on);
 int    mpdx_unet_set_inner_run_parts(mpdx_unet* u, int parts);
 int    mpdx_unet_set_inner_run_width(mpdx_unet* u, int width);
diff --git a/mpd_public_amd/_lib.py b/mpd_public_amd/_lib.py
--- a/mpd_public_amd/_lib.py
+++ b/mpd_public_amd/_lib.py
@@ -82,6 +82,9 @@
     "mpdx_unet_destroy": (None, [_vp]),
     "mpdx_unet_set_plan_join": (_i, [_vp, _i]),
     "mpdx_unet_plan_joined": (_i, [_vp]),
+    "mpdx_unet_set_level_split": (_i, [_vp, _i]),
+    "mpdx_unet_plan_split": (_i, [_vp]),
+    "mpdx_level_split_block": (_i, [_i, _i, _vp, _vp]),
     "mpdx_unet_set_inner_run": (_i, [_vp, _i]),
     "mpdx_unet_set_inner_run_parts": (_i, [_vp, _i]),
     "mpdx_unet_set_inner_run_width": (_i, [_vp, _i]),
diff --git a/mpd_public_amd/csrc/fused_level.hpp b/mpd_public_amd/csrc/fused_level.hpp
--- a/mpd_public_amd/csrc/fused_level.hpp
+++ b/mpd_public_amd/csrc/fused_level.hpp
@@ -1,6 +1,7 @@
 #pragma once
 #include "conv_block.hpp"
 #include "fused_geom.hpp"
+#include "inner_run.hpp"
 
 namespace mpdx {
 
@@ -40,6 +41,7 @@
     static constexpr int GS = COUT / 8;
     static constexpr int RB = GS / 4;
     static constexpr int NPARTS = NSn * RB;
+    static constexpr bool kSplit = false;
     static_assert(T == 4 || T == 8, "4 or 8 tiles");
     static_assert(MSn == 2 || MSn == 4 || MSn == 8, "2, 4 or 8 tile rows");
     static_assert(MP == 1 || (MODE != CONV_UPT && NSn == 1), "M-passes: one position tile");
@@ -47,6 +49,16 @@
     static_assert(MODE != CONV_UPT || NCR == 0, "no folded residual on resampling ops");
     static_assert(!GN || NPARTS == 2 || NPARTS == 4, "GroupNorm region of 128 or 256 elements");
     static_assert(LOUT >= 16 || !GN, "half-used tiles: resampling ops only");
+};
+
+template <class S>
+struct FusedHalfShape {
+    static constexpr int MODE = S::MODE, KS = S::KS, NC16 = S::NC16, NCR = S::NCR, COUT = S::COUT, LOUT = S::LOUT, GN = S::GN;
+    static constexpr int NTAP = S::NTAP, NBLK = S::NBLK, TOT = S::TOT, MSn = S::MSn, MSW = S::MSW, NSn = S::NSn;
+    static constexpr int MP = 1, T = kFusedWaves, NTW = 1, NSEQ = 1, NJ = 1, SLEN = TOT;
+    static constexpr int GS = S::GS, RB = S::RB, NPARTS = S::NPARTS;
+    static constexpr bool kSplit = true;
+    static_assert(S::MP == 2 && S::NSn == 1 && S::MSW == kFusedWaves && S::MODE != CONV_UPT && S::GS == 16, "half rows: 8 tile rows on one position tile, one group per row");
 };
 
 struct FusedOp {
@@ -180,9 +192,41 @@
     return v;
 }
 
-template <class S, bool SAVE = false, class A = FusedArgs>
-__device__ __forceinline__ void fused_conv_op(const A& a, const FusedLay& lay, const FusedOp& op, f32x4 (&ring)[kFusedRing], float* smem, int wave, int lane, int b,
-                                              int nbase, int nmax, long long* tr_base, int& tr) {
+struct FusedSplitCtx {
+    int role = 0;
+    unsigned* counter = nullptr;
+    unsigned target = 0;
+    long long budget = 0;
+    const float* xsrc = nullptr;
+};
+constexpr int kSplitHalfFloats = kFusedWaves * 16 * 16;
+
+__device__ __forceinline__ bool fused_split_poll(const FusedSplitCtx& sx, int* flag, int wave, int lane) {
+    if (wave == 0) {
+        const long long t0 = (long long)__builtin_amdgcn_s_memtime();
+        int ok;
+        for (;;) {
+            const unsigned v = __hip_atomic_load(sx.counter, __ATOMIC_RELAXED, __HIP_MEMORY_SCOPE_AGENT);
+            const int d = (int)(v - sx.target);
+            if (d >= 0) { ok = (unsigned)d < kRunPoisonSeen; break; }
+            if ((long long)__builtin_amdgcn_s_memtime() - t0 > sx.budget) { ok = 0; break; }
+            __builtin_amdgcn_s_sleep(1);
+        }
+        if (lane == 0) *flag = ok;
+    }
+    __syncthreads();
+    return *flag != 0;
+}
+__device__ __forceinline__ void fused_split_load(const float* xsrc, f32x4* sm4, int dst_off4, int dst_rs4, int col4, int wave, int lane) {
+    const int j = lane & 15, q = lane >> 4;
+    const __amdgpu_buffer_rsrc_t rs = __builtin_amdgcn_make_buffer_rsrc((void*)xsrc, 0, 0x7fffffff, 0x00020000);
+    const f32x4 v = __builtin_bit_cast(f32x4, __builtin_amdgcn_raw_buffer_load_b128(rs, ((wave * 16 + j) * 16 + q * 4) * 4, 0, 16));
+    sm4[dst_off4 + (j + 2) * dst_rs4 + col4 + wave * 4 + q] = v;
+}
+
+template <class S, bool SAVE = false, class A = FusedArgs, bool XOUT = false>
+__device__ __forceinline__ bool fused_conv_op(const A& a, const FusedLay& lay, const FusedOp& op, f32x4 (&ring)[kFusedRing], float* smem, int wave, int lane, int b,
+                                              int nbase, int nmax, long long* tr_base, int& tr, float* xdst = nullptr, const FusedSplitCtx& sx = FusedSplitCtx()) {
     constexpr int P = kFusedRing, DB = MPDX_FUSED_DB, NTW = S::NTW, NJ = S::NJ;
     f32x4* const sm4 = (f32x4*)smem;
     const int j = lane & 15, q = lane >> 4;
@@ -213,7 +257,8 @@
     }
     const int rs4 = op.src_rs4;
     const __amdgpu_buffer_rsrc_t wrs = fused_weights_rsrc(a.packed);
-    const int sbase = (op.sbase + ms * (S::SLEN * 256)) * 4;
+    int sbase = (op.sbase + ms * (S::SLEN * 256)) * 4;
+    if constexpr (S::kSplit) sbase = (op.sbase + (ms * 2 + sx.role) * (S::TOT * 256)) * 4;
     const unsigned lane_bytes = (unsigned)lane * 16u;
     auto read_b = [&](int r, int t) -> f32x4 {
         const int rr = r % S::TOT, par = r / S::TOT;
@@ -265,7 +310,11 @@
     const float* par_op = smem + lay.par_off + op.p_off;
     int c0t[NTW], mst[NTW];
 #pragma unroll
-    for (int t = 0; t < NTW; ++t) { mst[t] = (S::MP > 1) ? ms + t * S::MSW : ms; c0t[t] = mst[t] * 16 + q * 4; }
+    for (int t = 0; t < NTW; ++t) {
+        mst[t] = (S::MP > 1) ? ms + t * S::MSW : ms;
+        if constexpr (S::kSplit) mst[t] = ms + kFusedWaves * sx.role;
+        c0t[t] = mst[t] * 16 + q * 4;
+    }
     f32x4 y[NTW];
     if (S::GN) {
         constexpr bool LOCAL = (S::MSW == kFusedWaves);
@@ -358,6 +407,13 @@
     for (int t = 0; t < NTW; ++t) {
         if (!col_ok) continue;
         if (op.dst_off4 >= 0) sm4[op.dst_off4 + (npos[t] + 2) * op.dst_rs4 + (c0t[t] >> 2)] = y[t];
+        if constexpr (XOUT) {
+            static_assert(NTW == 1 && S::LOUT == 16 && S::NSn == 1 && S::MSW == kFusedWaves, "XOUT: one tile per wave, 16 positions");
+            if (op.dst_off4 >= 0) {
+                const __amdgpu_buffer_rsrc_t xrs = __builtin_amdgcn_make_buffer_rsrc((void*)xdst, 0, 0x7fffffff, 0x00020000);
+                __builtin_amdgcn_raw_buffer_store_b128(__builtin_bit_cast(u32x4, y[t]), xrs, ((ms * 16 + j) * 16 + q * 4) * 4, 0, 16);
+            }
+        }
         if (op.gdst >= 0) *(f32x4*)(a.gout[op.gdst] + ((size_t)b * S::LOUT + npos[t]) * S::COUT + c0t[t]) = y[t];
         if constexpr (SAVE) if (op.save_out >= 0) *(f32x4*)(a.save + op.save_out + ((size_t)b * S::LOUT + npos[t]) * S::COUT + c0t[t]) = y[t];
     }
@@ -371,9 +427,21 @@
     }
     FOP_STAMP();
     __builtin_amdgcn_s_setprio(0);
+    if constexpr (S::kSplit) {
+        if (op.dst_off4 >= 0) {
+            asm volatile("s_waitcnt vmcnt(0) lgkmcnt(0)\n\ts_barrier" ::: "memory");
+            if (wave == 0 && lane == 0) __hip_atomic_fetch_add(sx.counter, 1u, __ATOMIC_RELAXED, __HIP_MEMORY_SCOPE_AGENT);
+            FOP_STAMP();
+            const bool ok = fused_split_poll(sx, (int*)(smem + lay.stat_off), wave, lane);
+            FOP_STAMP();
+            if (!ok) return false;
+            fused_split_load(sx.xsrc, sm4, op.dst_off4, op.dst_rs4, (sx.role ^ 1) * 16, wave, lane);
+        }
+    }
     lds_barrier();
     FOP_STAMP();
 #undef FOP_STAMP
+    return true;
 }
 
 template <class GEOM>
@@ -782,6 +850,98 @@
     }
 }
 
+template <class SD, int I, int END>
+__device__ __forceinline__ void fused_join_down_to(const FusedJoinDown& dn, const FusedLay& lay, f32x4 (&ring)[kFusedRing], float* smem, int wave, int lane, int b,
+                                                   long long* tr_base, int& tr, float* xdst) {
+    static_assert(END < SD::N, "half-row ops follow");
+    if constexpr (I < END) {
+        const FusedOp op = fused_static_desc<typename SD::GEOM, I, false>(dn);
+        int nbase = dn.sbase[I] * 4;
+        int nmax = 0;
+        if constexpr (I + 1 < SD::N) {
+            using N = typename FusedShapeOf<SD::ids[I + 1 < SD::N ? I + 1 : I]>::type;
+            if constexpr (I + 1 == END) {
+                nbase = (dn.sbase[I + 1] + wave * 2 * (N::TOT * 256)) * 4;
+                nmax = N::TOT - 1;
+            } else {
+                nbase = (dn.sbase[I + 1] + (wave & (N::MSn < kFusedWaves ? N::MSn - 1 : kFusedWaves - 1)) * (N::SLEN * 256)) * 4;
+                nmax = N::SLEN - 1;
+            }
+        }
+        fused_conv_op<typename FusedShapeOf<SD::ids[I]>::type, false, FusedJoinDown, I + 1 == END>(dn, lay, op, ring, smem, wave, lane, b, nbase, nmax,
+                                                                                                    tr + 5 <= 128 ? tr_base : nullptr, tr, xdst);
+        fused_join_down_to<SD, I + 1, END>(dn, lay, ring, smem, wave, lane, b, tr_base, tr, xdst);
+    }
+}
+
+template <class SD>
+__device__ __forceinline__ void fused_join_junction(const FusedArgs& a, float* smem, int tid) {
+    f32x4* const sm4 = (f32x4*)smem;
+    {
+        constexpr FusedGeom gd = SD::GEOM::g;
+        const f32x4 z = {0.f, 0.f, 0.f, 0.f};
+        if (tid < 2 * gd.in_rs4) {
+            sm4[gd.in_off4 + tid] = z;
+            sm4[gd.in_off4 + (gd.in_rows - 2) * gd.in_rs4 + tid] = z;
+        }
+        const int D = a.D;
+#pragma unroll
+        for (int k = 0; k < (gd.L0 * gd.in_rs4 + kFusedThreads - 1) / kFusedThreads; ++k) {
+            const int i = tid + k * kFusedThreads;
+            if (i >= gd.L0 * gd.in_rs4) continue;
+            const int l = i / gd.in_rs4, c = (i - l * gd.in_rs4) * 4;
+            const int at = gd.in_off4 + (l + 2) * gd.in_rs4 + (c >> 2);
+            if (c >= D) sm4[at] = z;
+            else if (c + 4 > D) {
+#pragma unroll
+                for (int e = 1; e < 4; ++e)
+                    if (c + e >= D) smem[at * 4 + e] = 0.f;
+            }
+        }
+    }
+}
+
+template <class SU, class SD, int END>
+__device__ __forceinline__ void fused_join_body(const FusedJoinArgs& ja, float* smem, f32x4 (&ring)[kFusedRing], const int b, float* xdst) {
+    using JL = FusedJoinLay<SU, SD>;
+    f32x4* const sm4 = (f32x4*)smem;
+    const FusedArgs& a = ja.up;
+    const FusedJoinDown& dn = ja.dn;
+    const int tid = threadIdx.x, lane = tid & 63;
+    const int wave = __builtin_amdgcn_readfirstlane(tid >> 6);
+    int tr = 0;
+    long long* const tr_base = (MPDX_TRACE_PTR(a.trace) && b == 0 && lane == 0) ? a.trace + wave * 128 : nullptr;
+    if (tr_base) tr_base[tr] = (long long)__builtin_readcyclecounter();
+    ++tr;
+    f32x4 jv[JL::JK];
+#pragma unroll
+    for (int k = 0; k < JL::JK; ++k) {
+        const int idx = tid + k * kFusedThreads;
+        const int it = idx - JL::npar4 < JL::ntt4 ? idx - JL::npar4 : 0;
+        const float* src = idx < JL::npar4 ? dn.packed + dn.gpar_off + (size_t)idx * 4 : dn.tt_row + dn.tt_lo + (size_t)it * 4;
+        jv[k] = *(const f32x4*)src;
+    }
+    __builtin_amdgcn_sched_barrier(0);
+    FinalPre fp;
+    const FusedLay lay = fused_lay<typename SU::GEOM>(a);
+    fused_prologue<typename SU::GEOM>(a, lay, smem, ring, tid, lane, wave, b, tr_base, tr);
+#pragma unroll
+    for (int k = 0; k < JL::JK; ++k) {
+        const int idx = tid + k * kFusedThreads;
+        if (idx < JL::npar4) sm4[(JL::par_off >> 2) + idx] = jv[k];
+        else if (idx - JL::npar4 < JL::ntt4) sm4[(JL::tt_off >> 2) + idx - JL::npar4] = jv[k];
+    }
+    fused_join_up_from<SU, SD, 0>(a, dn, lay, ring, fp, smem, tid, wave, lane, b, tr_base, tr);
+
+    fused_join_junction<SD>(a, smem, tid);
+    lds_barrier();
+    if (tr_base) tr_base[tr] = (long long)__builtin_readcyclecounter();
+    ++tr;
+    FusedLay dlay = {};
+    dlay.stat_off = JL::stat_off; dlay.par_off = JL::par_off; dlay.tt_off = JL::tt_off;
+    fused_join_down_to<SD, 0, END>(dn, dlay, ring, smem, wave, lane, b, tr_base, tr, xdst);
+}
+
 template <class SU, class SD>
 __global__ __launch_bounds__(kFusedThreads) void fused_join_kernel(const FusedJoinArgs ja) {
 #ifndef MPDX_NO_WARM_KERNARG
@@ -819,7 +979,6 @@
         else if (idx - JL::npar4 < JL::ntt4) sm4[(JL::tt_off >> 2) + idx - JL::npar4] = jv[k];
     }
     fused_join_up_from<SU, SD, 0>(a, dn, lay, ring, fp, smem, tid, wave, lane, b, tr_base, tr);
-
     {
         constexpr FusedGeom gd = SD::GEOM::g;
         const f32x4 z = {0.f, 0.f, 0.f, 0.f};
@@ -850,4 +1009,158 @@
     fused_join_down_from<SD, 0>(dn, dlay, ring, smem, wave, lane, b, tr_base, tr);
 }
 
-}
+struct SplitSlot { int b, role; };
+constexpr int split_nb8(int B) { return 8 * ((B + 7) / 8); }
+constexpr int split_grid(int B) { return 2 * split_nb8(B); }
+constexpr int split_block(int b, int role, int nb8) { return b + role * nb8; }
+__host__ __device__ constexpr SplitSlot split_slot(int block, int nb8) { return block < nb8 ? SplitSlot{block, 0} : SplitSlot{block - nb8, 1}; }
+constexpr bool split_map_ok() {
+    for (int B = 1; B <= 128; ++B) {
+        const int nb8 = split_nb8(B), grid = split_grid(B);
+        int live = 0;
+        for (int x = 0; x < grid; ++x) {
+            const SplitSlot s = split_slot(x, nb8);
+            if (s.b < 0 || s.role < 0 || s.role > 1) return false;
+            if (s.b >= B) continue;
+            if (split_block(s.b, s.role, nb8) != x || (x & 7) != (s.b & 7)) return false;
+            ++live;
+        }
+        if (live != 2 * B || nb8 % 8 || nb8 < B) return false;
+    }
+    return true;
+}
+static_assert(split_map_ok(), "block <-> (trajectory, role): a bijection on the live blocks, one XCD per trajectory");
+
+constexpr int kSplitFrom = 10, kSplitSlots = 5;
+constexpr int kSplitTrajFloats = kSplitSlots * 2 * kSplitHalfFloats;
+constexpr unsigned kSplitAdvance = 1 + 2 * (kSplitSlots - 1);
+constexpr int kSplitMaxB = 128;
+struct FusedSplitArgs {
+    float* xch;
+    unsigned* counters;
+    unsigned* status;
+    long long budget;
+    unsigned base;
+    int nb8;
+};
+
+template <class SD, int I>
+__device__ __forceinline__ int fused_split_from(const FusedJoinDown& dn, const FusedSplitArgs& sa, const FusedLay& lay, f32x4 (&ring)[kFusedRing], float* smem, int wave,
+                                                int lane, int b, int role, long long* tr_base, int& tr) {
+    if constexpr (I < SD::N) {
+        using S = FusedHalfShape<typename FusedShapeOf<SD::ids[I]>::type>;
+        static_assert(S::TOT >= kFusedRing, "every ring slot holds a block of this op when it starts");
+        const FusedOp op = fused_static_desc<typename SD::GEOM, I, false>(dn);
+        int nbase = dn.sbase[I] * 4;
+        int nmax = 0;
+        if constexpr (I + 1 < SD::N) {
+            using N = typename FusedShapeOf<SD::ids[I + 1 < SD::N ? I + 1 : I]>::type;
+            nbase = (dn.sbase[I + 1] + (wave * 2 + role) * (N::TOT * 256)) * 4;
+            nmax = N::TOT - 1;
+        }
+        constexpr int slot = I - kSplitFrom + 1;
+        float* const xt = sa.xch + (size_t)b * kSplitTrajFloats + slot * 2 * kSplitHalfFloats;
+        FusedSplitCtx sx;
+        sx.role = role; sx.counter = sa.counters + (size_t)b * kInnerRunCounterStride; sx.target = sa.base + 1u + 2u * (unsigned)slot; sx.budget = sa.budget;
+        sx.xsrc = xt + (role ^ 1) * kSplitHalfFloats;
+        if (!fused_conv_op<S, false, FusedJoinDown, S::LOUT == 16>(dn, lay, op, ring, smem, wave, lane, b, nbase, nmax, tr_base, tr, xt + role * kSplitHalfFloats, sx)) return I;
+        return fused_split_from<SD, I + 1>(dn, sa, lay, ring, smem, wave, lane, b, role, tr_base, tr);
+    } else {
+        return -1;
+    }
+}
+
+template <class SD>
+__device__ __forceinline__ void fused_split_give_up(const FusedJoinDown& dn, const FusedSplitArgs& sa, int b, int role, int at, unsigned target) {
+    const int tid = threadIdx.x;
+    if (tid == 0) {
+        __hip_atomic_fetch_or(sa.status, 1u | ((unsigned)at << 8), __ATOMIC_RELAXED, __HIP_MEMORY_SCOPE_SYSTEM);
+        __hip_atomic_store(sa.counters + (size_t)b * kInnerRunCounterStride, target + kRunPoison, __ATOMIC_RELAXED, __HIP_MEMORY_SCOPE_AGENT);
+    }
+    constexpr FusedGeom gd = SD::GEOM::g;
+    constexpr int g1 = gd.ops[SD::N - 2].gdst, g2 = gd.ops[SD::N - 1].gdst;
+    for (int e = tid; e < 24 * 64; e += kFusedThreads) {
+        const int p = e >> 6, c = role * 64 + (e & 63);
+        if (p < 16) dn.gout[g1][((size_t)b * 16 + p) * 128 + c] = __builtin_nanf("");
+        else dn.gout[g2][((size_t)b * 8 + (p - 16)) * 128 + c] = __builtin_nanf("");
+    }
+}
+
+template <class SU, class SD>
+__global__ __launch_bounds__(kFusedThreads) void fused_join_split_kernel(const FusedJoinArgs ja, const FusedSplitArgs sa) {
+    const SplitSlot slot = split_slot((int)blockIdx.x, sa.nb8);
+    if (slot.b >= ja.up.B) return;
+#ifndef MPDX_NO_WARM_KERNARG
+    warm_kernarg<(int)(sizeof(FusedJoinArgs) + sizeof(FusedSplitArgs))>();
+#endif
+    using JL = FusedJoinLay<SU, SD>;
+    constexpr FusedGeom gd = SD::GEOM::g;
+    constexpr FusedGeomOp g0 = gd.ops[kSplitFrom];
+    using S0 = typename FusedShapeOf<SD::ids[kSplitFrom]>::type;
+    static_assert(SD::N == kSplitFrom + kSplitSlots && gd.ops[kSplitFrom - 1].dst_off4 == g0.src_off4 && S0::NC16 == 4, "the level: the program's last five ops, 64 channels in");
+    static_assert(gd.ops[SD::N - 1].dst_off4 < 0 && gd.ops[SD::N - 2].gdst >= 0 && gd.ops[SD::N - 1].gdst >= 0, "the level's last op leaves through global memory only");
+    extern __shared__ __attribute__((aligned(16))) float smem[];
+    f32x4* const sm4 = (f32x4*)smem;
+    const FusedJoinDown& dn = ja.dn;
+    const int tid = threadIdx.x, lane = tid & 63;
+    const int wave = __builtin_amdgcn_readfirstlane(tid >> 6);
+    const int b = slot.b, role = slot.role;
+    float* const x0 = sa.xch + (size_t)b * kSplitTrajFloats;
+    unsigned* const counter = sa.counters + (size_t)b * kInnerRunCounterStride;
+    FusedLay dlay = {};
+    dlay.stat_off = JL::stat_off; dlay.par_off = JL::par_off; dlay.tt_off = JL::tt_off;
+    int tr = 0;
+    long long* const tr_base = (MPDX_TRACE_PTR(ja.up.trace) && b == 0 && lane == 0) ? ja.up.trace + 512 + (role * kFusedWaves + wave) * 64 : nullptr;
+    f32x4 ring[kFusedRing];
+    if (role == 0) {
+        fused_join_body<SU, SD, kSplitFrom>(ja, smem, ring, b, x0);
+        if (tr_base) tr_base[tr] = (long long)__builtin_readcyclecounter();
+        ++tr;
+        asm volatile("s_waitcnt vmcnt(0)" ::: "memory");
+        __syncthreads();
+        if (tid == 0) __hip_atomic_fetch_add(counter, 1u, __ATOMIC_RELAXED, __HIP_MEMORY_SCOPE_AGENT);
+        if (tr_base) tr_base[tr] = (long long)__builtin_readcyclecounter();
+        ++tr;
+    } else {
+        if (tr_base) tr_base[tr] = (long long)__builtin_readcyclecounter();
+        ++tr;
+        f32x4 jv[JL::JK];
+#pragma unroll
+        for (int k = 0; k < JL::JK; ++k) {
+            const int idx = tid + k * kFusedThreads;
+            const int it = idx - JL::npar4 < JL::ntt4 ? idx - JL::npar4 : 0;
+            const float* src = idx < JL::npar4 ? dn.packed + dn.gpar_off + (size_t)idx * 4 : dn.tt_row + dn.tt_lo + (size_t)it * 4;
+            jv[k] = *(const f32x4*)src;
+        }
+        fused_ring_request(ring, fused_weights_rsrc(dn.packed), (dn.sbase[kSplitFrom] + (wave * 2 + 1) * (S0::TOT * 256)) * 4, S0::TOT, (unsigned)lane * 16u);
+#pragma unroll
+        for (int k = 0; k < JL::JK; ++k) {
+            const int idx = tid + k * kFusedThreads;
+            if (idx < JL::npar4) sm4[(JL::par_off >> 2) + idx] = jv[k];
+            else if (idx - JL::npar4 < JL::ntt4) sm4[(JL::tt_off >> 2) + idx - JL::npar4] = jv[k];
+        }
+        if (tid < 2 * g0.src_rs4) {
+            const f32x4 z = {0.f, 0.f, 0.f, 0.f};
+            sm4[g0.src_off4 + tid] = z;
+            sm4[g0.src_off4 + (16 + 2) * g0.src_rs4 + tid] = z;
+        }
+        FusedSplitCtx sx;
+        sx.counter = counter; sx.target = sa.base + 1u; sx.budget = sa.budget;
+        if (tr_base) tr_base[tr] = (long long)__builtin_readcyclecounter();
+        ++tr;
+        if (!fused_split_poll(sx, (int*)(smem + dlay.stat_off), wave, lane)) {
+            fused_split_give_up<SD>(dn, sa, b, role, kSplitFrom - 1, sx.target);
+            return;
+        }
+        if (tr_base) tr_base[tr] = (long long)__builtin_readcyclecounter();
+        ++tr;
+        fused_split_load(x0, sm4, g0.src_off4, g0.src_rs4, 0, wave, lane);
+        lds_barrier();
+    }
+    if (tr_base) tr_base[tr] = (long long)__builtin_readcyclecounter();
+    ++tr;
+    const int at = fused_split_from<SD, kSplitFrom>(dn, sa, dlay, ring, smem, wave, lane, b, role, tr_base, tr);
+    if (at >= 0) fused_split_give_up<SD>(dn, sa, b, role, at, sa.base + 1u + 2u * (unsigned)(at - kSplitFrom + 1));
+}
+
+}
diff --git a/mpd_public_amd/csrc/host.hpp b/mpd_public_amd/csrc/host.hpp
--- a/mpd_public_amd/csrc/host.hpp
+++ b/mpd_public_amd/csrc/host.hpp
@@ -119,6 +119,17 @@
         unsigned status_host = 0;
         unsigned status_word() const { return status ? __atomic_load_n(status, __ATOMIC_RELAXED) : status_host; }
     } run;
+    int level_split = -1;
+    int plan_split = 0;
+    struct LevelSplitState {
+        int capacity = -1;
+        int wgs = 0;
+        float* xch = nullptr;
+        unsigned* counters = nullptr;
+        unsigned base = 0;
+        int live = 1 << 30;
+        bool rezero = false;
+    } split;
     struct CopyJob { size_t src, dst; int n0, ss0, ds0, n1, ss1, ds1, n_inner; };
     struct Fused {
         int first = 0, count = 0;
@@ -187,6 +198,8 @@
 int launch_fused_train(const mpdx_unet::Fused& f, const FusedArgs& a, int B, hipStream_t st);
 int launch_fused_join(const FusedJoinArgs& ja, int B, hipStream_t st);
 size_t fused_join_lds_bytes();
+int launch_fused_join_split(const FusedJoinArgs& ja, const FusedSplitArgs& sa, int B, hipStream_t st);
+int fused_join_split_workgroups_per_cu();
 struct NoiseRng;
 int launch_guide(const mpdx_guide_params* gp, float* x, float* grad_out, const float* hs, const float* hg, const uint32_t* amax_in,
                  uint32_t* amax_out, int n_per_ctx, int B, int H, int D, hipStream_t st, const float* noise = nullptr, float noise_scale = 0.f,
diff --git a/mpd_public_amd/csrc/k_fused.hip b/mpd_public_amd/csrc/k_fused.hip
--- a/mpd_public_amd/csrc/k_fused.hip
+++ b/mpd_public_amd/csrc/k_fused.hip
@@ -47,4 +47,17 @@
     return 0;
 }
 
+int fused_join_split_workgroups_per_cu() {
+    const void* kern = (const void*)fused_join_split_kernel<FusedSeqUpAB, FusedSeqDown3>;
+    if (raise_lds_limit(kern)) return 0;
+    int n = 0;
+    if (hipOccupancyMaxActiveBlocksPerMultiprocessor(&n, kern, kFusedThreads, fused_join_lds_bytes()) != hipSuccess) return (void)hipGetLastError(), 0;
+    return n;
 }
+int launch_fused_join_split(const FusedJoinArgs& ja, const FusedSplitArgs& sa, int B, hipStream_t st) {
+    if (int rc = raise_lds_limit((const void*)fused_join_split_kernel<FusedSeqUpAB, FusedSeqDown3>)) return rc;
+    hipLaunchKernelGGL((fused_join_split_kernel<FusedSeqUpAB, FusedSeqDown3>), dim3(split_grid(B)), dim3(kFusedThreads), fused_join_lds_bytes(), st, ja, sa);
+    return 0;
+}
+
+}
diff --git a/mpd_public_amd/csrc/mpdx.hip b/mpd_public_amd/csrc/mpdx.hip
--- a/mpd_public_amd/csrc/mpdx.hip
+++ b/mpd_public_amd/csrc/mpdx.hip
@@ -707,21 +707,6 @@
     if (int rc = fill_fused_args(u, f, packed, tt_row, x, ws, B, fa, a)) return rc;
     return launch_fused_args(f, a, B, st);
 }
-static int run_fused_join(mpdx_unet* u, const mpdx_unet::Fused& up, const mpdx_unet::Fused& dn, const float* packed, const float* tt_row, const float* tt_next,
-                          const float* x, float* ws, int B, const FinalArgs* fa, hipStream_t st, long long* trace = nullptr) {
-    if (int rc = ensure_fused_streams(u, packed, st)) return rc;
-    FusedJoinArgs ja;
-    FusedArgs d;
-    if (int rc = fill_fused_args(u, up, packed, tt_row, x, ws, B, fa, ja.up)) return rc;
-    if (int rc = fill_fused_args(u, dn, packed, tt_next, x, ws, B, nullptr, d)) return rc;
-    ja.up.trace = trace;
-    ja.dn.packed = d.packed; ja.dn.tt_row = d.tt_row;
-    for (int k = 0; k < 3; ++k) ja.dn.gout[k] = d.gout[k];
-    ja.dn.gpar_off = d.gpar_off; ja.dn.tt_lo = d.tt_lo;
-    for (int k = 0; k < kMaxFusedOps; ++k) ja.dn.sbase[k] = k < d.nops ? d.ops[k].sbase : 0;
-    return launch_fused_join(ja, B, st);
-}
-
 static int run_index(int width) { return width == kRunNarrow ? 1 : 0; }
 static int inner_run_resident(int cus, int width, int wgs_per_cu) { return cus * std::min(width == kRunNarrow ? 2 : 1, wgs_per_cu); }
 static int inner_run_counter_lines(int cus, int width) { return inner_run_resident(cus, width, 2) / 8 + 8; }
@@ -771,9 +756,58 @@
 static int handle_status_error(const mpdx_unet* u, const char* fn) {
     const unsigned w = u->run.status_word();
     if (!w) return 0;
-    return fail(MPDX_E_DEVICE, "%s: a workgroup of the inner-level run gave up its wait (status 0x%x: layer %u of the run); the outputs of that plan hold NaN. "
-                "mpdx_unet_set_status(u, 0) clears the word", fn, w, w >> 8);
-}
+    return fail(MPDX_E_DEVICE, "%s: a workgroup of an inner-level run or of the paired joined launch gave up its wait (status 0x%x: layer %u of the run, or down op %u of the paired launch); the outputs of that plan hold NaN. "
+                "mpdx_unet_set_status(u, 0) clears the word", fn, w, w >> 8, w >> 8);
+}
+static int level_split_create(mpdx_unet* u, int cus) {
+    mpdx_unet::LevelSplitState& s = u->split;
+    if (s.capacity >= 0) return 0;
+    s.capacity = 0;
+    if (int rc = inner_run_create(u->run, cus)) return rc;
+    if (u->run.capacity <= 0 || !u->run.status_dev) return 0;
+    s.wgs = fused_join_split_workgroups_per_cu();
+    if (s.wgs < 1) return 0;
+    HIP_TRY(hipMalloc((void**)&s.xch, (size_t)kSplitMaxB * kSplitTrajFloats * sizeof(float)));
+    HIP_TRY(hipMalloc((void**)&s.counters, (size_t)kSplitMaxB * kInnerRunCounterStride * sizeof(unsigned)));
+    HIP_TRY(hipMemset(s.counters, 0, (size_t)kSplitMaxB * kInnerRunCounterStride * sizeof(unsigned)));
+    s.capacity = cus;
+    return 0;
+}
+static void level_split_free(mpdx_unet::LevelSplitState& s) {
+    if (s.xch) (void)hipFree(s.xch);
+    if (s.counters) (void)hipFree(s.counters);
+}
+static int level_split_begin(mpdx_unet::LevelSplitState& s, int B, hipStream_t st, unsigned* base_out) {
+    if (B > kSplitMaxB) return fail(MPDX_E_STATE, "paired joined launch of %d trajectories (at most %d)", B, kSplitMaxB);
+    if (s.rezero || B > s.live) {
+        HIP_TRY(hipMemsetAsync(s.counters, 0, (size_t)kSplitMaxB * kInnerRunCounterStride * sizeof(unsigned), st));
+        s.base = 0; s.rezero = false;
+    }
+    s.live = B;
+    *base_out = s.base;
+    s.base += kSplitAdvance;
+    return 0;
+}
+static int run_fused_join(mpdx_unet* u, const mpdx_unet::Fused& up, const mpdx_unet::Fused& dn, const float* packed, const float* tt_row, const float* tt_next,
+                          const float* x, float* ws, int B, const FinalArgs* fa, hipStream_t st, long long* trace = nullptr, bool split = false) {
+    if (int rc = ensure_fused_streams(u, packed, st)) return rc;
+    FusedJoinArgs ja;
+    FusedArgs d;
+    if (int rc = fill_fused_args(u, up, packed, tt_row, x, ws, B, fa, ja.up)) return rc;
+    if (int rc = fill_fused_args(u, dn, packed, tt_next, x, ws, B, nullptr, d)) return rc;
+    ja.up.trace = trace;
+    ja.dn.packed = d.packed; ja.dn.tt_row = d.tt_row;
+    for (int k = 0; k < 3; ++k) ja.dn.gout[k] = d.gout[k];
+    ja.dn.gpar_off = d.gpar_off; ja.dn.tt_lo = d.tt_lo;
+    for (int k = 0; k < kMaxFusedOps; ++k) ja.dn.sbase[k] = k < d.nops ? d.ops[k].sbase : 0;
+    if (!split) return launch_fused_join(ja, B, st);
+    FusedSplitArgs sa;
+    memset(&sa, 0, sizeof(sa));
+    if (int rc = level_split_begin(u->split, B, st, &sa.base)) return rc;
+    sa.xch = u->split.xch; sa.counters = u->split.counters; sa.status = u->run.status_dev; sa.budget = u->run.budget; sa.nb8 = split_nb8(B);
+    return launch_fused_join_split(ja, sa, B, st);
+}
+
 static long long* g_run_trace = nullptr;
 static int g_run_trace_kind = -1;
 constexpr int kRunTraceSlots = 32;
@@ -859,7 +893,7 @@
 template <class Hook>
 static int walk_pass(mpdx_unet* u, const std::vector<mpdx_unet::Unit>& units, const float* packed, const float* row, const float* x, float* ws,
                      int B, FinalArgs& fa, hipStream_t st, Hook&& hook, bool first_done = false, const float* next_row = nullptr,
-                     long long* join_trace = nullptr) {
+                     long long* join_trace = nullptr, bool split = false) {
     const int n = (int)units.size();
     bool final_done = false;
     for (int i = first_done ? 1 : 0; i < n; ++i) {
@@ -867,7 +901,7 @@
         if (un.kind == mpdx_unet::kProgram) final_done |= u->fused[un.fused].has_final;
         if (hook(kSkipUnit, i)) continue;
         if (int rc = hook(kBeforeLaunch, i)) return rc;
-        const int rc = next_row && i == n - 1 ? run_fused_join(u, u->fused[un.fused], u->fused[units[0].fused], packed, row, next_row, x, ws, B, &fa, st, join_trace)
+        const int rc = next_row && i == n - 1 ? run_fused_join(u, u->fused[un.fused], u->fused[units[0].fused], packed, row, next_row, x, ws, B, &fa, st, join_trace, split)
                                               : run_unit(u, un, packed, row, x, ws, B, &fa, st);
         if (rc) return rc;
         if (int rc = hook(kAfterLaunch, i)) return rc;
@@ -973,10 +1007,12 @@
 }
 static int inner_run_auto_width(int B) { return (void)B, kRunNarrow; }
 static int tail_run_auto_width(int B) { return B <= 64 ? kRunNarrow : kRunWide; }
+static bool level_split_auto(int B) { return B <= kSplitMaxB; }
 struct PlanSchedule {
     std::vector<mpdx_unet::Unit> units;
     bool run = false;
     bool join = false;
+    bool split = false;
     int build(mpdx_unet* u, int B, bool with_run = true) {
         units = current_units(u, B, nullptr);
         const int cus = device_cus();
@@ -1008,6 +1044,11 @@
         if (first.kind != mpdx_unet::kProgram || last.kind != mpdx_unet::kProgram || first.fused == last.fused) return 0;
         const mpdx_unet::Fused &dn = u->fused[first.fused], &up = u->fused[last.fused];
         join = dn.program == 5 && dn.in1 == SRC_X && dn.in2 == SRC_NONE && !dn.has_final && up.program == 3 && up.has_final && B <= cus;
+        const bool want = u->level_split > 0 || (u->level_split < 0 && level_split_auto(B));
+        if (join && want && u->cfg.state_dim <= 16 && split_grid(B) <= cus && B <= kSplitMaxB && sw::geo() && !sw::debug()) {
+            if (int rc = level_split_create(u, cus)) return rc;
+            split = u->split.capacity > 0 && split_grid(B) <= u->split.capacity * std::min(1, u->split.wgs);
+        }
         return 0;
     }
 };
@@ -1078,6 +1119,21 @@
     return 0;
 }
 int mpdx_unet_plan_joined(const mpdx_unet* u) { return u ? u->plan_joined : 0; }
+int mpdx_unet_set_level_split(mpdx_unet* u, int on) {
+    if (!u) return fail(MPDX_E_INVALID, "null argument");
+    u->level_split = on < 0 ? -1 : on ? 1 : 0;
+    return 0;
+}
+int mpdx_unet_plan_split(const mpdx_unet* u) { return u ? u->plan_split : 0; }
+int mpdx_level_split_block(int B, int block, int32_t* trajectory, int32_t* role) {
+    if (B <= 0 || B > kSplitMaxB) return fail(MPDX_E_INVALID, "mpdx_level_split_block: B=%d", B);
+    const int grid = split_grid(B);
+    if (block < 0 || block >= grid) return fail(MPDX_E_INVALID, "mpdx_level_split_block: block %d of %d", block, grid);
+    const SplitSlot s = split_slot(block, split_nb8(B));
+    if (trajectory) *trajectory = s.b < B ? s.b : -1;
+    if (role) *role = s.role;
+    return grid;
+}
 
 int mpdx_unet_set_inner_run(mpdx_unet* u, int on) {
     if (!u) return fail(MPDX_E_INVALID, "null argument");
@@ -1118,6 +1174,7 @@
     if (u->run.status) __atomic_store_n(u->run.status, word, __ATOMIC_RELAXED);
     u->run.status_host = word;
     if (!word && u->run.counters) u->run.ctr[0].rezero = u->run.ctr[1].rezero = true;
+    if (!word) u->split.rezero = true;
     return 0;
 }
 
@@ -1126,6 +1183,7 @@
     if (u && u->pack_chunks_dev) (void)hipFree(u->pack_chunks_dev);
     if (u && u->jobs_dev) (void)hipFree(u->jobs_dev);
     if (u) inner_run_free(u->run);
+    if (u) level_split_free(u->split);
     delete u;
 }
 
@@ -1281,7 +1339,7 @@
     if (int rc = check_ready(u)) return rc;
     PlanSchedule ps;
     if (int rc = ps.build(u, B)) return rc;
-    u->inner_runs = u->inner_run_layers = u->plan_joined = 0;
+    u->inner_runs = u->inner_run_layers = u->plan_joined = u->plan_split = 0;
     hipStream_t st = (hipStream_t)stream;
     const int H = u->cfg.n_support_points, D = u->cfg.state_dim;
     const size_t n = (size_t)B * H * D;
@@ -1322,10 +1380,11 @@
         } else {
             fa.mode = 2; fa.absmax = fl;
         }
-        if (int rc = walk_pass(u, ps.units, packed, timetab + (size_t)t * u->tt_row, padded_input(u, x, ws, B, st), ws, B, fa, st, no_hook, down_done, tt_next))
+        if (int rc = walk_pass(u, ps.units, packed, timetab + (size_t)t * u->tt_row, padded_input(u, x, ws, B, st), ws, B, fa, st, no_hook, down_done, tt_next, nullptr, ps.split))
             return rc;
         down_done = join;
         u->plan_joined += join ? 1 : 0;
+        u->plan_split += join && ps.split ? 1 : 0;
         if (guided) {
             for (int j = 0; j < n_guide_steps; ++j) {
                 const bool last = j == n_guide_steps - 1;
@@ -1345,7 +1404,7 @@
         }
     }
     HIP_TRY(hipGetLastError());
-    return ps.run ? handle_status_error(u, "mpdx_plan") : 0;
+    return ps.run || ps.split ? handle_status_error(u, "mpdx_plan") : 0;
 }
 
 int mpdx_randn(float* out, size_t n, uint64_t seed, uint64_t offset, void* stream) {
diff --git a/mpd_public_amd/csrc/unet_measure.hpp b/mpd_public_amd/csrc/unet_measure.hpp
--- a/mpd_public_amd/csrc/unet_measure.hpp
+++ b/mpd_public_amd/csrc/unet_measure.hpp
@@ -143,7 +143,7 @@
         if (pass == 2 && run_kind >= 0) { g_run_trace = dev.p; g_run_trace_kind = run_kind; }
         else if (pass == 2 && !joined) { g_fused_trace = dev.p; g_fused_trace_seg = seg; }
         const float* next_row = pass == 2 && joined ? timetab : nullptr;
-        if (int rc = walk_pass(u, ps.units, packed, timetab, padded_input(u, x, ws, B, st), ws, B, fa, st, no_hook, false, next_row, dev.p)) return rc;
+        if (int rc = walk_pass(u, ps.units, packed, timetab, padded_input(u, x, ws, B, st), ws, B, fa, st, no_hook, false, next_row, dev.p, ps.split)) return rc;
     }
     HIP_TRY(hipStreamSynchronize(st));
     const int n = std::min(cap, 1024);
diff --git a/mpd_public_amd/temporal_unet.py b/mpd_public_amd/temporal_unet.py
--- a/mpd_public_amd/temporal_unet.py
+++ b/mpd_public_amd/temporal_unet.py
@@ -158,6 +158,12 @@
 
     def plan_joined(self) -> int:
         return int(_lib.load().mpdx_unet_plan_joined(self._handle()))
+
+    def set_level_split(self, on):
+        _lib.check(_lib.load().mpdx_unet_set_level_split(self._handle(), -1 if on is None else int(bool(on))), "mpdx_unet_set_level_split")
+
+    def plan_split(self) -> int:
+        return int(_lib.load().mpdx_unet_plan_split(self._handle()))
 
     def set_inner_run(self, on: bool):
         _lib.check(_lib.load().mpdx_unet_set_inner_run(self._handle(), int(bool(on))), "mpdx_unet_set_inner_run")
```

Result: faster. 6664 denoising-steps/s (median of 6 runs) (+2.8%).
